# stefanopini/simple-HRNet

Hardware: AMD Instinct MI355X
Metric: person-crops/sec HRNet-W48 384x288 (model forward + heat-map decode) (higher is better)
Workload: dtype bf16; 1 GPU; HRNet-W48 384x288, batch=256 random crops per GPU, bf16 MFMA (BASELINE configs[2]); global_batch=256, micro_batch=256, lanes_per_gpu=1, parallelism=dp1 (crop sharding, RCCL all-gather of keypoints), weights=random-init seeded (synth_state_dict seed 0), BN stats randomised, engine_switches=

## Files before the change

include/hrnet_mi355.h:

```cpp
#ifndef HRNET_MI355_H
#define HRNET_MI355_H

#include <stddef.h>
#include <stdint.h>

#ifdef __cplusplus
extern "C" {
#endif

typedef struct hrn_ctx *hrn_handle;

enum { HRN_F32 = 0, HRN_BF16 = 1, HRN_F16 = 2 };
enum { HRN_BOX_I32 = 0, HRN_BOX_F32 = 1 };
enum { HRN_T_F32 = 0, HRN_T_I64 = 1 };

typedef struct {
    const char *name;
    const void *data;
    int32_t ndim;
    int64_t dims[4];
    int32_t dtype;
} hrn_tensor_desc;

typedef struct {
// ... 117 lines not shown
enum { HRN_LB_RGB = 0, HRN_LB_BGR = 1 };
enum { HRN_DET_COMPACT = 1 };
enum { HRN_DET_MAX_CLASSES = 16 };
typedef struct { int32_t new_w, new_h, left, top; double ratio_w, ratio_h, dw, dh; } hrn_letterbox;
int hrn_letterbox_geometry(int rule, const int32_t *frame_hw , int n, int out_h, int out_w,
                           hrn_letterbox *out );
const char *hrn_letterbox_last_error(void);
int hrn_letterbox_frames(hrn_handle h, const hrn_frame *frames_host, int n, int rule, int out_h, int out_w,
                         const uint8_t *pad , int order, int form, void *out_dev, hrn_letterbox *geometry_host ,
                         void *stream);
int hrn_letterbox_frames_yuv(hrn_handle h, const hrn_yuv_frame *frames_host, int n, int rule, int out_h, int out_w,
                             const uint8_t *pad , int order, int form, void *out_dev,
                             hrn_letterbox *geometry_host , void *stream);
int hrn_detections_to_frame(int rule, const float *dets, int det_stride, const int32_t *start , int P,
                            const hrn_letterbox *geometry, const int32_t *frame_hw , int out_h, int out_w,
                            int conf_col, float conf_thres, int class_col, const int32_t *classes, int nclasses, int flags,
                            float *dets_out, int32_t *counts_out , int32_t *status_out );
int hrn_detections_to_frame_dev(hrn_handle h, int rule, const float *dets_dev, int det_stride, const int32_t *start_host, int P,
                                const hrn_letterbox *geometry_host, const int32_t *frame_hw_host, int out_h, int out_w,
                                int conf_col, float conf_thres, int class_col, const int32_t *classes_host, int nclasses, int flags,
                                float *dets_out_dev, int32_t *counts_dev, int32_t *status_dev, void *stream);

enum { HRN_INTER_NEAREST = 0, HRN_INTER_LINEAR = 1, HRN_INTER_CUBIC = 2 };
int hrn_resize_frames(hrn_handle h, const uint8_t *frames_dev, int n, int frame_h, int frame_w, int interpolation,
                      float *images_dev, void *stream);

int hrn_warp_crops(hrn_handle h, const uint8_t *frames_dev, int nframes, int frame_h, int frame_w,
                   const int32_t *frame_index_host, const double *matrices_host, int n, float *images_dev, void *stream);

int hrn_forward_flip_tta(hrn_handle h, const void *images_dev, int n, const int32_t *flip_pairs_host, int npairs,
                         int post_processing, float *heatmaps_dev, float *preds_dev, float *maxvals_dev, void *stream);

int hrn_target_centers(const double *joints, const float *vis, const float *joints_weight , int n, int J,
                       int height, int width, double sigma, int32_t *mu_out, float *draw_out, float *target_weight_out);
int hrn_generate_targets(hrn_handle h, const double *joints_host, const float *vis_host, const float *joints_weight_host,
                         int n, double sigma, float *targets_dev, float *target_weight_host, void *stream);
typedef struct {
    double *loss_mse, *loss_ohkm;
    float *avg_acc;
    int32_t *cnt;
    float *acc, *dists;
    double *map_loss;
    float *preds, *target_preds, *maxvals;
} hrn_score_out;
int hrn_score_heatmaps(hrn_handle h, const float *heatmaps_dev, int n, const float *targets_dev, const double *joints_host,
                       const float *vis_host, const float *joints_weight_host, double sigma, const float *target_weight_host,
                       float pck_thr, int ohkm_topk, const hrn_score_out *out_dev, void *stream);

enum { HRN_REFINE_NONE = 0, HRN_REFINE_QUARTER = 1, HRN_REFINE_DARK = 2 };
int hrn_forward_refined(hrn_handle h, const void *images_dev, int n, const void *boxes_dev, int box_dtype, int refine,
                        float *pts_dev, float *heatmaps_dev, void *stream);
int hrn_refine_coords(hrn_handle h, const float *heatmaps_dev, int n, int refine, float *coords_dev, void *stream);

int hrn_nms(int32_t *keep_out, int32_t *num_out, const float *boxes_host, int boxes_num, int boxes_dim,
            float nms_overlap_thresh, int device_id);
int hrn_nms_release(int device_id);
const char *hrn_nms_last_error(void);

int hrn_oks_nms(int32_t *keep_out, int32_t *num_out, const double *kpts, const double *areas, const int32_t *order, int n, int J,
                double thresh, const double *sigmas, double in_vis_thre);
int hrn_soft_oks_nms(int32_t *keep_out, int32_t *num_out, const double *kpts, const double *areas, const double *scores_sorted,
                     const int32_t *order, int n, int J, double thresh, const double *sigmas, double in_vis_thre);
int hrn_pose_similarity(const double *boxes_a, const float *poses_a, int na, const double *boxes_b, const float *poses_b, int nb, int J,
                        float *sim_bbox, float *sim_pose);
int hrn_assignment(const double *cost, int rows, int cols, int32_t *row_to_col);

typedef struct {
    char name[96];
    int32_t c, h, w;
    int32_t conv_index;
} hrn_tap_info;
int hrn_tap_count(hrn_handle h);
int hrn_get_tap_info(hrn_handle h, int index, hrn_tap_info *out);
int hrn_forward_tap(hrn_handle h, const void *images_dev, int n, const char *tap_name, int crop0, int ncrops, int crop_step,
                    float *dst_dev, float *heatmaps_dev, void *stream);

int hrn_conv_count(hrn_handle h);
int hrn_get_conv_info(hrn_handle h, int index, hrn_conv_info *out);
double hrn_flops_per_crop(hrn_handle h);
int64_t hrn_workspace_bytes(hrn_handle h);
int64_t hrn_map_rebuilds(hrn_handle h);
int hrn_launches_per_pass(hrn_handle h);
int hrn_stem_fused(hrn_handle h);
int hrn_conv_compact(hrn_handle h, int index);
const char *hrn_switches(hrn_handle h);
int64_t hrn_debug_pad_violations(hrn_handle h);
int hrn_plan_block_map(hrn_handle h, int group, int n, int reverse, int32_t *blocks, int capacity, int32_t *members,
                       int member_capacity);
int hrn_plan_direct_map(hrn_handle h, int group, int n, int32_t *blocks, int capacity, int32_t *members, int member_capacity,
                        int32_t *pixels_per_tile);
int hrn_plan_s2_map(hrn_handle h, int group, int n, int32_t *blocks, int capacity, int32_t *parts, int part_capacity,
                    int32_t *active);
int hrn_profile_pass(hrn_handle h, const void *images_dev, int n, float *conv_ms, int conv_ms_len,
                     float *other_ms , void *stream);
const char *hrn_version(void);

#ifdef __cplusplus
}
#endif
#endif
```

simple-hrnet_amd/_lib.py:

```python
from __future__ import annotations

import ctypes
import os
import shutil
import subprocess
from typing import List

_HERE = os.path.dirname(os.path.abspath(__file__))
CSRC = os.path.join(_HERE, "csrc")
INCLUDE = os.path.join(os.path.dirname(_HERE), "include")
LIB_PATH = os.path.join(_HERE, "libhrnet_mi355.so")
if os.environ.get("HRN_LIB_TAG"):
    LIB_PATH = LIB_PATH.replace(".so", "_%s.so" % os.environ["HRN_LIB_TAG"])
SOURCES = ["kernels.hip", "conv3x3_lds.hip", "conv_s2.hip", "stem_fused.hip", "conv3x3_f32.hip", "bottleneck_chain.hip", "prepath.hip", "warp.hip", "nms.hip", "postproc.cpp", "hrnet_mi355.cpp",
           "decode.hip",
           "score.hip",
           "draw.hip",
           "track.hip",
           "pose_nms.hip",
           "letterbox.hip",
           "assoc.hip",
           "conv3x3_lds_f16.hip", "conv_s2_f16.hip", "bottleneck_chain_f16.hip"]
HEADERS = [os.path.join(CSRC, "kernels.h"), os.path.join(CSRC, "dt16.h"), os.path.join(CSRC, "argmax.h"), os.path.join(CSRC, "conv3x3_n96.inc"), os.path.join(CSRC, "conv3x3_lds.inc"),
           os.path.join(CSRC, "conv_s2.inc"), os.path.join(CSRC, "bottleneck_chain.inc"), os.path.join(INCLUDE, "hrnet_mi355.h")]
# ... 45 lines not shown

def _stale(src: str) -> bool:
    o = _obj(src)
    if not os.path.exists(o) or not _stamp_ok():
        return True
    t = os.path.getmtime(o)
    return any(os.path.getmtime(d) > t for d in _deps(src))


def needs_build() -> bool:
    if not os.path.exists(LIB_PATH):
        return True
    if os.environ.get("HRN_LIB_TAG"):
        return False
    t = os.path.getmtime(LIB_PATH)
    deps = set()
    for s in SOURCES:
        deps.update(_deps(s))
    if any(os.path.getmtime(d) > t for d in deps):
        return True
    if os.path.isdir(_obj_dir()) and not _stamp_ok():
        return shutil.which("hipcc") is not None or os.path.exists("/opt/rocm/bin/hipcc")
    return False


def build(force: bool = False, verbose: bool = False) -> str:
    if not force and not needs_build():
        return LIB_PATH
    import fcntl
    from concurrent.futures import ThreadPoolExecutor

    os.makedirs(_obj_dir(), exist_ok=True)
    with open(os.path.join(_obj_dir(), "build.lock"), "w") as lock:
        fcntl.flock(lock, fcntl.LOCK_EX)
        try:
            if force or needs_build():
                os.makedirs(_obj_dir(), exist_ok=True)
                cflags = [f for f in HIPCC_FLAGS if f != "-shared"]

                def compile_one(src):
                    tmp = "%s.tmp.%d" % (_obj(src), os.getpid())
                    cmd = [_hipcc()] + cflags + ["-c", "-o", tmp, os.path.join(CSRC, src)]
                    if verbose:
                        print(" ".join(cmd), flush=True)
                    subprocess.check_call(cmd)
                    os.replace(tmp, _obj(src))

                todo = [s for s in SOURCES if force or _stale(s)]
                stamp = _stamp()
                with ThreadPoolExecutor(max_workers=min(len(todo), os.cpu_count() or 4, MAX_BUILD_WORKERS) or 1) as ex:
                    list(ex.map(compile_one, todo))
                tmp = "%s.tmp.%d" % (LIB_PATH, os.getpid())
                cmd = [_hipcc(), "--offload-arch=gfx950", "-shared", "-fPIC", "-o", tmp] + [_obj(s) for s in SOURCES]
                if verbose:
                    print(" ".join(cmd), flush=True)
                subprocess.check_call(cmd)
                with open(os.path.join(_obj_dir(), "build.stamp"), "w") as f:
                    f.write(stamp + "\n")
                os.replace(tmp, LIB_PATH)
        finally:
            fcntl.flock(lock, fcntl.LOCK_UN)
    return LIB_PATH


class TensorDesc(ctypes.Structure):
    _fields_ = [("name", ctypes.c_char_p), ("data", ctypes.c_void_p), ("ndim", ctypes.c_int32),
                ("dims", ctypes.c_int64 * 4), ("dtype", ctypes.c_int32)]


class ConvInfo(ctypes.Structure):
    _fields_ = [("name", ctypes.c_char * 96),
                ("cin", ctypes.c_int32), ("cout", ctypes.c_int32), ("ksize", ctypes.c_int32),
                ("stride", ctypes.c_int32), ("relu", ctypes.c_int32), ("has_residual", ctypes.c_int32),
                ("in_h", ctypes.c_int32), ("in_w", ctypes.c_int32), ("out_h", ctypes.c_int32),
                ("out_w", ctypes.c_int32), ("kpad", ctypes.c_int32), ("nr", ctypes.c_int32),
                ("algo", ctypes.c_int32), ("ks", ctypes.c_int32),
                ("w_offset", ctypes.c_int64), ("w_bytes", ctypes.c_int64), ("b_offset", ctypes.c_int64),
                ("flops", ctypes.c_double)]


class TapInfo(ctypes.Structure):
    _fields_ = [("name", ctypes.c_char * 96), ("c", ctypes.c_int32), ("h", ctypes.c_int32), ("w", ctypes.c_int32),
                ("conv_index", ctypes.c_int32)]


class ScoreOut(ctypes.Structure):
    _fields_ = [(name, ctypes.c_void_p) for name in ("loss_mse", "loss_ohkm", "avg_acc", "cnt", "acc", "dists", "map_loss", "preds",
                                                     "target_preds", "maxvals")]


class Frame(ctypes.Structure):
    _fields_ = [("data", ctypes.c_void_p), ("height", ctypes.c_int32), ("width", ctypes.c_int32)]


class YuvFrameC(ctypes.Structure):
    _fields_ = [("y", ctypes.c_void_p), ("u", ctypes.c_void_p), ("v", ctypes.c_void_p), ("height", ctypes.c_int32),
                ("width", ctypes.c_int32), ("pitch_y", ctypes.c_int32), ("pitch_c", ctypes.c_int32), ("format", ctypes.c_int32),
                ("matrix", ctypes.c_int32), ("range", ctypes.c_int32)]


class Letterbox(ctypes.Structure):
    _fields_ = [("new_w", ctypes.c_int32), ("new_h", ctypes.c_int32), ("left", ctypes.c_int32), ("top", ctypes.c_int32),
                ("ratio_w", ctypes.c_double), ("ratio_h", ctypes.c_double), ("dw", ctypes.c_double), ("dh", ctypes.c_double)]


class CanvasC(ctypes.Structure):
    _fields_ = list(YuvFrameC._fields_)


_P = ctypes.c_void_p
SYMBOLS = {
    "hrn_create": (ctypes.c_int, [ctypes.POINTER(_P), ctypes.c_int, ctypes.c_int, ctypes.c_int, ctypes.c_int,
                                  ctypes.c_int, ctypes.c_int, ctypes.c_int]),
    "hrn_create_model": (ctypes.c_int, [ctypes.POINTER(_P), ctypes.c_int, ctypes.c_int, ctypes.c_int, ctypes.c_int,
                                        ctypes.c_int, ctypes.c_int, ctypes.c_int, ctypes.c_int]),
    "hrn_destroy": (None, [_P]),
    "hrn_last_error": (ctypes.c_char_p, [_P]),
    "hrn_load_weights": (ctypes.c_int, [_P, ctypes.POINTER(TensorDesc), ctypes.c_int]),
    "hrn_weight_blob_bytes": (ctypes.c_int64, [_P]),
    "hrn_weight_blob_ptr": (_P, [_P]),
    "hrn_adopt_weights": (ctypes.c_int, [_P]),
    "hrn_weight_blob_read": (ctypes.c_int, [_P, ctypes.c_int64, _P, ctypes.c_int64]),
    "hrn_forward": (ctypes.c_int, [_P, _P, ctypes.c_int, _P, ctypes.c_int, _P, _P, _P]),
    "hrn_resize_frames": (ctypes.c_int, [_P, _P, ctypes.c_int, ctypes.c_int, ctypes.c_int, ctypes.c_int, _P, _P]),
    "hrn_warp_crops": (ctypes.c_int, [_P, _P, ctypes.c_int, ctypes.c_int, ctypes.c_int, _P, _P, ctypes.c_int, _P, _P]),
    "hrn_target_centers": (ctypes.c_int, [_P, _P, _P, ctypes.c_int, ctypes.c_int, ctypes.c_int, ctypes.c_int, ctypes.c_double, _P, _P, _P]),
    "hrn_generate_targets": (ctypes.c_int, [_P, _P, _P, _P, ctypes.c_int, ctypes.c_double, _P, _P, _P]),
    "hrn_score_heatmaps": (ctypes.c_int, [_P, _P, ctypes.c_int, _P, _P, _P, _P, ctypes.c_double, _P, ctypes.c_float, ctypes.c_int,
                                          ctypes.POINTER(ScoreOut), _P]),
    "hrn_preprocess_frame": (ctypes.c_int, [_P, _P, ctypes.c_int, ctypes.c_int, _P, ctypes.c_int, ctypes.c_int, ctypes.c_int, _P, _P, _P, _P]),
    "hrn_preprocess_frames": (ctypes.c_int, [_P, ctypes.POINTER(Frame), ctypes.c_int, _P, ctypes.c_int, _P, ctypes.c_int, ctypes.c_int, _P, _P, _P, _P]),
    "hrn_yuv_coefficients": (ctypes.c_int, [ctypes.c_int, ctypes.c_int, _P]),
    "hrn_yuv_to_bgr": (ctypes.c_int, [_P, ctypes.POINTER(YuvFrameC), _P, _P]),
    "hrn_preprocess_frames_yuv": (ctypes.c_int, [_P, ctypes.POINTER(YuvFrameC), ctypes.c_int, _P, ctypes.c_int, _P, ctypes.c_int, ctypes.c_int,
                                                 _P, _P, _P, _P]),
    "hrn_draw_poses": (ctypes.c_int, [_P, ctypes.POINTER(CanvasC), ctypes.c_int, _P, ctypes.c_int, ctypes.c_int, _P, _P, ctypes.c_int,
                                      _P, ctypes.c_int, _P, ctypes.c_int, _P, ctypes.c_int, ctypes.c_int, ctypes.c_float, _P]),
    "hrn_draw_poses_ids_dev": (ctypes.c_int, [_P, ctypes.POINTER(CanvasC), ctypes.c_int, _P, ctypes.c_int, ctypes.c_int, _P, _P, ctypes.c_int,
                                              _P, ctypes.c_int, _P, ctypes.c_int, _P, ctypes.c_int, ctypes.c_int, ctypes.c_float, _P]),
    "hrn_associate_people": (ctypes.c_int, [ctypes.c_int, _P, _P, ctypes.c_int, _P, _P, _P, _P, _P, _P, ctypes.c_double, ctypes.c_double,
                                            ctypes.c_double, _P, _P, _P]),
    "hrn_associate_people_last_error": (ctypes.c_char_p, []),
    "hrn_associate_people_dev": (ctypes.c_int, [_P, ctypes.c_int, _P, _P, ctypes.c_int, _P, _P, _P, _P, _P, _P, ctypes.c_double,
                                                ctypes.c_double, ctypes.c_double, _P, _P, _P, _P]),
    "hrn_assoc_exp": (ctypes.c_int, [_P, ctypes.c_int, _P]),
    "hrn_associate_similarity": (ctypes.c_int, [_P, _P, ctypes.c_int, _P, _P, ctypes.c_int, ctypes.c_int, ctypes.c_double, _P, _P]),
    "hrn_pose_nms": (ctypes.c_int, [ctypes.c_int, _P, ctypes.c_int, ctypes.c_int, _P, _P, _P, ctypes.c_double, ctypes.c_double,
                                    ctypes.c_double, _P, _P, _P, _P, _P, _P]),
    "hrn_pose_nms_last_error": (ctypes.c_char_p, []),
    "hrn_pose_nms_dev": (ctypes.c_int, [_P, ctypes.c_int, _P, ctypes.c_int, ctypes.c_int, _P, _P, _P, ctypes.c_double, ctypes.c_double,
                                        ctypes.c_double, _P, _P, _P, _P, _P, _P, _P]),
    "hrn_pose_nms_oks_row": (ctypes.c_int, [ctypes.c_int, ctypes.c_int, ctypes.c_int, _P, _P, ctypes.c_int, ctypes.c_double, _P, _P]),
    "hrn_letterbox_geometry": (ctypes.c_int, [ctypes.c_int, _P, ctypes.c_int, ctypes.c_int, ctypes.c_int, _P]),
    "hrn_letterbox_last_error": (ctypes.c_char_p, []),
    "hrn_letterbox_frames": (ctypes.c_int, [_P, ctypes.POINTER(Frame), ctypes.c_int, ctypes.c_int, ctypes.c_int, ctypes.c_int, _P, ctypes.c_int,
                                            ctypes.c_int, _P, _P, _P]),
    "hrn_letterbox_frames_yuv": (ctypes.c_int, [_P, ctypes.POINTER(YuvFrameC), ctypes.c_int, ctypes.c_int, ctypes.c_int, ctypes.c_int, _P,
                                                ctypes.c_int, ctypes.c_int, _P, _P, _P]),
    "hrn_detections_to_frame": (ctypes.c_int, [ctypes.c_int, _P, ctypes.c_int, _P, ctypes.c_int, _P, _P, ctypes.c_int, ctypes.c_int, ctypes.c_int,
                                               ctypes.c_float, ctypes.c_int, _P, ctypes.c_int, ctypes.c_int, _P, _P, _P]),
    "hrn_detections_to_frame_dev": (ctypes.c_int, [_P, ctypes.c_int, _P, ctypes.c_int, _P, ctypes.c_int, _P, _P, ctypes.c_int, ctypes.c_int,
                                                   ctypes.c_int, ctypes.c_float, ctypes.c_int, _P, ctypes.c_int, ctypes.c_int, _P, _P, _P, _P]),
    "hrn_yuv_from_bgr": (ctypes.c_int, [ctypes.c_int, ctypes.c_int, _P, ctypes.c_int, _P]),
    "hrn_crop_geometry": (ctypes.c_int, [_P, ctypes.c_int, ctypes.c_int, _P, ctypes.c_int, ctypes.c_int, ctypes.c_int, ctypes.c_int, _P, _P]),
    "hrn_crop_geometry_last_error": (ctypes.c_char_p, []),
    "hrn_pose_boxes": (ctypes.c_int, [_P, ctypes.c_int, ctypes.c_int, _P, ctypes.c_int, ctypes.c_float, ctypes.c_int, ctypes.c_double,
                                      ctypes.c_double, _P]),
    "hrn_pose_boxes_last_error": (ctypes.c_char_p, []),
    "hrn_boxes_from_poses": (ctypes.c_int, [_P, _P, ctypes.c_int, ctypes.c_int, _P, ctypes.c_int, ctypes.c_float, ctypes.c_int,
                                            ctypes.c_double, ctypes.c_double, _P, _P]),
    "hrn_preprocess_frames_dev": (ctypes.c_int, [_P, ctypes.POINTER(Frame), ctypes.c_int, _P, ctypes.c_int, _P, ctypes.c_int, ctypes.c_int,
                                                 _P, _P, _P, _P]),
    "hrn_preprocess_frames_yuv_dev": (ctypes.c_int, [_P, ctypes.POINTER(YuvFrameC), ctypes.c_int, _P, ctypes.c_int, _P, ctypes.c_int,
                                                     ctypes.c_int, _P, _P, _P, _P]),
    "hrn_forward_flip_tta": (ctypes.c_int, [_P, _P, ctypes.c_int, _P, ctypes.c_int, ctypes.c_int, _P, _P, _P, _P]),
    "hrn_forward_refined": (ctypes.c_int, [_P, _P, ctypes.c_int, _P, ctypes.c_int, ctypes.c_int, _P, _P, _P]),
    "hrn_refine_coords": (ctypes.c_int, [_P, _P, ctypes.c_int, ctypes.c_int, _P, _P]),
    "hrn_nms": (ctypes.c_int, [_P, _P, _P, ctypes.c_int, ctypes.c_int, ctypes.c_float, ctypes.c_int]),
    "hrn_nms_release": (ctypes.c_int, [ctypes.c_int]),
    "hrn_nms_last_error": (ctypes.c_char_p, []),
    "hrn_oks_nms": (ctypes.c_int, [_P, _P, _P, _P, _P, ctypes.c_int, ctypes.c_int, ctypes.c_double, _P, ctypes.c_double]),
    "hrn_soft_oks_nms": (ctypes.c_int, [_P, _P, _P, _P, _P, _P, ctypes.c_int, ctypes.c_int, ctypes.c_double, _P, ctypes.c_double]),
    "hrn_pose_similarity": (ctypes.c_int, [_P, _P, ctypes.c_int, _P, _P, ctypes.c_int, ctypes.c_int, _P, _P]),
    "hrn_assignment": (ctypes.c_int, [_P, ctypes.c_int, ctypes.c_int, _P]),
    "hrn_tap_count": (ctypes.c_int, [_P]),
    "hrn_get_tap_info": (ctypes.c_int, [_P, ctypes.c_int, ctypes.POINTER(TapInfo)]),
    "hrn_forward_tap": (ctypes.c_int, [_P, _P, ctypes.c_int, ctypes.c_char_p, ctypes.c_int, ctypes.c_int, ctypes.c_int, _P, _P, _P]),
    "hrn_conv_count": (ctypes.c_int, [_P]),
    "hrn_get_conv_info": (ctypes.c_int, [_P, ctypes.c_int, ctypes.POINTER(ConvInfo)]),
    "hrn_flops_per_crop": (ctypes.c_double, [_P]),
    "hrn_workspace_bytes": (ctypes.c_int64, [_P]),
    "hrn_map_rebuilds": (ctypes.c_int64, [_P]),
    "hrn_launches_per_pass": (ctypes.c_int, [_P]),
    "hrn_switches": (ctypes.c_char_p, [_P]),
    "hrn_stem_fused": (ctypes.c_int, [_P]),
    "hrn_conv_compact": (ctypes.c_int, [_P, ctypes.c_int]),
    "hrn_debug_pad_violations": (ctypes.c_int64, [_P]),
    "hrn_plan_block_map": (ctypes.c_int, [_P, ctypes.c_int, ctypes.c_int, ctypes.c_int, _P, ctypes.c_int, _P, ctypes.c_int]),
    "hrn_plan_direct_map": (ctypes.c_int, [_P, ctypes.c_int, ctypes.c_int, _P, ctypes.c_int, _P, ctypes.c_int, _P]),
    "hrn_plan_s2_map": (ctypes.c_int, [_P, ctypes.c_int, ctypes.c_int, _P, ctypes.c_int, _P, ctypes.c_int, _P]),
    "hrn_profile_pass": (ctypes.c_int, [_P, _P, ctypes.c_int, ctypes.POINTER(ctypes.c_float), ctypes.c_int,
                                        ctypes.POINTER(ctypes.c_float), _P]),
    "hrn_version": (ctypes.c_char_p, []),
}

_lib = None


def load(auto_build: bool = True) -> ctypes.CDLL:
    global _lib
    if _lib is not None:
        return _lib
    if auto_build and needs_build():
        build()
    lib = ctypes.CDLL(LIB_PATH)
    for name, (res, args) in SYMBOLS.items():
        fn = getattr(lib, name)
        fn.restype = res
        fn.argtypes = args
    _lib = lib
    return lib


def header_symbols() -> List[str]:
    import re

    text = open(os.path.join(INCLUDE, "hrnet_mi355.h")).read()
    text = re.sub(r"/\*.*?\*/", "", text, flags=re.S)
    return sorted(set(re.findall(r"\b(hrn_[a-z_0-9]+)\s*\(", text)))
```

simple-hrnet_amd/csrc/ctx_memory.inc:

```
    bool hip_ok(hipError_t e, const char *what) {
        if (e == hipSuccess) return true;
        err = std::string(what) + ": " + hipGetErrorString(e);
        return false;
    }
    bool refuse_plan_only() {
        if (plan_only) err = "plan-only handle (device_id < 0): there is no CPU compute path";
        return plan_only;
    }

    bool allocate() {
        workspace_bytes = 0;
        for (auto &b : buffers) workspace_bytes += (int64_t)b.bytes;
        const int64_t small_crops = std::min<int64_t>(max_batch, (191 + head_slabs) / head_slabs);
        const int64_t part = std::max((int64_t)max_batch * joints * head_slabs, small_crops * joints * head_slabs_small);
        workspace_bytes += part * 8;
        if (plan_only) {
            fill_problems();
            index_s2groups();
            blob = (char *)calloc(1, (size_t)blob_bytes);
            return blob != nullptr;
        }
        if (!hip_ok(hipSetDevice(device), "hipSetDevice")) return false;
        for (auto &b : buffers) {
            if (!hip_ok(hipMalloc((void **)&b.dev, b.bytes), "hipMalloc(activation)")) return false;
// ... 45 lines not shown
        const bool keep_short_full = small && small_keep_above > 0 && small_blocks > small_keep_above;
        auto short_conv = [&](const ConvOp &cv) { return cv.ks != 16 && !cv.n96 && (cv.ks == 48 ? 2 : 1) * cv.slices <= 2; };
        auto small_conv = [&](const ConvOp &cv) {
            if (cv.ks == 16 && f32_small_slices > 0 && cv.slices >= f32_small_slices) return true;
            return small && !(keep_short_full && short_conv(cv));
        };
        auto tile_px = [&](const ConvOp &cv, const Tensor &to) {
            return fused_now(cv, nb) ? 512 : small_conv(cv) ? 128 : conv3x3_lds_bm(cv.ks, cv.nr, to.wp);
        };
        auto tiles_per_block = [&](const ConvOp &cv, int div) {
            return std::max(1, conv3_tiles_per_block(cv) / (fused_now(cv, nb) ? bbf_tpb_div : 1) / div);
        };
        auto count_blocks = [&](int div) {
            long total = 0;
            for (int ci : g.conv_idx) {
                const ConvOp &cv = convs[ci];
                if (skipped(cv, nb)) continue;
                const Tensor &to = tensors[cv.out_t];
                const int bm = tile_px(cv, to);
                const int mtiles = (int)((m_pixels(cv, to, nb) + bm - 1) / bm);
                const int tpb = tiles_per_block(cv, div);
                total += (long)((mtiles + tpb - 1) / tpb) * cv.ntiles;
            }
            return total;
        };
        int div = 1;
        while (div < 64 && count_blocks(div) < 512) div *= 2;
        int lf = all_short ? 1 : (int)std::min<long>(long_factor, count_blocks(div) / 768);
        if (lf < 1) lf = 1;
        for (size_t k = 0; k < g.conv_idx.size(); ++k) {
            const ConvOp &cv = convs[g.conv_idx[k]];
            if (skipped(cv, nb)) continue;
            const Tensor &to = tensors[cv.out_t];
            const int bm = tile_px(cv, to);
            const bool fused = fused_now(cv, nb);
            const int prob = fused ? g.fused_prob[k] : (int)k;
            const int mtiles = (int)((m_pixels(cv, to, nb) + bm - 1) / bm);
            const int tpb_short = tiles_per_block(cv, div);
            const int tpb_long = tpb_short * lf;
            const int long_tiles = ((int)(mtiles * long_share) / (8 * tpb_long)) * (8 * tpb_long);
            for (int phase = 0; phase < 2; ++phase) {
                const int tpb = phase == 0 ? tpb_long : tpb_short;
                const int first = phase == 0 ? 0 : long_tiles;
                const int count = phase == 0 ? long_tiles : mtiles - long_tiles;
                if (count <= 0) continue;
                const int mgroups = (count + tpb - 1) / tpb;
                const int total = mgroups * cv.ntiles;
                int seq = 0;
                for (int round = 0; round * 8 < mgroups; ++round)
                    for (int nt = 0; nt < cv.ntiles; ++nt)
                        for (int x = 0; x < 8; ++x) {
                            const int mg = round * 8 + x;
                            if (mg >= mgroups) continue;
                            const int i = seq++;
                            int tiles = count - mg * tpb;
                            if (tiles > tpb) tiles = tpb;
                            double key = (i + 0.5) / total;
                            if (block_order == 1)
                                key = -(fused ? 28000.0 + (tiles - 1) * bbf_slide_cost
                                        : (double)tiles * (cv.ks == 16 ? cv.slices * (double)bm * 36.0 + 2000.0
                                                        : cv.n96      ? cv.slices * 3.0 * (bm == 512 ? 3900.0 : 3000.0) + (bm == 512 ? 7000.0 : 5000.0)
                                                                 : cv.slices * 2.0 * (bm == 512 ? 4300.0 : 3500.0) + (bm == 512 ? 5000.0 : 3000.0))) +
                                      1e-3 * key;
                            int mt0 = first + mg * tpb;
                            if (reverse) mt0 = mtiles - mt0 - tiles;
                            ents.push_back({key, int2{prob | (nt << 8) | (tiles << 16), mt0 | (fused ? 1 << 29 : small_conv(cv) ? 1 << 30 : 0)}, bm});
                        }
            }
        }
        std::stable_sort(ents.begin(), ents.end(), [](const Ent &a, const Ent &b) { return a.key < b.key; });
        if (tile_px_out) {
            tile_px_out->resize(ents.size());
            for (size_t i = 0; i < ents.size(); ++i) (*tile_px_out)[i] = ents[i].bm;
        }
        if (out) {
            out->resize(ents.size());
            for (size_t i = 0; i < ents.size(); ++i) (*out)[i] = ents[i].v;
        }
        return (int)ents.size();
    }

    const Tensor &grid_of(const ConvOp &cv) const { return tensors[cv.up ? cv.in_t : cv.out_t]; }

    ConvArgs conv_args(const ConvOp &cv, int nb, bool rev) const {
        const Tensor &ti = tensors[cv.in_t], &to = grid_of(cv);
        ConvArgs a;
        a.in = row0(cv.in_t), a.out = row0(cv.out_t);
        a.w = blob + cv.w_off, a.bias = (const float *)(blob + cv.b_off);
        a.res = cv.res_t >= 0 ? row0(cv.res_t) : nullptr;
        a.cin = cv.cin, a.cout = cv.cout;
        a.in_wp = ti.wp, a.in_hpwp = ti.hpwp;
        a.out_h = to.h, a.out_w = to.w, a.out_wp = to.wp, a.out_hpwp = to.hpwp;
        a.m = nb * to.hpwp;
        a.ksize = cv.k, a.stride = cv.stride, a.relu = cv.relu, a.kchunks = cv.kchunks;
        a.rev = rev;
        a.pre_mode = pre_mode;
        a.wlds = direct_wlds && is16() ? 1 : 0;
        a.xlds = conv_xl(cv) ? 1 : 0;
        a.up = cv.up ? 1 : 0, a.up_a = cv.up ? (cv.up - 1) >> 1 : 0, a.up_b = cv.up ? (cv.up - 1) & 1 : 0;
        a.up_wp = tensors[cv.out_t].wp, a.up_hpwp = tensors[cv.out_t].hpwp;
        for (int t = 0; t < 4; ++t) {
            const int dy = (t >> 1) - 1 + a.up_a, dx = (t & 1) - 1 + a.up_b;
            a.taps[t] = cv.up ? dy * ti.wp + dx : 0;
        }
        return a;
    }

    int direct_group_blocks(const DirectGroup &g, int nb, std::vector<int2> *out, int mr = 4) const {
        struct Cls {
            int in_t, k, stride;
            std::vector<int> members;
            double cost = 0;
        };
        std::vector<Cls> cls;
        for (size_t k = 0; k < g.conv_idx.size(); ++k) {
            const ConvOp &cv = convs[g.conv_idx[k]];
            size_t ci = 0;
            for (; ci < cls.size(); ++ci)
                if (cls[ci].in_t == cv.in_t && cls[ci].k == cv.k && cls[ci].stride == cv.stride) break;
            if (ci == cls.size()) cls.push_back(Cls{cv.in_t, cv.k, cv.stride, {}, 0});
            cls[ci].members.push_back((int)k);
            cls[ci].cost += (double)grid_of(cv).hpwp * (cv.cout / (16 * g.nr)) * cv.kchunks;
        }
        std::stable_sort(cls.begin(), cls.end(), [](const Cls &a, const Cls &b) { return a.cost > b.cost; });
        int n = 0;
        if (out) out->clear();
        for (const Cls &cl : cls) {
            const int mtiles = (nb * grid_of(convs[g.conv_idx[cl.members[0]]]).hpwp + 64 * mr - 1) / (64 * mr);
            for (int round = 0; round * 8 < mtiles; ++round)
                for (int k : cl.members) {
                    const int ngroups = convs[g.conv_idx[k]].cout / (16 * g.nr);
                    for (int ng = 0; ng < ngroups; ++ng)
                        for (int x = 0; x < 8; ++x, ++n)
                            if (out) out->push_back(int2{k | (ng << 8), round * 8 + x});
                }
        }
        return n;
    }

    int64_t m_pixels(const ConvOp &cv, const Tensor &to, int nb) const {
        return cv.compact ? (int64_t)nb * to.h * to.w : (int64_t)nb * to.hpwp;
    }
    static int compact_slab_rows(int h, int w, int bm, int crops) {
        const int wp = w + 1, hpwp = (h + 1) * wp, hw = h * w;
        auto flat = [&](int64_t c) { const int64_t n = c / hw, r = c % hw; return n * hpwp + (r / w) * wp + r % w; };
        const int64_t m = (int64_t)crops * hw;
        int64_t span = 0;
        for (int64_t c0 = 0; c0 < m; c0 += bm) span = std::max(span, flat(std::min(c0 + bm, m) - 1) - flat(c0) + 1);
        return (int)span + 2 * wp + 2;
    }

    bool setup_dgroups() {
        for (auto &g : dgroups) {
            g.map_capacity = std::max<int64_t>(direct_group_blocks(g, max_batch, nullptr), 4 * 512 + 64 * (int64_t)g.conv_idx.size() * 8);
            for (MapSlot &sl : g.slot) {
                if (!alloc_slot(sl, g.map_capacity, g.conv_idx.size())) return false;
                workspace_bytes += g.map_capacity * (int64_t)sizeof(int2) + (int64_t)(g.conv_idx.size() * sizeof(ConvArgs));
            }
        }
        return true;
    }

    size_t index_s2groups() {
        size_t n = 0;
        for (auto &g : s2groups) g.prob_first = (int)n, n += g.probs.size();
        if (stem_fuse) stemf.prob_first = (int)n, n += stemf.probs.size();
        return n;
    }
    long s2_tiles(const S2Group &g, int nb) const {
        long t = 0;
        for (auto &pr : g.probs) t += (long)nb * pr.tiles_per_image;
        return t;
    }
    bool s2_active(const S2Group &g, int nb) const { return s2_tiles(g, nb) >= s2_min_tiles; }
    int s2_blocks(const S2Group &g, int nb, std::vector<int2> *out) const {
        struct Ent {
            double key;
            int2 v;
        };
        std::vector<double> cost(g.probs.size());
        double total = 0;
        for (size_t k = 0; k < g.probs.size(); ++k) {
            const S2Group::Prob &pr = g.probs[k];
            const Tensor &to = tensors[convs[pr.parts[0].first].out_t];
            const int frags = (pr.rows * to.wp + 15) / 16;
            const int wm = std::max(1, 8 / (int)pr.parts.size());
            const int cin = convs[pr.parts[0].first].cin;
            cost[k] = (double)((frags + wm - 1) / wm) * ((9 * cin + 31) / 32) * s2_frags_per_part(cin) + 60;
            total += cost[k] * nb * pr.tiles_per_image;
        }
        const double per_block = total / s2_target_blocks;
        std::vector<Ent> ents;
        for (size_t k = 0; k < g.probs.size(); ++k) {
            const S2Group::Prob &pr = g.probs[k];
            const int tiles = nb * pr.tiles_per_image;
            int run = (int)(per_block / cost[k] + 0.5);
            run = run < 1 ? 1 : run > 64 ? 64 : run;
            if (&g == &stemf) run = (tiles + s2_target_blocks - 1) / s2_target_blocks;
            for (int t0 = 0; t0 < tiles; t0 += run) {
                const int cnt = tiles - t0 < run ? tiles - t0 : run;
                ents.push_back({-(cnt * cost[k]) + 1e-9 * t0, int2{(int)k | (cnt << 8), t0}});
            }
        }
        std::stable_sort(ents.begin(), ents.end(), [](const Ent &a, const Ent &b) { return a.key < b.key; });
        if (out) {
            out->resize(ents.size());
            for (size_t i = 0; i < ents.size(); ++i) (*out)[i] = ents[i].v;
        }
        return (int)ents.size();
    }

    static void s2_wave_table(int nparts, unsigned char *part, unsigned char *f0, unsigned char *fs) {
        struct W {
            int p, i, m;
        };
        std::vector<W> ws;
        for (int p = 0; p < nparts; ++p) {
            const int m = std::max(1, 8 / nparts + (p < 8 % nparts ? 1 : 0));
            for (int i = 0; i < m && (int)ws.size() < 8; ++i) ws.push_back({p, i, m});
        }
        std::stable_sort(ws.begin(), ws.end(), [](const W &a, const W &b) { return a.m < b.m; });
        double load[4] = {0, 0, 0, 0};
        bool used[8] = {};
        for (int w = 0; w < 8; ++w) part[w] = 0xff, f0[w] = 0, fs[w] = 1;
        for (const W &x : ws) {
            int best = -1;
            for (int w = 0; w < 8; ++w)
                if (!used[w] && (best < 0 || load[w & 3] < load[best & 3] - 1e-12)) best = w;
            used[best] = true;
            load[best & 3] += 1.0 / x.m;
            part[best] = (unsigned char)x.p, f0[best] = (unsigned char)x.i, fs[best] = (unsigned char)x.m;
        }
    }

    bool setup_s2groups() {
        const size_t nprob = index_s2groups();
        if (!nprob) return true;
        std::vector<S2Problem> hp(nprob);
        std::vector<S2Group *> all;
        for (auto &g : s2groups) all.push_back(&g);
        if (stem_fuse) all.push_back(&stemf);
// ... 91 lines not shown

    size_t fill_problems() {
        const size_t nprob = index_groups();
        probs_host.assign(nprob, Conv3Problem{});
        std::vector<Conv3Problem> &hp = probs_host;
        for (auto &g : groups) {
            g.max_wp = 0;
            for (size_t k = 0; k < g.conv_idx.size(); ++k) {
                const ConvOp &cv = convs[g.conv_idx[k]];
                const Tensor &to = tensors[cv.out_t];
                Conv3Problem &q = hp[g.prob_first + k];
                q.in = row0(cv.in_t), q.out = row0(cv.out_t);
                q.w = blob + cv.w_off, q.bias = (const float *)(blob + cv.b_off);
                q.res = cv.res_t >= 0 ? row0(cv.res_t) : nullptr;
                q.cin = cv.cin, q.cout = cv.cout, q.h = to.h, q.wd = to.w, q.wp = to.wp, q.hpwp = to.hpwp;
                q.relu = cv.relu, q.slices = cv.slices, q.ntiles = cv.ntiles;
                q.w2 = nullptr, q.bias2 = nullptr;
                q.n96 = cv.n96 ? 1 : 0;
                q.compact = cv.compact ? 1 : 0, q.hw = to.h * to.w;
                q.slab_rows = q.slab_rows_small = 0;
                if (cv.compact) {
                    fast_div(q.hw, &q.magic_hw, &q.shift_hw);
                    fast_div(to.w, &q.magic_w, &q.shift_w);
                    q.slab_rows = compact_slab_rows(to.h, to.w, 512, max_batch), q.slab_rows_small = compact_slab_rows(to.h, to.w, 128, max_batch);
                }
                q.tiles_per_block = conv3_tiles_per_block(cv);
                q.bm = conv3x3_lds_bm(cv.ks, cv.nr, to.wp);
                fast_div(to.hpwp, &q.magic_hpwp, &q.shift_hpwp);
                fast_div(to.wp, &q.magic_wp, &q.shift_wp);
                if (to.wp > g.max_wp) g.max_wp = to.wp;
                if (cv.fuse_with >= 0) {
                    const ConvOp &c2 = convs[cv.fuse_with];
                    Conv3Problem &f = hp[g.prob_first + g.fused_prob[k]];
                    f = q;
                    f.out = row0(c2.out_t), f.relu = c2.relu, f.res = nullptr;
                    f.w2 = blob + c2.w_off, f.bias2 = (const float *)(blob + c2.b_off);
                }
            }
        }
        return nprob;
    }

    bool setup_groups() {
        const size_t nprob = fill_problems();
        if (!nprob) return true;
        std::vector<Conv3Problem> &hp = probs_host;
        for (auto &g : groups) {
            g.map_capacity = 64 + 4 * (int64_t)std::max(small_below, 256) + 1024;
            for (int ci : g.conv_idx) {
                const ConvOp &cv = convs[ci];
                const Tensor &to = tensors[cv.out_t];
                const int bm = f32_small_slices > 0 ? 128 : conv3x3_lds_bm(cv.ks, cv.nr, to.wp);
                g.map_capacity += (int64_t)((max_batch * to.hpwp + bm - 1) / bm) * cv.ntiles;
            }
            for (MapSlot &sl : g.slot) {
                if (!alloc_slot(sl, g.map_capacity, 0)) return false;
                workspace_bytes += g.map_capacity * (int64_t)sizeof(int2);
            }
        }
        if (!hip_ok(hipMalloc((void **)&probs_dev, nprob * sizeof(Conv3Problem)), "hipMalloc(problems)")) return false;
        return hip_ok(hipMemcpy(probs_dev, hp.data(), nprob * sizeof(Conv3Problem), hipMemcpyHostToDevice),
                      "hipMemcpy(problems)");
    }

    void free_all() {
        if (plan_only) {
            free(blob);
        } else {
            (void)hipSetDevice(device);
            for (auto &b : buffers)
                if (b.dev) (void)hipFree(b.dev);
            if (blob) (void)hipFree(blob);
            if (scratch_hm) (void)hipFree(scratch_hm);
            free_scratch();
            if (part_val) (void)hipFree(part_val);
            if (part_idx) (void)hipFree(part_idx);
            if (probs_dev) (void)hipFree(probs_dev);
            if (s2probs_dev) (void)hipFree(s2probs_dev);
            for (auto &g : s2groups)
                for (MapSlot &sl : g.slot) free_slot(sl);
            for (MapSlot &sl : stemf.slot) free_slot(sl);
            for (auto &g : groups)
                for (MapSlot &sl : g.slot) free_slot(sl);
            for (auto &g : dgroups)
                for (MapSlot &sl : g.slot) free_slot(sl);
        }
        blob = nullptr;
    }

    char *row0(int t) const {
        const Tensor &tt = tensors[t];
        const Buffer &b = buffers[tt.buf];
        return b.dev ? b.dev + b.lead_rows * tt.c * esize : nullptr;
    }
```

simple-hrnet_amd/csrc/ctx_plan.inc:

```
    int new_tensor(int ch, int h, int w) {
        Tensor t;
        t.c = ch, t.h = h, t.w = w, t.wp = w + 1, t.hp = h + 1, t.hpwp = t.wp * t.hp;
        for (size_t i = 0; i < buffers.size(); ++i)
            if (!buffers[i].in_use && buffers[i].c == ch && buffers[i].h == h && buffers[i].w == w) {
                t.buf = (int)i;
                break;
            }
        if (t.buf < 0) {
            Buffer b;
            b.c = ch, b.h = h, b.w = w;
            b.lead_rows = (size_t)t.wp + 1;
            b.rows = b.lead_rows + (size_t)max_batch * t.hpwp + t.wp + 1 + kConvBlockRows;
            b.bytes = (size_t)align_up((int64_t)(b.rows * ch * esize), 256);
            buffers.push_back(b);
            t.buf = (int)buffers.size() - 1;
        }
        buffers[t.buf].in_use = true;
        tensors.push_back(t);
        return (int)tensors.size() - 1;
    }
    void release(int t) { buffers[tensors[t].buf].in_use = false; }

    int default_nr(int cout, int stride) const {
        int nr = (cout % 64 == 0) ? 4 : (cout % 48 == 0) ? 3 : 2;
        if (is16() && stride == 2 && cout % 96 == 0 && direct_nr6) nr = 6;
        return nr;
    }
    int common_nr(const std::vector<int> &couts, int stride) const {
        bool all64 = true, all48 = true, all96 = true;
        for (int co : couts) all64 &= co % 64 == 0, all48 &= co % 48 == 0, all96 &= co % 96 == 0;
        if (is16() && stride == 2 && all96 && direct_nr6) return 6;
        return all64 ? 4 : all48 ? 3 : 2;
    }

    static int s2_rows(int wop, int ho, int cin) {
        const int r = (s2_slot_capacity(cin) - 2 * wop) / s2_pair_pitch(wop);
        return r > ho ? ho : (r < 0 ? 0 : r);
    }

    int add_conv(const std::string &conv, const std::string &bn, int in_t, int cout, int k, int stride, int relu,
                 int res_t = -1, bool emit = true, int nr_override = 0, int up = 0, int up_out_t = -1, bool force_generic = false) {
        const Tensor ti = tensors[in_t];
        ConvOp op;
        op.conv = conv, op.bn = bn, op.in_t = in_t, op.res_t = res_t;
        op.cin = ti.c, op.cout = cout, op.k = k, op.stride = stride, op.relu = relu;
        const int oh = ti.h / stride, ow = ti.w / stride;
        op.up = up;
        op.out_t = up ? up_out_t : new_tensor(cout, oh, ow);
        const int kc = is16() ? 32 : 16;
        const int K = k * k * op.cin;
        op.kchunks = (K + kc - 1) / kc;
        op.kpad = op.kchunks * kc;
        op.nr = nr_override ? nr_override : default_nr(cout, stride);
        op.flops = 2.0 * cout * (double)K * oh * ow;
        int lds_ks = 0, lds_nrb = 0;
        if (is16() && k == 3 && stride == 1 && !disable_lds && !up && !force_generic) {
            const int64_t out_bytes = ((int64_t)max_batch * (oh + 1) * (ow + 1) + 2 * (ow + 2) + 512) * std::max(op.cin, cout) * 2;
            if (!disable_n96 && op.cin % 32 == 0 && cout % 96 == 0 && conv3x3_lds_bm(32, 6, ow + 1) > 0 && out_bytes < (int64_t(1) << 32))
                lds_ks = 32, lds_nrb = 6, op.n96 = true;
            else if (op.cin % 48 == 0 && cout % 48 == 0)
                lds_ks = 48, lds_nrb = 3;
            else if (op.cin % 32 == 0 && !disable_lds32)
                lds_ks = 32, lds_nrb = cout % 64 == 0 ? 4 : cout % 48 == 0 ? 3 : cout % 32 == 0 ? 2 : 0;
            if (lds_nrb && conv3x3_lds_bm(lds_ks, lds_nrb, ow + 1) == 0) lds_nrb = 0;
            if (op.n96 && lds_nrb == 6 && !disable_compact && conv3x3_lds_bm(32, 6, ow + 1) == 512 &&
                1.0 - (double)(oh * ow) / ((oh + 1) * (ow + 1)) >= compact_min_pad &&
                (compact_slab_rows(oh, ow, 512, max_batch) + 15) / 16 * 16 <= conv3x3_n96_max_rows() && (int64_t)max_batch * oh * ow < (int64_t(1) << 27))
                op.compact = true;
        }
        if (lds_nrb) {
            op.algo = 1, op.ks = lds_ks, op.nr = lds_nrb;
            op.slices = op.cin / lds_ks, op.ntiles = cout / (16 * lds_nrb), op.nch = (9 * lds_ks + 31) / 32;
            op.kpad = op.nch * 32 * op.slices;
        }
        if (dtype == HRN_F32 && k == 3 && stride == 1 && !up && !disable_lds && !disable_f32lds && op.cin % 16 == 0 &&
            (cout % 48 == 0 || cout % 32 == 0) && conv3x3_lds_bm(16, cout % 48 == 0 ? 3 : 2, ow + 1) > 0) {
            op.algo = 1, op.ks = 16, op.nr = cout % 48 == 0 ? 3 : 2;
            op.slices = op.cin / 16, op.ntiles = cout / (16 * op.nr), op.nch = 9;
            op.kpad = 9 * 16 * op.slices;
        }
        if (is16() && k == 3 && stride == 2 && (op.cin == 48 || op.cin == 32 || op.cin == 64) &&
            cout % (16 * s2_frags_per_part(op.cin)) == 0 && !up && !disable_s2 && op.algo == 0 &&
            (s2_rows(ow + 1, oh, op.cin) >= 2 || s2_rows(ow + 1, oh, op.cin) == oh))
            op.s2 = true;
        convs.push_back(op);
        if (emit) emit_convs({(int)convs.size() - 1});
        return op.out_t;
    }

    static int c3_family(const ConvOp &cv) { return ((cv.ks == 48 && cv.nr == 3) || cv.n96) ? 0 : cv.ks * 16 + cv.nr; }

    void emit_direct(const std::vector<int> &idx, std::vector<Op> &dst) {
        std::vector<std::vector<int>> dsets;
        for (int i : idx) {
            if (disable_dgroup) {
                dst.push_back({OP_CONV, i});
                continue;
            }
            bool placed = false;
            for (auto &set : dsets)
                if (convs[set[0]].nr == convs[i].nr && set.size() < 255) {
                    set.push_back(i);
                    placed = true;
                    break;
                }
            if (!placed) dsets.push_back({i});
        }
        for (auto &set : dsets) {
            if (set.size() == 1) {
                dst.push_back({OP_CONV, set[0]});
                continue;
            }
            DirectGroup g;
            g.conv_idx = set, g.nr = convs[set[0]].nr;
            dgroups.push_back(g);
            dst.push_back({OP_CONV_GROUP, (int)dgroups.size() - 1});
        }
    }

    void emit_convs(const std::vector<int> &idx) {
        std::vector<int> lds, direct, s2;
        for (int i : idx) {
            if (convs[i].algo == 1)
                lds.push_back(i);
            else if (convs[i].s2)
                s2.push_back(i);
            else
                direct.push_back(i);
        }
        emit_direct(direct, ops);
        if (!s2.empty()) {
            S2Group g;
            g.conv_idx = s2;
            for (int i : s2) {
                const ConvOp &cv = convs[i];
                for (int t = 0; t < cv.cout / (16 * s2_frags_per_part(cv.cin)); ++t) {
                    S2Group::Prob *pr = nullptr;
                    for (auto &q : g.probs)
                        if (q.in_t == cv.in_t && (int)q.parts.size() < kS2MaxParts) pr = &q;
                    if (!pr) {
                        g.probs.push_back(S2Group::Prob());
                        pr = &g.probs.back();
                        pr->in_t = cv.in_t;
                        const Tensor &to = tensors[cv.out_t];
                        pr->rows = s2_rows(to.wp, to.h, cv.cin);
                        pr->tiles_per_image = (to.h + pr->rows - 1) / pr->rows;
                    }
                    pr->parts.push_back({i, t});
                }
            }
            emit_direct(s2, g.fallback);
            s2groups.push_back(g);
            ops.push_back({OP_S2_GROUP, (int)s2groups.size() - 1});
        }
        if (lds.empty()) return;
        std::vector<std::vector<int>> sets;
        for (int i : lds) {
            bool placed = false;
            if (!disable_group)
                for (auto &set : sets)
                    if (c3_family(convs[set[0]]) == c3_family(convs[i])) {
                        set.push_back(i);
                        placed = true;
                        break;
                    }
            if (!placed) sets.push_back({i});
        }
        for (auto &set : sets) {
            Conv3Group g;
            g.conv_idx = set;
            groups.push_back(g);
            ops.push_back({OP_CONV3_GROUP, (int)groups.size() - 1});
        }
    }

    int add_fuse(const std::vector<int> &terms, const std::vector<int> &shifts, const std::string &name) {
        FuseOp f;
        f.name = name;
        f.nterms = (int)terms.size();
        for (int i = 0; i < f.nterms; ++i) f.term_t[i] = terms[i], f.shift[i] = shifts[i];
        const Tensor &t0 = tensors[terms[0]];
        int ref = -1;
        for (int i = 0; i < f.nterms; ++i)
            if (shifts[i] == 0) ref = terms[i];
        const Tensor &tr = tensors[ref >= 0 ? ref : terms[0]];
        (void)t0;
        f.out_t = new_tensor(tr.c, tr.h, tr.w);
        fuses.push_back(f);
        return f.out_t;
    }

    void add_stage(const std::string &name, std::vector<int> &xs, int nout) {
        const int nb = (int)xs.size();
        char buf[160];
        for (int k = 0; k < 4; ++k) {
            std::vector<int> t1(nb), g1, g2;
            for (int b = 0; b < nb; ++b) {
                snprintf(buf, sizeof buf, "%s.branches.%d.%d", name.c_str(), b, k);
                const std::string p = buf;
                t1[b] = add_conv(p + ".conv1", p + ".bn1", xs[b], c << b, 3, 1, 1, -1, false);
                g1.push_back((int)convs.size() - 1);
            }
            emit_convs(g1);
            for (int b = 0; b < nb; ++b) {
                snprintf(buf, sizeof buf, "%s.branches.%d.%d", name.c_str(), b, k);
                const std::string p = buf;
                const int t2 = add_conv(p + ".conv2", p + ".bn2", t1[b], c << b, 3, 1, 1, xs[b], false);
                const int i2 = (int)convs.size() - 1, i1 = g1[b];
                const ConvOp &a1 = convs[i1], &a2 = convs[i2];
                if (!disable_bbf && is16() && a1.algo == 1 && a2.algo == 1 && a1.ks == 48 && a1.nr == 3 && a1.slices == 1 &&
                    a1.ntiles == 1 && a2.slices == 1 && a2.ntiles == 1 && conv3x3_lds_bbf_ok(tensors[t2].wp)) {
                    convs[i1].fuse_with = i2;
                    convs[i2].fused_away = true;
                }
                g2.push_back(i2);
                release(t1[b]);
                release(xs[b]);
                xs[b] = t2;
            }
            emit_convs(g2);
        }
        std::vector<std::vector<int>> term(nout, std::vector<int>(nb, -1));
        std::vector<std::vector<int>> cur(nout, std::vector<int>(nb, -1));
        for (int level = 0; level < nb; ++level) {
            std::vector<int> made, dead;
            for (int j = 0; j < nb; ++j) {
                std::vector<int> c1, c2;
                if (level == 0)
                    for (int i = 0; i < nout && i < j; ++i) c1.push_back(c << i);
                for (int i = j + 1 + level; i < nout; ++i)
                    if (level == 0) c2.push_back(i - j == 1 ? (c << i) : (c << j));
                const int nr1 = (dgroup_nr_mode == 1 && c1.size() > 1) ? common_nr(c1, 1) : 0;
                const int nr2 = (dgroup_nr_mode == 1 && c2.size() > 1) ? common_nr(c2, 2) : 0;
                for (int i = 0; i < nout; ++i) {
                    snprintf(buf, sizeof buf, "%s.fuse_layers.%d.%d", name.c_str(), i, j);
                    const std::string q = buf;
                    if (i < j && level == 0) {
                        term[i][j] = add_conv(q + ".0", q + ".1", xs[j], c << i, 1, 1, 0, -1, false, nr1);
                        made.push_back((int)convs.size() - 1);
                    } else if (i > j && level < i - j) {
                        const bool last = (level == i - j - 1);
                        snprintf(buf, sizeof buf, "%s.%d", q.c_str(), level);
                        const std::string qq = buf;
                        const int src = level == 0 ? xs[j] : cur[i][j];
                        const int nt = add_conv(qq + ".0", qq + ".1", src, last ? (c << i) : (c << j), 3, 2, last ? 0 : 1, -1,
                                                false, level == 0 ? nr2 : 0);
                        made.push_back((int)convs.size() - 1);
                        if (level > 0) dead.push_back(src);
                        cur[i][j] = nt;
                        if (last) term[i][j] = nt;
                    }
                }
            }
            if (made.empty()) break;
            emit_convs(made);
            for (int t : dead) release(t);
        }
        std::vector<int> outs;
        for (int i = 0; i < nout; ++i) {
            std::vector<int> terms, shifts;
            for (int j = 0; j < nb; ++j) {
                terms.push_back(i == j ? xs[j] : term[i][j]);
                shifts.push_back(i < j ? j - i : 0);
            }
            snprintf(buf, sizeof buf, "%s.fuse.%d", name.c_str(), i);
            outs.push_back(add_fuse(terms, shifts, buf));
        }
        {
            const int first = (int)fuses.size() - nout;
            for (int i = 0; i < nout; ++i) {
                fuses[first + i].group = disable_fgroup ? 1 : (i == 0 ? nout : 0);
                if (fuses[first + i].group) ops.push_back({OP_FUSE, first + i});
            }
        }
        for (int i = 0; i < nout; ++i)
            for (int j = 0; j < nb; ++j)
                if (i != j) release(term[i][j]);
        for (int b = 0; b < nb; ++b) release(xs[b]);
        xs = outs;
    }

    int add_layer1(int x, int nblocks) {
        char buf[96];
        int o1_next = -1;
        for (int b = 0; b < nblocks; ++b) {
            snprintf(buf, sizeof buf, "layer1.%d", b);
            const std::string p = buf;
            int o1 = o1_next, r = x;
            const bool chain = is16() && !disable_chain && b < nblocks - 1;
            int ds_idx = -1;
            if (b == 0 && chain && !disable_chain_ds) {
                o1 = add_conv(p + ".conv1", p + ".bn1", x, 64, 1, 1, 1);
                r = add_conv(p + ".downsample.0", p + ".downsample.1", x, 256, 1, 1, 0, -1, false, 2);
                ds_idx = (int)convs.size() - 1;
                release(r);
            } else if (b == 0) {
                o1 = add_conv(p + ".conv1", p + ".bn1", x, 64, 1, 1, 1, -1, false);
                r = add_conv(p + ".downsample.0", p + ".downsample.1", x, 256, 1, 1, 0, -1, false);
                emit_convs({(int)convs.size() - 2, (int)convs.size() - 1});
            } else if (o1 < 0) {
                o1 = add_conv(p + ".conv1", p + ".bn1", x, 64, 1, 1, 1);
            }
            const bool c2_generic = is16() && b >= 1;
            const bool chain3 = c2_generic && !disable_chain && !disable_chain3;
            const int o2 = c2_generic ? add_conv(p + ".conv2", p + ".bn2", o1, 64, 3, 1, 1, -1, !chain3, 2, 0, -1, true)
                                      : add_conv(p + ".conv2", p + ".bn2", o1, 64, 3, 1, 1);
            const int i2 = (int)convs.size() - 1;
            int o3;
            o1_next = -1;
            if (chain3 && !chain) {
                o3 = add_conv(p + ".conv3", p + ".bn3", o2, 256, 1, 1, 1, r, false, 2);
                chains.push_back({(int)convs.size() - 1, -1, -1, i2});
                ops.push_back({OP_CHAIN, (int)chains.size() - 1});
            } else if (chain) {
                snprintf(buf, sizeof buf, "layer1.%d", b + 1);
                const std::string pn = buf;
                o3 = add_conv(p + ".conv3", p + ".bn3", o2, 256, 1, 1, 1, r, false, 2);
                const int i3 = (int)convs.size() - 1;
                o1_next = add_conv(pn + ".conv1", pn + ".bn1", o3, 64, 1, 1, 1, -1, false, 4);
                chains.push_back({i3, (int)convs.size() - 1, ds_idx, chain3 ? i2 : -1});
                ops.push_back({OP_CHAIN, (int)chains.size() - 1});
            } else {
                o3 = add_conv(p + ".conv3", p + ".bn3", o2, 256, 1, 1, 1, r);
            }
            release(o1), release(o2);
            if (b == 0 && ds_idx < 0) release(r);
            release(x);
            x = o3;
        }
        return x;
    }

    void build_plan_poseresnet() {
        static const int spec50[4] = {3, 4, 6, 3}, spec101[4] = {3, 4, 23, 3}, spec152[4] = {3, 8, 36, 3};
        const int *layers = c == 50 ? spec50 : c == 101 ? spec101 : spec152;
        stem_out_t = new_tensor(64, H / 2, W / 2);
        ops.push_back({OP_STEM7, 0});
        int x = new_tensor(64, H / 4, W / 4);
        pool_in_t = stem_out_t, pool_out_t = x;
        ops.push_back({OP_MAXPOOL, 0});
        release(stem_out_t);
        char buf[96];
        x = add_layer1(x, layers[0]);
        for (int li = 1; li < 4; ++li) {
            const int planes = 64 << li;
            for (int b = 0; b < layers[li]; ++b) {
                snprintf(buf, sizeof buf, "layer%d.%d", li + 1, b);
                const std::string p = buf;
                const int stride = (b == 0 && li > 0) ? 2 : 1;
                int r = x;
                const int o1 = add_conv(p + ".conv1", p + ".bn1", x, planes, 1, 1, 1, -1, false);
                std::vector<int> first{(int)convs.size() - 1};
                if (b == 0) {
                    r = add_conv(p + ".downsample.0", p + ".downsample.1", x, planes * 4, 1, stride, 0, -1, false);
                    first.push_back((int)convs.size() - 1);
                }
                emit_convs(first);
                const int o2 = add_conv(p + ".conv2", p + ".bn2", o1, planes, 3, stride, 1);
                const int o3 = add_conv(p + ".conv3", p + ".bn3", o2, planes * 4, 1, 1, 1, r);
                release(o1), release(o2);
                if (b == 0) release(r);
                release(x);
                x = o3;
            }
        }
        for (int i = 0; i < 3; ++i) {
            const Tensor tx = tensors[x];
            const int up_t = new_tensor(256, tx.h * 2, tx.w * 2);
            snprintf(buf, sizeof buf, "deconv_layers.%d", 3 * i);
            const std::string cn = buf;
            snprintf(buf, sizeof buf, "deconv_layers.%d", 3 * i + 1);
            const std::string bn = buf;
            std::vector<int> phases;
            for (int ph = 0; ph < 4; ++ph) {
                add_conv(cn, bn, x, 256, 2, 1, 1, -1, false, 0, 1 + ph, up_t);
                phases.push_back((int)convs.size() - 1);
            }
            emit_convs(phases);
            release(x);
            x = up_t;
        }
        head_in_t = x;
        head_c = tensors[x].c;
        ops.push_back({OP_HEAD, 0});
        ops.push_back({OP_DECODE, 0});
        layout_blob();
    }

    void build_plan() {
        if (model == 1) return build_plan_poseresnet();
        head_c = c;
        stem_out_t = new_tensor(64, H / 2, W / 2);
        ops.push_back({OP_STEM, 0});
        int x = add_conv("conv2", "bn2", stem_out_t, 64, 3, 2, 1);
        stem_conv2_op = (int)ops.size() - 1;
        if (is16() && !disable_stem_fuse && !disable_stem_mfma && stem_fused_fits(tensors[x].wp, W)) {
            stem_fuse = true;
            convs.back().w2_image = true;
            stemf = S2Group();
            stemf.conv_idx = {(int)convs.size() - 1};
            for (int t = 0; t < 2; ++t) {
                if (stemf.probs.empty()) {
                    stemf.probs.push_back(S2Group::Prob());
                    stemf.probs[0].in_t = stem_out_t;
                    stemf.probs[0].rows = 1, stemf.probs[0].tiles_per_image = tensors[x].h;
                }
                stemf.probs[0].parts.push_back({(int)convs.size() - 1, t});
            }
        }
        release(stem_out_t);
        char buf[96];
        x = add_layer1(x, 4);
        std::vector<int> xs;
        xs.push_back(add_conv("transition1.0.0", "transition1.0.1", x, c, 3, 1, 1, -1, false));
        xs.push_back(add_conv("transition1.1.0.0", "transition1.1.0.1", x, 2 * c, 3, 2, 1, -1, false));
        emit_convs({(int)convs.size() - 2, (int)convs.size() - 1});
        release(x);
        add_stage("stage2.0", xs, 2);
        xs.push_back(add_conv("transition2.2.0.0", "transition2.2.0.1", xs[1], 4 * c, 3, 2, 1));
        for (int m = 0; m < 4; ++m) {
            snprintf(buf, sizeof buf, "stage3.%d", m);
            add_stage(buf, xs, 3);
        }
        xs.push_back(add_conv("transition3.3.0.0", "transition3.3.0.1", xs[2], 8 * c, 3, 2, 1));
        add_stage("stage4.0", xs, 4);
        add_stage("stage4.1", xs, 4);
        add_stage("stage4.2", xs, 1);
        head_in_t = xs[0];
        ops.push_back({OP_HEAD, 0});
        ops.push_back({OP_DECODE, 0});

        layout_blob();
    }

    void index_taps() {
        taps.clear();
        auto add = [&](const std::string &name, int tensor, int op, int conv) {
            for (TapPoint &t : taps)
                if (t.name == name) {
                    t.op = op;
                    return;
                }
            taps.push_back(TapPoint{name, tensor, op, conv});
        };
        for (size_t oi = 0; oi < ops.size(); ++oi) {
            const Op &op = ops[oi];
            switch (op.kind) {
                case OP_STEM:
                case OP_STEM7: add("stem", stem_out_t, (int)oi, -1); break;
                case OP_MAXPOOL: add("maxpool", pool_out_t, (int)oi, -1); break;
                case OP_CONV: add(convs[op.idx].conv, convs[op.idx].out_t, (int)oi, op.idx); break;
                case OP_CONV3_GROUP:
                    for (int ci : groups[op.idx].conv_idx) add(convs[ci].conv, convs[ci].out_t, (int)oi, ci);
                    break;
                case OP_CONV_GROUP:
                    for (int ci : dgroups[op.idx].conv_idx) add(convs[ci].conv, convs[ci].out_t, (int)oi, ci);
                    break;
                case OP_S2_GROUP:
                    for (int ci : s2groups[op.idx].conv_idx) add(convs[ci].conv, convs[ci].out_t, (int)oi, ci);
                    break;
                case OP_CHAIN:
                    add(convs[chains[op.idx].conv3].conv, convs[chains[op.idx].conv3].out_t, (int)oi, chains[op.idx].conv3);
                    if (chains[op.idx].conv1 >= 0)
                        add(convs[chains[op.idx].conv1].conv, convs[chains[op.idx].conv1].out_t, (int)oi, chains[op.idx].conv1);
                    break;
                case OP_FUSE:
                    for (int k = 0; k < fuses[op.idx].group; ++k) add(fuses[op.idx + k].name, fuses[op.idx + k].out_t, (int)oi, -1);
                    break;
                default: break;
            }
        }
    }

    void layout_blob() {
        int64_t off = 0;
        stem_w_off = off, off = align_up(off + (model == 1 ? 147 : 27) * 64 * 4, 256);
        stem_b_off = off, off = align_up(off + 64 * 4, 256);
        stem_wp_off = off, off = align_up(off + (model == 1 ? 5 : 1) * 4 * 1024, 256);
        for (auto &cv : convs) {
            cv.w_off = off;
            cv.w_bytes = cv.algo == 1 ? (int64_t)cv.ntiles * cv.slices * cv.nch * cv.nr * 1024
                                      : (int64_t)(cv.cout / 16) * cv.kchunks * 1024;
            off = align_up(off + cv.w_bytes, 256);
            cv.b_off = off;
            off = align_up(off + cv.cout * 4, 256);
            if (cv.s2 || cv.w2_image) {
                const int nf = s2_frags_per_part(cv.cin);
                cv.w2_off = off;
                cv.w2_bytes = (int64_t)(cv.cout / (16 * nf)) * ((9 * cv.cin + 31) / 32) * nf * 1024;
                off = align_up(off + cv.w2_bytes, 256);
            }
        }
        head_w_off = off, off = align_up(off + (int64_t)joints * head_c * 4, 256);
        head_b_off = off, off = align_up(off + joints * 4, 256);
        head_wp_off = off, off = align_up(off + (int64_t)((joints + 31) / 32) * 2 * ((head_c + 31) / 32) * 1024, 256);
        blob_bytes = off;

        const int hw = (H / 4) * (W / 4);
        head_slab_px = 1024;
        head_slabs = (hw + head_slab_px - 1) / head_slab_px;
        head_slabs_small = (hw + kHeadSlabPxSmall - 1) / kHeadSlabPxSmall;
    }
```

simple-hrnet_amd/csrc/ctx_run.inc:

```
    struct Timing {
        std::vector<hipEvent_t> ev;
    };

    bool run_pass(const float *images, int nb, const void *boxes, int box_dtype, float *pts, float *heatmaps,
                  hipStream_t s, Timing *tm, int flip = 0, const TapReq *tap = nullptr, int refine = RF_NONE) {
        if (tm && !hip_ok(hipEventRecord(tm->ev[0], s), "hipEventRecord")) return false;
        const bool fused_stem = stem_fuse && !(tap && tap->op == 0);
        for (size_t oi = 0; oi < ops.size(); ++oi) {
            const bool rev = alternate && (oi & 1);
            hipError_t e = hipSuccess;
            if (fused_stem && oi == 0)
                e = exec_stem_fused(images, nb, s, flip);
            else if (!(fused_stem && (int)oi == stem_conv2_op))
                e = exec_op(ops[oi], rev, images, nb, boxes, box_dtype, pts, heatmaps, s, flip, refine);
            if (!hip_ok(e, "kernel launch")) return false;
            if (tap && tap->op == (int)oi) {
                const Tensor &t = tensors[tap->tensor];
                TapArgs a;
                a.in = row0(tap->tensor), a.dst = tap->dst;
                a.c = t.c, a.h = t.h, a.w = t.w, a.wp = t.wp, a.hpwp = t.hpwp;
                a.crop0 = tap->crop0, a.ncrops = tap->ncrops, a.crop_step = tap->crop_step;
                if (!hip_ok(launch_tap(dtype, a, s), "tap launch")) return false;
            }
            if (tm && !hip_ok(hipEventRecord(tm->ev[oi + 1], s), "hipEventRecord")) return false;
        }
        return true;
    }

    hipError_t exec_stem_fused(const float *images, int nb, hipStream_t s, int flip) {
        S2Group &g = stemf;
        bool hit;
        MapSlot *sl = find_slot(g.slot, nb, &hit);
        hipError_t e = slot_ready(sl, hit, s);
        if (e != hipSuccess) return e;
        if (!hit) {
            sl->nblocks = s2_blocks(g, nb, &g.map_host);
            if (sl->nblocks > g.map_capacity) return hipErrorInvalidValue;
            memcpy(sl->pin, g.map_host.data(), (size_t)sl->nblocks * sizeof(int2));
            e = hipMemcpyAsync(sl->dev, sl->pin, (size_t)sl->nblocks * sizeof(int2), hipMemcpyHostToDevice, s);
            if (e == hipSuccess) e = hipEventRecord(sl->landed, s);
            if (e != hipSuccess) return e;
            sl->nb = nb;
            ++map_builds;
        }
        const Tensor &t = tensors[stem_out_t];
        StemArgs a;
        a.images = images, a.out = nullptr;
        a.w = nullptr, a.bias = (const float *)(blob + stem_b_off), a.wp = (const void *)(blob + stem_wp_off);
        a.n = nb, a.H = H, a.W = W;
        a.out_h = t.h, a.out_w = t.w, a.out_wp = t.wp, a.out_hpwp = t.hpwp;
        a.flip = flip;
        return launch_stem_fused(dtype, s2probs_dev + g.prob_first, sl->dev, sl->nblocks, a, s);
    }

    hipError_t exec_op(const Op &op, bool rev, const float *images, int nb, const void *boxes, int box_dtype, float *pts,
                       float *heatmaps, hipStream_t s, int flip, int refine) {
        hipError_t e = hipSuccess;
        switch (op.kind) {
        case OP_STEM: {
            const Tensor &t = tensors[stem_out_t];
            StemArgs a;
            a.images = images, a.out = row0(stem_out_t);
            a.w = (const float *)(blob + stem_w_off), a.bias = (const float *)(blob + stem_b_off);
            a.wp = (is16() && !disable_stem_mfma) ? (const void *)(blob + stem_wp_off) : nullptr;
            a.n = nb, a.H = H, a.W = W;
            a.out_h = t.h, a.out_w = t.w, a.out_wp = t.wp, a.out_hpwp = t.hpwp;
            a.flip = flip;
            e = launch_stem(dtype, a, s);
            break;
        }
        case OP_STEM7: {
            const Tensor &t = tensors[stem_out_t];
            Stem7Args a;
            a.images = images, a.out = row0(stem_out_t);
            a.w = (const float *)(blob + stem_w_off), a.bias = (const float *)(blob + stem_b_off);
            a.wp = (is16() && !disable_stem_mfma) ? (const void *)(blob + stem_wp_off) : nullptr;
            a.n = nb, a.H = H, a.W = W;
            a.out_h = t.h, a.out_w = t.w, a.out_wp = t.wp, a.out_hpwp = t.hpwp;
            a.flip = flip;
            e = launch_stem7(dtype, a, s);
            break;
        }
        case OP_MAXPOOL: {
            const Tensor &ti = tensors[pool_in_t], &to = tensors[pool_out_t];
            PoolArgs a;
            a.in = row0(pool_in_t), a.out = row0(pool_out_t);
            a.c = to.c, a.n = nb, a.in_wp = ti.wp, a.in_hpwp = ti.hpwp;
            a.out_h = to.h, a.out_w = to.w, a.out_wp = to.wp, a.out_hpwp = to.hpwp;
            e = launch_maxpool(dtype, a, s);
            break;
        }
        case OP_CONV: {
            const ConvOp &cv = convs[op.idx];
            const ConvArgs a = conv_args(cv, nb, rev);
            e = launch_conv(dtype, a, cv.nr, s);
            break;
        }
        case OP_CONV3_GROUP: {
            Conv3Group &g = groups[op.idx];
            bool hit;
            MapSlot *sl = find_slot(g.slot, nb, &hit);
            if ((e = slot_ready(sl, hit, s)) != hipSuccess) break;
            if (!hit) {
                sl->nblocks = group_blocks(g, nb, &g.map_host, rev);
                if (sl->nblocks > g.map_capacity) {
                    e = hipErrorInvalidValue;
                    break;
                }
                memcpy(sl->pin, g.map_host.data(), (size_t)sl->nblocks * sizeof(int2));
                e = hipMemcpyAsync(sl->dev, sl->pin, (size_t)sl->nblocks * sizeof(int2), hipMemcpyHostToDevice, s);
                if (e == hipSuccess) e = hipEventRecord(sl->landed, s);
                if (e != hipSuccess) break;
                sl->nb = nb;
                ++map_builds;
            }
            e = (dtype == HRN_F16 ? launch_conv3x3_lds_f16 : launch_conv3x3_lds)(probs_dev + g.prob_first, sl->dev, sl->nblocks, nb,
                                                                             convs[g.conv_idx[0]].ks, convs[g.conv_idx[0]].nr, s);
            break;
        }
        case OP_CONV_GROUP: {
            DirectGroup &g = dgroups[op.idx];
            bool hit;
            MapSlot *sl = find_slot(g.slot, nb, &hit);
            if ((e = slot_ready(sl, hit, s)) != hipSuccess) break;
            if (!hit) {
                for (size_t k = 0; k < g.conv_idx.size(); ++k) sl->args_pin[k] = conv_args(convs[g.conv_idx[k]], nb, rev);
                sl->mr = 4;
                while (sl->mr > 1 && direct_group_blocks(g, nb, nullptr, sl->mr) < 512) sl->mr >>= 1;
                sl->nblocks = direct_group_blocks(g, nb, &g.map_host, sl->mr);
                if (sl->nblocks > g.map_capacity) {
                    e = hipErrorInvalidValue;
                    break;
                }
                memcpy(sl->pin, g.map_host.data(), (size_t)sl->nblocks * sizeof(int2));
                e = hipMemcpyAsync(sl->args_dev, sl->args_pin, g.conv_idx.size() * sizeof(ConvArgs), hipMemcpyHostToDevice, s);
                if (e == hipSuccess)
                    e = hipMemcpyAsync(sl->dev, sl->pin, (size_t)sl->nblocks * sizeof(int2), hipMemcpyHostToDevice, s);
                if (e == hipSuccess) e = hipEventRecord(sl->landed, s);
                if (e != hipSuccess) break;
                sl->nb = nb;
                ++map_builds;
            }
            {
                int wl = direct_wlds && is16() ? 1 : 0;
                if (wl)
                    for (int ci : g.conv_idx)
                        if (conv_xl(convs[ci])) wl = 2;
                e = launch_conv_group(dtype, sl->args_dev, sl->dev, sl->nblocks, g.nr, sl->mr, wl, s);
            }
            break;
        }
        case OP_S2_GROUP: {
            S2Group &g = s2groups[op.idx];
            if (!s2_active(g, nb)) {
                for (const Op &f : g.fallback) {
                    e = exec_op(f, rev, images, nb, boxes, box_dtype, pts, heatmaps, s, flip, refine);
                    if (e != hipSuccess) break;
                }
                break;
            }
            bool hit;
            MapSlot *sl = find_slot(g.slot, nb, &hit);
            if ((e = slot_ready(sl, hit, s)) != hipSuccess) break;
            if (!hit) {
                sl->nblocks = s2_blocks(g, nb, &g.map_host);
                if (sl->nblocks > g.map_capacity) {
                    e = hipErrorInvalidValue;
                    break;
                }
                memcpy(sl->pin, g.map_host.data(), (size_t)sl->nblocks * sizeof(int2));
                e = hipMemcpyAsync(sl->dev, sl->pin, (size_t)sl->nblocks * sizeof(int2), hipMemcpyHostToDevice, s);
                if (e == hipSuccess) e = hipEventRecord(sl->landed, s);
                if (e != hipSuccess) break;
                sl->nb = nb;
                ++map_builds;
            }
            e = (dtype == HRN_F16 ? launch_conv_s2_f16 : launch_conv_s2)(s2probs_dev + g.prob_first, sl->dev, sl->nblocks, s);
            break;
        }
        case OP_CHAIN: {
            const Chain &ch = chains[op.idx];
            const ConvOp &c3 = convs[ch.conv3];
            const Tensor &to = tensors[c3.out_t];
            ChainArgs a;
            a.in = row0(c3.in_t), a.res = row0(c3.res_t), a.out_y = row0(c3.out_t);
            a.w3 = blob + c3.w_off, a.b3 = (const float *)(blob + c3.b_off);
            a.out_t = nullptr, a.w1 = nullptr, a.b1 = nullptr;
            if (ch.conv1 >= 0) {
                const ConvOp &c1 = convs[ch.conv1];
                a.out_t = row0(c1.out_t), a.w1 = blob + c1.w_off, a.b1 = (const float *)(blob + c1.b_off);
            }
            a.in3 = nullptr, a.w2 = nullptr, a.b2 = nullptr;
            if (ch.conv2 >= 0) {
                const ConvOp &c2 = convs[ch.conv2];
                a.in3 = row0(c2.in_t), a.w2 = blob + c2.w_off, a.b2 = (const float *)(blob + c2.b_off);
                a.in = nullptr;
            }
            a.x = nullptr, a.wds = nullptr, a.bds = nullptr;
            if (ch.ds >= 0) {
                const ConvOp &cd = convs[ch.ds];
                a.x = row0(cd.in_t), a.wds = blob + cd.w_off, a.bds = (const float *)(blob + cd.b_off);
                a.res = nullptr;
            }
            a.m = nb * to.hpwp, a.h = to.h, a.w = to.w, a.wp = to.wp, a.hpwp = to.hpwp, a.rev = rev, a.max_blocks = chain_blocks;
            e = dtype == HRN_F16 ? launch_bottleneck_chain_f16(a, s) : launch_bottleneck_chain(a, s);
            break;
        }
        case OP_FUSE: {
            FuseGroupArgs ga;
            ga.nf = fuses[op.idx].group;
            for (int k = 0; k < ga.nf; ++k) {
                const FuseOp &f = fuses[op.idx + k];
                const Tensor &to = tensors[f.out_t];
                FuseArgs &a = ga.f[k];
                a.nterms = f.nterms;
                for (int i = 0; i < f.nterms; ++i) {
                    const Tensor &tt = tensors[f.term_t[i]];
                    a.t[i].ptr = row0(f.term_t[i]), a.t[i].shift = f.shift[i];
                    a.t[i].wp = tt.wp, a.t[i].hpwp = tt.hpwp;
                }
                for (int i = f.nterms; i < 4; ++i) a.t[i] = FuseTerm{nullptr, 0, 0, 0};
                a.out = row0(f.out_t), a.c = to.c, a.h = to.h, a.w = to.w, a.wp = to.wp, a.hpwp = to.hpwp;
                a.m = nb * to.hpwp, a.rev = rev;
            }
            e = ga.nf == 1 ? launch_fuse(dtype, ga.f[0], s) : launch_fuse_group(dtype, ga, s);
            break;
        }
        case OP_HEAD: {
            const Tensor &t = tensors[head_in_t];
            HeadArgs a;
            a.in = row0(head_in_t);
            a.wgt = (const float *)(blob + head_w_off), a.bias = (const float *)(blob + head_b_off);
            a.wimg = (is16() && !disable_head_mfma) ? (const void *)(blob + head_wp_off) : nullptr;
            a.heatmaps = heatmaps, a.part_val = part_val, a.part_idx = part_idx;
            a.n = nb, a.c = t.c, a.joints = joints, a.h = t.h, a.w = t.w, a.wp = t.wp, a.hpwp = t.hpwp;
            a.slabs = head_slabs_for(nb), a.slab_px = head_px_for(nb);
            e = launch_head(dtype, a, s);
            break;
        }
        case OP_DECODE: {
            if (!pts) break;
            const Tensor &t = tensors[head_in_t];
            DecodeArgs a{};
            a.part_val = part_val, a.part_idx = part_idx, a.heatmaps = heatmaps, a.boxes = boxes;
            a.box_is_float = box_dtype == HRN_BOX_F32, a.pts = pts;
            a.n = nb, a.joints = joints, a.h = t.h, a.w = t.w, a.slabs = head_slabs_for(nb), a.mode = refine;
            e = launch_decode(a, s);
            break;
        }
    }
        return e;
    }

    bool check_forward_args(const void *images, int n, const void *boxes, float *pts, float *heatmaps, bool outputs_optional = false) {
        if (refuse_plan_only()) return false;
        if (!weights_loaded) {
            err = "weights not loaded (call hrn_load_weights or hrn_adopt_weights)";
            return false;
        }
        if (n < 0 || (n > 0 && !images)) {
            err = "bad images / n";
            return false;
        }
        if (!pts && !heatmaps && !outputs_optional) {
            err = "both pts and heatmaps are NULL";
            return false;
        }
        if (pts && !boxes && n > 0) {
            err = "pts requested without boxes";
            return false;
        }
        return true;
    }
```

simple-hrnet_amd/csrc/ctx_types.h:

```cpp
#pragma once

using namespace hrn;

std::string g_create_error;

struct Tensor {
    int c = 0, h = 0, w = 0;
    int wp = 0, hp = 0, hpwp = 0;
    int buf = -1;
};

struct Buffer {
    int c, h, w;
    size_t lead_rows, rows, bytes;
    char *dev = nullptr;
    bool in_use = false;
};

enum OpKind { OP_STEM, OP_STEM7, OP_MAXPOOL, OP_CONV, OP_CONV3_GROUP, OP_CONV_GROUP, OP_S2_GROUP, OP_CHAIN, OP_FUSE, OP_HEAD, OP_DECODE };

struct ConvOp {
    std::string conv, bn;
    int in_t, out_t, res_t;
    int cin, cout, k, stride, relu;
    int kpad, kchunks, nr;
    int algo = 0;
    int up = 0;
    int ks = 0, slices = 0, ntiles = 0, nch = 0;
    bool n96 = false;
    int fuse_with = -1;
    bool fused_away = false;
    int64_t w_off = 0, w_bytes = 0, b_off = 0;
    bool compact = false;
    bool s2 = false;
    bool w2_image = false;
    int64_t w2_off = 0, w2_bytes = 0;
    double flops = 0;
};

constexpr int kMapSlots = 4;
struct MapSlot {
    int nb = -1;
    int nblocks = 0;
    int mr = 4;
    int2 *dev = nullptr, *pin = nullptr;
    ConvArgs *args_dev = nullptr, *args_pin = nullptr;
    hipEvent_t landed = nullptr;
    hipStream_t up_stream = nullptr;
    uint64_t stamp = 0;
};

struct Conv3Group {
    std::vector<int> conv_idx;
    std::vector<int> fused_prob;
    int prob_first = 0;
    int max_wp = 0;
    int64_t map_capacity = 0;
    MapSlot slot[kMapSlots];
    std::vector<int2> map_host;
};

struct DirectGroup {
    std::vector<int> conv_idx;
    int nr = 0;
    int64_t map_capacity = 0;
    MapSlot slot[kMapSlots];
    std::vector<int2> map_host;
};

struct Op {
    OpKind kind;
    int idx;
};

struct S2Group {
    struct Prob {
        int in_t;
        std::vector<std::pair<int, int>> parts;
        int rows = 1, tiles_per_image = 1;
    };
    std::vector<int> conv_idx;
    std::vector<Prob> probs;
    std::vector<Op> fallback;
    int prob_first = 0;
    int64_t map_capacity = 0;
    MapSlot slot[kMapSlots];
    std::vector<int2> map_host;
};

struct FuseOp {
    int term_t[4];
    int shift[4];
    int nterms;
    int out_t;
    std::string name;
    int group = 1;
};

struct TapPoint {
    std::string name;
    int tensor;
    int op;
    int conv;
};
struct TapReq {
    int op, tensor, crop0, ncrops, crop_step;
    float *dst;
};

inline void fast_div(int d, unsigned *magic, int *shift) {
    int l = 0;
    while ((1 << l) < d) ++l;
    *shift = 30 + l;
    *magic = (unsigned)((1ull << *shift) / (unsigned)d + 1);
}

inline int64_t align_up(int64_t x, int64_t a) { return (x + a - 1) / a * a; }

inline uint16_t f32_to_bf16_host(float f) {
    uint32_t u;
    memcpy(&u, &f, 4);
    u += 0x7fffu + ((u >> 16) & 1u);
    return (uint16_t)(u >> 16);
}

inline uint16_t f32_to_f16_host(float f) {
    uint32_t x;
    memcpy(&x, &f, 4);
    const uint16_t sign = (uint16_t)((x >> 16) & 0x8000u);
    const uint32_t ax = x & 0x7fffffffu;
    if (ax > 0x7f800000u) return sign | 0x7e00u;
    if (ax >= 0x477ff000u) return sign | 0x7c00u;
    if (ax >= 0x38800000u) {
        uint32_t m = ax - 0x38000000u;
        m += 0xfffu + ((m >> 13) & 1u);
        return sign | (uint16_t)(m >> 13);
    }
    float a;
    memcpy(&a, &ax, 4);
    return sign | (uint16_t)std::nearbyint(a * 16777216.0f);
}
```

simple-hrnet_amd/csrc/hrnet_mi355.cpp:

```cpp
#include "../../include/hrnet_mi355.h"

#include <hip/hip_runtime.h>

#include <algorithm>
#include <cmath>
#include <cstdio>
#include <cstdlib>
#include <cstring>
#include <map>
#include <memory>
#include <string>
#include <vector>

#include "assoc_math.h"
#include "letterbox_math.h"
#include "pose_nms_math.h"
#include "kernels.h"
#include "track_geometry.h"

namespace {
#include "ctx_types.h"
}

namespace {
thread_local std::string g_env_seen;
const char *env_sw(const char *name) {
    const char *v = hrn_env(name);
    if (v) {
        const std::string item = std::string(name) + "=" + v + ";";
        if (g_env_seen.find(item) == std::string::npos) g_env_seen += item;
    }
    return v;
}
}

struct hrn_ctx {
    std::string switches;
    int c, joints, H, W, dtype, max_batch, device;
    int model = 0;
    int head_c = 0;
    int pool_in_t = -1, pool_out_t = -1;
    bool plan_only;
    int esize;
    std::string err;
    bool is16() const { return dtype == HRN_BF16 || dtype == HRN_F16; }

    std::vector<Tensor> tensors;
    std::vector<Buffer> buffers;
    std::vector<ConvOp> convs;
    std::vector<FuseOp> fuses;
    std::vector<Conv3Group> groups;
    std::vector<DirectGroup> dgroups;
    std::vector<S2Group> s2groups;
    S2Problem *s2probs_dev = nullptr;
    struct Chain {
        int conv3, conv1, ds;
        int conv2 = -1;
    };
    std::vector<Chain> chains;
    std::vector<TapPoint> taps;
    Conv3Problem *probs_dev = nullptr;
    std::vector<Op> ops;
    int stem_out_t = -1, head_in_t = -1;
    int64_t stem_w_off = 0, stem_b_off = 0, stem_wp_off = 0, head_w_off = 0, head_b_off = 0, head_wp_off = 0;

    int64_t blob_bytes = 0;
    char *blob = nullptr;
    bool weights_loaded = false;

    bool disable_lds = env_sw("HRN_DISABLE_LDS") != nullptr;
    bool assoc_no_assign = env_sw("HRN_ASSOC_NO_ASSIGN") != nullptr;
    bool disable_group = env_sw("HRN_DISABLE_GROUP") != nullptr;
    bool disable_dgroup = env_sw("HRN_DISABLE_DGROUP") != nullptr;
    bool disable_chain = env_sw("HRN_DISABLE_CHAIN") != nullptr;
    bool small_tiles = env_sw("HRN_SMALL_TILES") ? atoi(env_sw("HRN_SMALL_TILES")) != 0 : true;
    int small_below = env_sw("HRN_SMALL_BELOW") ? atoi(env_sw("HRN_SMALL_BELOW")) : 384;
    int small_keep_above = env_sw("HRN_SMALL_KEEP") ? atoi(env_sw("HRN_SMALL_KEEP")) : 300;
    bool disable_chain_ds = env_sw("HRN_DISABLE_CHAIN_DS") != nullptr;
    int pre_mode = env_sw("HRN_PRE_MODE") ? atoi(env_sw("HRN_PRE_MODE")) : 1;
    int chain_blocks = env_sw("HRN_CHAIN_BLOCKS") ? atoi(env_sw("HRN_CHAIN_BLOCKS")) : 512;
    bool disable_chain3 = env_sw("HRN_DISABLE_CHAIN3") != nullptr;
    bool direct_wlds = !(env_sw("HRN_DIRECT_WLDS") && atoi(env_sw("HRN_DIRECT_WLDS")) == 0);
    bool direct_xlds = !(env_sw("HRN_DIRECT_XLDS") && atoi(env_sw("HRN_DIRECT_XLDS")) == 0);
    bool conv_xl(const ConvOp &cv) const {
        return direct_xlds && direct_wlds && is16() && cv.k == 3 && cv.stride == 2 && cv.cin % 32 == 0 && !cv.up && cv.res_t < 0 && cv.nr == 6 &&
               cv.kchunks >= 4;
    }
    bool disable_bbf = env_sw("HRN_BBF") && atoi(env_sw("HRN_BBF")) == 0;
    int bbf_tpb_div = env_sw("HRN_BBF_TPB_DIV") ? std::max(1, atoi(env_sw("HRN_BBF_TPB_DIV"))) : 3;
    double bbf_slide_cost = env_sw("HRN_BBF_SLIDE_COST") ? atof(env_sw("HRN_BBF_SLIDE_COST")) : 24600.0;
    int bbf_min_tiles = env_sw("HRN_BBF_MIN_TILES") ? atoi(env_sw("HRN_BBF_MIN_TILES")) : 1100;
    int dgroup_nr_mode = env_sw("HRN_DGROUP_NR") ? atoi(env_sw("HRN_DGROUP_NR")) : 1;
    bool disable_lds32 = env_sw("HRN_DISABLE_LDS32") != nullptr;
    bool disable_n96 = env_sw("HRN_DISABLE_N96") != nullptr;
    bool disable_fgroup = env_sw("HRN_DISABLE_FGROUP") != nullptr;
    bool disable_f32lds = env_sw("HRN_DISABLE_F32LDS") != nullptr;
    int f32_small_slices = env_sw("HRN_F32_SMALL_SLICES") ? atoi(env_sw("HRN_F32_SMALL_SLICES")) : 0;
    std::vector<Conv3Problem> probs_host;
    bool disable_compact = env_sw("HRN_DISABLE_COMPACT") != nullptr;
    double compact_min_pad = env_sw("HRN_COMPACT_MIN_PAD") ? atof(env_sw("HRN_COMPACT_MIN_PAD")) : 0.08;
    bool disable_s2 = env_sw("HRN_DISABLE_S2") != nullptr;
    int s2_min_tiles = env_sw("HRN_S2_MIN_TILES") ? atoi(env_sw("HRN_S2_MIN_TILES")) : 256;
    int s2_target_blocks = env_sw("HRN_S2_BLOCKS") ? std::max(1, atoi(env_sw("HRN_S2_BLOCKS"))) : 256;
    bool disable_stem_mfma = env_sw("HRN_DISABLE_STEM_MFMA") != nullptr;
    bool disable_stem_fuse = env_sw("HRN_DISABLE_STEM_FUSE") != nullptr;
    bool stem_fuse = false;
    int stem_conv2_op = -1;
    S2Group stemf;
    bool disable_head_mfma = env_sw("HRN_DISABLE_HEAD_MFMA") != nullptr;
    bool direct_nr6 = env_sw("HRN_DIRECT_NR6") ? atoi(env_sw("HRN_DIRECT_NR6")) != 0 : true;
    int half_stages_per_block = env_sw("HRN_HALF_STAGES") ? atoi(env_sw("HRN_HALF_STAGES")) : 8;
    bool alternate = env_sw("HRN_ALTERNATE") ? atoi(env_sw("HRN_ALTERNATE")) != 0 : true;
    int block_order = env_sw("HRN_BLOCK_ORDER") ? atoi(env_sw("HRN_BLOCK_ORDER")) : 1;
    int long_factor = env_sw("HRN_LONG_FACTOR") ? atoi(env_sw("HRN_LONG_FACTOR")) : 4;
    double long_share = env_sw("HRN_LONG_SHARE") ? atof(env_sw("HRN_LONG_SHARE")) : 0.85;
    int head_slabs = 1, head_slab_px = 1024;
    static constexpr int kHeadSlabPxSmall = 256;
    int head_slabs_small = 1;
    int head_px_for(int nb) const { return (long)nb * head_slabs >= 192 ? head_slab_px : kHeadSlabPxSmall; }
    int head_slabs_for(int nb) const { return (long)nb * head_slabs >= 192 ? head_slabs : head_slabs_small; }
    float *part_val = nullptr;
    int *part_idx = nullptr;
    uint64_t map_clock = 0;
    int64_t map_builds = 0;
    float *scratch_hm = nullptr;
    float *scratch_heatmaps() {
        if (!scratch_hm && !hip_ok(hipMalloc((void **)&scratch_hm, (size_t)max_batch * joints * (H / 4) * (W / 4) * sizeof(float)),
                                   "hipMalloc(scratch heat-maps)"))
            scratch_hm = nullptr;
        return scratch_hm;
    }
    int64_t workspace_bytes = 0;

#include "ctx_plan.inc"
#include "ctx_memory.inc"
#include "ctx_weights.inc"
#include "ctx_run.inc"
#include "ctx_scratch.inc"
};

namespace {
using CallScope = hrn_ctx::CallScope;

template <class Pass>
int each_micro_batch(hrn_ctx *h, int n, bool scratch, hipStream_t s, const Pass &pass) {
    if (!h->hip_ok(hipSetDevice(h->device), "hipSetDevice")) return 6;
    if (n == 0) return 0;
    if (scratch && !h->scratch_heatmaps()) return 6;
    CallScope scope(h, &h->pass, s);
    if (!scope.entered) return 6;
    for (int off = 0; off < n; off += h->max_batch)
        if (!pass(off, std::min(n - off, h->max_batch))) return 8;
    return scope.leave() ? 0 : 6;
}

bool valid_refine(hrn_ctx *h, int refine) {
    if (refine == HRN_REFINE_NONE || refine == HRN_REFINE_QUARTER || refine == HRN_REFINE_DARK) return true;
    h->err = "refine must be HRN_REFINE_NONE, HRN_REFINE_QUARTER or HRN_REFINE_DARK";
    return false;
}

const char *bgr_frame_fault(const hrn_frame &f) { return !f.data || f.height <= 0 || f.width <= 0 ? "is null or has no size" : nullptr; }

template <class Frame>
bool frame_table_fault(hrn_handle h, const char *entry, int variant, int n, int nframes, int det_stride, bool pointers, const int32_t *fidx,
                       const Frame *frames, const char *(*frame_fault)(const Frame &)) {
    const std::string name = entry;
    std::string why;
    if (variant != HRN_CROP_PAD && variant != HRN_CROP_CLAMP) why = "variant must be HRN_CROP_PAD or HRN_CROP_CLAMP";
    else if (n < 0 || nframes < 0 || det_stride < 4 || (n > 0 && (nframes < 1 || !pointers))) why = "bad frames / detections / n";
    else if (n > 0 && !fidx && nframes != 1) why = name + ": without frame_index there must be one frame";
    for (int i = 0; why.empty() && i < n; ++i) {
        const long f = fidx ? (long)fidx[i] : 0;
        if (f < 0 || f >= nframes)
            why = name + ": frame_index " + std::to_string(f) + " of person " + std::to_string(i) + " is outside [0, " + std::to_string(nframes) + ")";
        else if (const char *fault = frame_fault(frames[f]))
            why = name + ": frame " + std::to_string(f) + ", which person " + std::to_string(i) + " is cut from, " + fault;
    }
// ... 1102 lines not shown
        h->err = maps ? "hrn_score_heatmaps: target maps come with target_weight and without visibility / joints_weight"
                      : "hrn_score_heatmaps: joints come with visibility and without target_weight";
        return 7;
    }
    if (!std::isfinite(pck_thr)) {
        h->err = "hrn_score_heatmaps: pck_thr is not finite";
        return 7;
    }
    if (ohkm_topk > h->joints) {
        h->err = "hrn_score_heatmaps: ohkm_topk " + std::to_string(ohkm_topk) + " exceeds the " + std::to_string(h->joints) + " joints";
        return 7;
    }
    if (!out_dev || !out_dev->loss_mse || !out_dev->loss_ohkm || !out_dev->avg_acc || !out_dev->cnt || !out_dev->acc ||
        (n > 0 && (!out_dev->dists || !out_dev->map_loss || !out_dev->preds || !out_dev->target_preds || !out_dev->maxvals))) {
        h->err = "hrn_score_heatmaps: every field of hrn_score_out must point to device memory (the per-person ones unless n is 0)";
        return 7;
    }
    if (!h->hip_ok(hipSetDevice(h->device), "hipSetDevice")) return 6;
    const int64_t count = (int64_t)n * h->joints;
    unsigned ring = 0;
    ScoreJoint *recs = (ScoreJoint *)h->pre_stage((size_t)std::max<int64_t>(count, 1) * sizeof(ScoreJoint), &ring);
    if (!recs) return 6;
    ScoreArgs a{};
    if (analytic) {
        const std::string bad = target_centers(joints_host, vis_host, joints_weight_host, n, h->joints, h->H, h->W, sigma, nullptr, nullptr,
                                               nullptr, recs);
        if (!bad.empty()) {
            h->err = "hrn_score_heatmaps: " + bad;
            return 7;
        }
        a.t = (int)(3.0 * sigma);
        a.table = h->score_table(a.t, sigma);
        if (!a.table) return 6;
    } else {
        for (int64_t k = 0; k < count; ++k) recs[k] = ScoreJoint{0, 0, target_weight_host[k], 0};
    }
    hipStream_t s = (hipStream_t)stream;
    const size_t bytes = (size_t)count * sizeof(ScoreJoint);
    if (!h->score_joints.reserve(h, bytes, (size_t)std::max<int64_t>(count, 256 * 17) * sizeof(ScoreJoint), "hipMalloc(score records)")) return 6;
    CallScope scope(h, &h->score_joints, s);
    if (!scope.entered || (count > 0 && !h->pre_upload(ring, s, {{h->score_joints.ptr, recs, bytes, "hipMemcpyAsync(score records)"}}))) return 6;
    a.heatmaps = heatmaps_dev, a.targets = targets_dev, a.joints = h->score_joints.as<ScoreJoint>();
    a.n = n, a.J = h->joints, a.h = h->H / 4, a.w = h->W / 4;
    a.map_loss = out_dev->map_loss, a.preds = out_dev->preds, a.target_preds = out_dev->target_preds, a.maxvals = out_dev->maxvals;
    a.loss_mse = out_dev->loss_mse, a.loss_ohkm = out_dev->loss_ohkm, a.avg_acc = out_dev->avg_acc, a.acc = out_dev->acc;
    a.dists = out_dev->dists, a.cnt = out_dev->cnt, a.pck_thr = pck_thr, a.ohkm_topk = ohkm_topk;
    if (!h->hip_ok(launch_score(a, s), "score launch")) return 8;
    return scope.leave() ? 0 : 6;
}

int hrn_tap_count(hrn_handle h) { return h ? (int)h->taps.size() : 0; }

int hrn_get_tap_info(hrn_handle h, int index, hrn_tap_info *out) {
    if (!h || !out || index < 0 || index >= (int)h->taps.size()) return 1;
    const TapPoint &tp = h->taps[index];
    const Tensor &t = h->tensors[tp.tensor];
    memset(out, 0, sizeof *out);
    snprintf(out->name, sizeof out->name, "%s", tp.name.c_str());
    out->c = t.c, out->h = t.h, out->w = t.w, out->conv_index = tp.conv;
    return 0;
}

int hrn_forward_tap(hrn_handle h, const void *images_dev, int n, const char *tap_name, int crop0, int ncrops, int crop_step,
                    float *dst_dev, float *heatmaps_dev, void *stream) {
    if (!h) return 1;
    if (!h->check_forward_args(images_dev, n, nullptr, nullptr, nullptr, true)) return 7;
    if (!tap_name || !dst_dev || n < 1 || n > h->max_batch || crop0 < 0 || ncrops < 1 || crop_step < 1 ||
        (int64_t)crop0 + (int64_t)(ncrops - 1) * crop_step >= n) {
        h->err = "hrn_forward_tap: needs a tap name, a destination, 1 <= n <= max_batch and crops crop0, crop0 + step, ... inside the call";
        return 7;
    }
    const TapPoint *tp = nullptr;
    for (const TapPoint &t : h->taps)
        if (t.name == tap_name) tp = &t;
    if (!tp) {
        h->err = std::string("hrn_forward_tap: no tensor named '") + tap_name + "' is written by this plan";
        return 7;
    }
    if (tp->conv >= 0 && h->fused_now(h->convs[tp->conv], n)) {
        h->err = std::string("hrn_forward_tap: '") + tap_name + "' stays in LDS at this batch size (fused BasicBlock pass); tap the block's conv2";
        return 7;
    }
    if (!h->hip_ok(hipSetDevice(h->device), "hipSetDevice")) return 6;
    const TapReq req{tp->op, tp->tensor, crop0, ncrops, crop_step, dst_dev};
    CallScope scope(h, &h->pass, (hipStream_t)stream);
    if (!scope.entered) return 6;
    if (!h->run_pass((const float *)images_dev, n, nullptr, 0, nullptr, heatmaps_dev, (hipStream_t)stream, nullptr, 0, &req)) return 8;
    return scope.leave() ? 0 : 6;
}

int hrn_conv_count(hrn_handle h) { return h ? (int)h->convs.size() : 0; }

int hrn_get_conv_info(hrn_handle h, int index, hrn_conv_info *out) {
    if (!h || !out || index < 0 || index >= (int)h->convs.size()) return 1;
    const ConvOp &cv = h->convs[index];
    memset(out, 0, sizeof *out);
    snprintf(out->name, sizeof out->name, "%s", cv.conv.c_str());
    out->cin = cv.cin, out->cout = cv.cout, out->ksize = cv.k, out->stride = cv.stride, out->relu = cv.relu;
    out->has_residual = cv.res_t >= 0;
    out->in_h = h->tensors[cv.in_t].h, out->in_w = h->tensors[cv.in_t].w;
    out->out_h = h->tensors[cv.out_t].h, out->out_w = h->tensors[cv.out_t].w;
    out->kpad = cv.kpad, out->nr = cv.nr, out->algo = cv.fuse_with >= 0 || cv.fused_away ? 2 : cv.n96 ? 3 : cv.s2 ? 4 : cv.algo, out->ks = cv.ks;
    out->w_offset = cv.w_off, out->w_bytes = cv.w_bytes, out->b_offset = cv.b_off;
    out->flops = cv.flops;
    return 0;
}

double hrn_flops_per_crop(hrn_handle h) {
    if (!h) return 0;
    double f = 2.0 * 64 * (h->model == 1 ? 147 : 27) * (h->H / 2) * (double)(h->W / 2);
    for (auto &cv : h->convs) f += cv.flops;
    f += 2.0 * h->joints * h->head_c * (h->H / 4) * (double)(h->W / 4);
    return f;
}

int64_t hrn_workspace_bytes(hrn_handle h) { return h ? h->workspace_bytes : 0; }
int64_t hrn_map_rebuilds(hrn_handle h) { return h ? h->map_builds : -1; }
int hrn_launches_per_pass(hrn_handle h) { return h ? (int)h->ops.size() - (h->stem_fuse ? 1 : 0) : 0; }
int hrn_stem_fused(hrn_handle h) { return h && h->stem_fuse ? 1 : 0; }
int hrn_conv_compact(hrn_handle h, int index) { return h && index >= 0 && index < (int)h->convs.size() && h->convs[index].compact ? 1 : 0; }
const char *hrn_switches(hrn_handle h) { return h ? h->switches.c_str() : ""; }

int64_t hrn_debug_pad_violations(hrn_handle h) {
    if (!h || h->plan_only) return -1;
    if (!h->hip_ok(hipSetDevice(h->device), "hipSetDevice")) return -1;
    unsigned long long *cnt = nullptr, host = 0;
    if (!h->hip_ok(hipMalloc((void **)&cnt, sizeof *cnt), "hipMalloc") || !h->hip_ok(hipMemset(cnt, 0, sizeof *cnt), "hipMemset")) return -1;
    bool ok = h->hip_ok(hipDeviceSynchronize(), "hipDeviceSynchronize");
    for (const Buffer &b : h->buffers) {
        if (!ok) break;
        PadCheckArgs a;
        a.buf = b.dev, a.count = cnt, a.rows = (long)b.rows, a.lead_rows = (long)b.lead_rows;
        a.c = b.c, a.h = b.h, a.w = b.w, a.wp = b.w + 1, a.hpwp = (b.h + 1) * (b.w + 1), a.nmax = h->max_batch;
        ok = h->hip_ok(launch_pad_check(h->dtype, a, nullptr), "pad check launch");
    }
    ok = ok && h->hip_ok(hipMemcpy(&host, cnt, sizeof host, hipMemcpyDeviceToHost), "hipMemcpy");
    (void)hipFree(cnt);
    return ok ? (int64_t)host : -1;
}

int hrn_plan_block_map(hrn_handle h, int group, int n, int reverse, int32_t *blocks, int capacity, int32_t *members, int member_capacity) {
    if (!h || n <= 0 || n > h->max_batch) return -1;
    if (group < 0 || group >= (int)h->groups.size()) return -1;
    const Conv3Group &g = h->groups[group];
    std::vector<int2> map;
    std::vector<int> px;
    const int nblocks = h->group_blocks(g, n, &map, reverse != 0, false, &px);
    for (int i = 0; i < nblocks && i < capacity; ++i) {
        const int x = map[i].x, y = map[i].y;
        int32_t *o = blocks + (size_t)i * 6;
        o[0] = x & 0xff, o[1] = (x >> 8) & 0xff, o[2] = x >> 16, o[3] = y & 0x1fffffff, o[4] = px[i],
        o[5] = ((y >> 29) & 1) | (((y >> 30) & 1) << 1);
    }
    int nm = 0;
    for (size_t k = 0; k < g.conv_idx.size(); ++k, ++nm)
        if (nm < member_capacity) members[nm] = g.conv_idx[k];
    for (size_t k = 0; k < g.conv_idx.size(); ++k)
        if (g.fused_prob[k] >= 0) {
            if (g.fused_prob[k] < member_capacity) members[g.fused_prob[k]] = g.conv_idx[k] | (1 << 30);
            ++nm;
        }
    return nblocks;
}

int hrn_plan_direct_map(hrn_handle h, int group, int n, int32_t *blocks, int capacity, int32_t *members, int member_capacity,
                        int32_t *pixels_per_tile) {
    if (!h || n <= 0 || n > h->max_batch) return -1;
    if (group < 0 || group >= (int)h->dgroups.size()) return -1;
    const DirectGroup &g = h->dgroups[group];
    int mr = 4;
    while (mr > 1 && h->direct_group_blocks(g, n, nullptr, mr) < 512) mr >>= 1;
    std::vector<int2> map;
    const int nblocks = h->direct_group_blocks(g, n, &map, mr);
    for (int i = 0; i < nblocks && i < capacity; ++i)
        blocks[(size_t)i * 3] = map[i].x & 0xff, blocks[(size_t)i * 3 + 1] = map[i].x >> 8, blocks[(size_t)i * 3 + 2] = map[i].y;
    for (size_t k = 0; k < g.conv_idx.size() && (int)k < member_capacity; ++k) members[k] = g.conv_idx[k];
    if (pixels_per_tile) *pixels_per_tile = 64 * mr;
    return nblocks;
}

int hrn_plan_s2_map(hrn_handle h, int group, int n, int32_t *blocks, int capacity, int32_t *parts, int part_capacity, int32_t *active) {
    if (!h || n <= 0 || n > h->max_batch) return -1;
    if (group == -1 && !h->stem_fuse) return -1;
    if (group < -1 || group >= (int)h->s2groups.size()) return -1;
    const S2Group &g = group == -1 ? h->stemf : h->s2groups[group];
    std::vector<int2> map;
    const int nblocks = h->s2_blocks(g, n, &map);
    for (int i = 0; i < nblocks && i < capacity; ++i)
        blocks[(size_t)i * 3] = map[i].x & 0xff, blocks[(size_t)i * 3 + 1] = map[i].x >> 8, blocks[(size_t)i * 3 + 2] = map[i].y;
    int np = 0;
    for (size_t k = 0; k < g.probs.size(); ++k)
        for (auto &pt : g.probs[k].parts) {
            if (np < part_capacity) {
                int32_t *o = parts + (size_t)np * 5;
                o[0] = (int32_t)k, o[1] = pt.first, o[2] = pt.second, o[3] = g.probs[k].rows, o[4] = g.probs[k].tiles_per_image;
            }
            ++np;
        }
    if (active) *active = h->s2_active(g, n) ? 1 : 0;
    return nblocks | (np << 20);
}

// ... 73 lines not shown
```

simple-hrnet_amd/csrc/kernels.h:

```cpp
#pragma once
#include <hip/hip_runtime.h>
#include <stdint.h>

#include <atomic>
#include <cstdlib>
#include <cstring>

namespace hrn {

inline hipError_t set_dynamic_lds(const void *func, int bytes, std::atomic<unsigned long long> &done) {
    int dev = 0;
    hipError_t e = hipGetDevice(&dev);
    if (e != hipSuccess) return e;
    const unsigned long long bit = 1ull << (dev & 63);
    if (done.load(std::memory_order_acquire) & bit) return hipSuccess;
    e = hipFuncSetAttribute(func, hipFuncAttributeMaxDynamicSharedMemorySize, bytes);
    if (e == hipSuccess) done.fetch_or(bit, std::memory_order_release);
    return e;
}

inline const char *hrn_env(const char *name) {
    static const bool debug = [] {
        const char *v = getenv("HRN_DEBUG_ENV");
        return v && *v && strcmp(v, "0") != 0;
    }();
    return debug ? getenv(name) : nullptr;
}

enum { DT_F32 = 0, DT_BF16 = 1, DT_F16 = 2 };

struct ConvArgs {
    const void *in;
    void *out;
    const void *w;
    const float *bias;
    const void *res;
    int cin, cout;
    int in_wp, in_hpwp;
    int out_h, out_w, out_wp, out_hpwp;
    int m;
    int ksize, stride, relu;
    int kchunks;
    int rev;
    int pre_mode;
    int wlds;
    int xlds;
    int up, up_a, up_b, up_wp, up_hpwp;
    int taps[4];
};

struct Conv3Problem {
    const void *in;
    void *out;
    const void *w;
    const float *bias;
    const void *res;
    int cin, cout;
    int h, wd, wp, hpwp;
    int relu;
    int slices;
    int ntiles;
    int tiles_per_block;
    int bm;
    unsigned magic_hpwp, magic_wp;
    int shift_hpwp, shift_wp;
    const void *w2;
    const float *bias2;
    int n96;
    int compact, hw;
    unsigned magic_hw, magic_w;
    int shift_hw, shift_w;
    int slab_rows, slab_rows_small;
};
int conv3x3_n96_ch64();
int conv3x3_lds_bbf_ok(int wp);
int conv3x3_n96_max_rows();
int conv3x3_lds_bm(int ks, int nrb, int wp);
int conv3x3_f32_bm(int wp);
hipError_t launch_conv3x3_f32(const Conv3Problem *probs_dev, const void *blockmap_dev, int nblocks, int nb, int nrb, hipStream_t s);

constexpr int kS2SlabBytes = 79872;
constexpr int s2_frags_per_part(int cin) { return cin == 48 ? 3 : 2; }
constexpr int s2_subslot_bytes(int cin) { return cin % 48 == 0 ? 96 : 32; }
constexpr int s2_region_bytes(int cin) { return kS2SlabBytes / (cin * 2 / s2_subslot_bytes(cin)) / 1024 * 1024; }
constexpr int s2_slot_capacity(int cin) { return s2_region_bytes(cin) / s2_subslot_bytes(cin); }
constexpr int s2_pair_pad(int wop) { return (8 - (3 * wop) % 8) % 8; }
constexpr int s2_pair_pitch(int wop) { return 4 * wop + s2_pair_pad(wop); }
constexpr int kS2MaxParts = 8;
struct S2Part {
    const void *w;
    const float *bias;
    void *out;
    int cout, ch0;
    int relu, pad_;
};
struct S2Problem {
    const void *in;
    int cin;
    int in_wp, in_hpwp;
    int ho, wo, wop, out_hpwp;
    int rows;
    int tiles_per_image;
    int nparts;
    unsigned char wave_part[8], wave_f0[8], wave_fs[8];
    unsigned magic_wop;
    int shift_wop;
    S2Part part[kS2MaxParts];
};
hipError_t launch_conv_s2(const S2Problem *probs_dev, const void *map_dev, int nblocks, hipStream_t s);
hipError_t launch_conv_s2_f16(const S2Problem *probs_dev, const void *map_dev, int nblocks, hipStream_t s);

constexpr int kStemFuseRegionBytes = 15360;
constexpr int kStemFusePatchBytes = 12544;
int stem_fused_fits(int wop, int w_in);

struct ChainArgs {
    const void *in;
    const void *res;
    void *out_y;
    void *out_t;
    const void *w3;
    const float *b3;
    const void *w1;
    const float *b1;
    const void *in3;
    const void *w2;
    const float *b2;
    const void *x;
    const void *wds;
    const float *bds;
    int m, h, w, wp, hpwp;
    int rev;
    int max_blocks;
};
hipError_t launch_bottleneck_chain(const ChainArgs &a, hipStream_t s);
hipError_t launch_bottleneck_chain_f16(const ChainArgs &a, hipStream_t s);

struct StemArgs {
    const float *images;
    void *out;
    const float *w;
    const float *bias;
    const void *wp;
    int n, H, W;
    int out_h, out_w, out_wp, out_hpwp;
    int flip;
};

hipError_t launch_stem_fused(int dtype, const S2Problem *probs_dev, const void *map_dev, int nblocks, const StemArgs &stem, hipStream_t s);

struct CropParams {
    int x1, y1, w_crop, h_crop;
    int pad_top, pad_left;
    int h_pad, w_pad;
    long long tmp_off;
    const unsigned char *frame;
    int frame_w, frame_h;
};
hipError_t launch_prepath(const CropParams *crops_dev, int n, int max_h_pad, unsigned char *tmp_dev, float *images_dev, int H, int W,
                          hipStream_t s);
struct YuvSource {
    const unsigned char *y, *u, *v;
    int pitch_y, pitch_c;
    int format;
    int coef[6];
    int pad_;
};
hipError_t launch_prepath_yuv(const CropParams *crops_dev, const YuvSource *src_dev, int n, int max_h_pad, unsigned char *tmp_dev,
                              float *images_dev, int H, int W, hipStream_t s);
hipError_t launch_yuv_to_bgr(const YuvSource &src, int height, int width, unsigned char *bgr_dev, hipStream_t s);
struct ResizeTaps {
    int ofs;
    short c[4];
};
inline double resize_scale(int dst, int src) { return 1.0 / ((double)dst / (double)src); }
hipError_t launch_resize_frames(const unsigned char *frames_dev, int n, int src_h, int src_w, int interp, ResizeTaps *taps_dev,
                                float *images_dev, int H, int W, hipStream_t s);
struct WarpParams {
    double m[6];
    int frame;
    int pad_;
};
hipError_t launch_warp_crops(const unsigned char *frames_dev, int frame_h, int frame_w, const WarpParams *params_dev, int n,
                             float *images_dev, int H, int W, hipStream_t s);

struct Stem7Args {
    const float *images;
    void *out;
    const float *w;
    const float *bias;
    const void *wp;
    int n, H, W;
    int out_h, out_w, out_wp, out_hpwp;
    int flip;
};
struct PoolArgs {
    const void *in;
    void *out;
    int c, n;
    int in_wp, in_hpwp;
    int out_h, out_w, out_wp, out_hpwp;
};
hipError_t launch_stem7(int dtype, const Stem7Args &a, hipStream_t s);
hipError_t launch_maxpool(int dtype, const PoolArgs &a, hipStream_t s);

struct FuseTerm {
    const void *ptr;
    int shift;
    int wp, hpwp;
};
struct FuseArgs {
    FuseTerm t[4];
    int nterms;
    void *out;
    int c, h, w, wp, hpwp;
    int m;
    int rev;
};

struct FuseGroupArgs {
    FuseArgs f[4];
    int nf;
    int block_end[4];
};
hipError_t launch_fuse_group(int dtype, FuseGroupArgs &g, hipStream_t s);

constexpr int kMaxJoints = 256;
struct HeadArgs {
    const void *in;
    const float *wgt;
    const void *wimg;
    const float *bias;
    float *heatmaps;
    float *part_val;
    int *part_idx;
    int n, c, joints, h, w, wp, hpwp, slabs, slab_px;
};

enum { RF_NONE = 0, RF_QUARTER = 1, RF_DARK = 2 };
struct DecodeArgs {
    const float *part_val;
    const int *part_idx;
    const void *boxes;
    int box_is_float;
    float *pts;
    int n, joints, h, w, slabs, mode;
    const float *heatmaps;
    float *coords;
};
hipError_t launch_decode(const DecodeArgs &a, hipStream_t s);
hipError_t launch_refine_coords(const DecodeArgs &a, hipStream_t s);

struct TtaArgs {
    float *hm;
    const float *hm_flipped;
    float *preds;
    float *maxvals;
    int pair[kMaxJoints];
    int n, joints, h, w, post_processing;
};
hipError_t launch_tta_decode(const TtaArgs &a, hipStream_t s);

struct ScoreJoint {
    int mu_x, mu_y;
    float weight;
    int draw;
};
struct ScoreArgs {
    const float *heatmaps;
    const float *targets;
    const ScoreJoint *joints;
    const float *table;
    int t;
    int n, J, h, w;
    double *map_loss;
    float *preds, *target_preds;
    float *maxvals;
    double *loss_mse, *loss_ohkm;
    float *avg_acc, *acc, *dists;
    int *cnt;
    float pck_thr;
    int ohkm_topk;
};
hipError_t launch_score(const ScoreArgs &a, hipStream_t s);
hipError_t launch_targets(const ScoreArgs &a, float *targets_out, hipStream_t s);

constexpr int kDrawTile = 32;
constexpr int kDrawMaxBones = 65535;
struct DrawFrame {
    unsigned char *p0, *p1, *p2;
    int height, width, pitch0, pitch1;
    int format;
    int radius;
// ... 48 lines not shown

struct AssocProblem {
    int cur0, n, prev0, m;
    long long scratch;
};
struct AssocArgs {
    int P, J;
    int no_assign;
    AssocProblem one;
    const AssocProblem *table;
    int *boxes;
    float *pts;
    const int *prev_boxes;
    const float *prev_pts;
    const int *prev_ids;
    int *next_id;
    double pose_alpha, similarity_threshold, smoothing_alpha;
    int *ids, *match, *status;
    char *scratch;
};
hipError_t launch_assoc(const AssocArgs &a, hipStream_t s);
hipError_t launch_bone_ids(const int *ids, int n, const unsigned *palette, int Cb, unsigned *bone, hipStream_t s);

struct PoseNmsProblem {
    int first, n;
};
struct PoseNmsArgs {
    int P, J, flags;
    PoseNmsProblem one;
    const PoseNmsProblem *table;
    void *kpts;
    void *areas;
    const void *scores;
    const double *sigmas;
    double thresh, in_vis_thre, rescore_thre;
    int *keep, *num;
    double *scores_out;
    int *suppressor, *status;
};
hipError_t launch_pose_nms(const PoseNmsArgs &a, hipStream_t s);

enum { LB_MODE_LINEAR = 0, LB_MODE_COPY = 1, LB_MODE_AREA = 2 };
struct LetterboxFrame {
    const unsigned char *bgr;
    YuvSource yuv;
    int src_h, src_w, new_h, new_w, top, left, mode, pad_;
    double scale_x, scale_y;
};
struct LetterboxArgs {
    int n, out_h, out_w, form, order, yuv;
    unsigned char pad[4];
    LetterboxFrame one;
    const LetterboxFrame *table;
    void *out;
};
hipError_t launch_letterbox(const LetterboxArgs &a, hipStream_t s);
struct DetFrame;
struct DetFilter;
struct DetArgs {
    int P, compact;
    const DetFrame *table;
    const float *dets;
    float *out;
    int *counts, *status;
};
hipError_t launch_detections_to_frame(const DetArgs &a, const DetFrame &one, const DetFilter &q, hipStream_t s);

struct TapArgs {
    const void *in;
    float *dst;
    int c, h, w, wp, hpwp, crop0, ncrops, crop_step;
};
hipError_t launch_tap(int dtype, const TapArgs &a, hipStream_t s);

struct PadCheckArgs {
    const void *buf;
    unsigned long long *count;
    long rows, lead_rows;
    int c, h, w, wp, hpwp, nmax;
};
hipError_t launch_pad_check(int dtype, const PadCheckArgs &a, hipStream_t s);

hipError_t launch_conv(int dtype, const ConvArgs &a, int nr, hipStream_t s);
hipError_t launch_conv_group(int dtype, const ConvArgs *probs_dev, const void *map_dev, int nblocks, int nr, int mr, int wlds,
                             hipStream_t s);
hipError_t launch_conv3x3_lds(const Conv3Problem *probs_dev, const void *blockmap_dev, int nblocks, int nb, int ks,
                              int nrb, hipStream_t s);
hipError_t launch_conv3x3_lds_f16(const Conv3Problem *probs_dev, const void *blockmap_dev, int nblocks, int nb, int ks,
                                  int nrb, hipStream_t s);
hipError_t launch_stem(int dtype, const StemArgs &a, hipStream_t s);
hipError_t launch_fuse(int dtype, const FuseArgs &a, hipStream_t s);
hipError_t launch_head(int dtype, const HeadArgs &a, hipStream_t s);

constexpr int kConvBlockRows = 704;

}
```

simple-hrnet_amd/csrc/kernels.hip:

```cpp
#include "kernels.h"
#include "argmax.h"
#include "dt16.h"
#include <stdlib.h>

namespace hrn {

typedef __attribute__((ext_vector_type(8))) __bf16 bf16x8;
typedef __attribute__((ext_vector_type(8))) short s16x8;
typedef __attribute__((ext_vector_type(4))) short s16x4;
typedef __attribute__((ext_vector_type(4))) float f32x4;

__device__ __forceinline__ float bf16_to_f32(unsigned short h) { return __uint_as_float(((unsigned)h) << 16); }
__device__ __forceinline__ unsigned short f32_to_bf16(float f) {
    unsigned u = __float_as_uint(f);
    u += 0x7fffu + ((u >> 16) & 1u);
    return (unsigned short)(u >> 16);
}

constexpr bool is16(int dt) { return dt != DT_F32; }

template <int DT>
struct Tr;
template <>
struct Tr<DT_BF16> {
    using elem = unsigned short;
    using vec = s16x8;
    using out4 = s16x4;
    static constexpr int KC = 32, VEC = 8;
    static __device__ __forceinline__ float ld(elem e) { return bf16_to_f32(e); }
    static __device__ __forceinline__ elem st(float f) { return f32_to_bf16(f); }
};
template <>
struct Tr<DT_F16> {
    using elem = unsigned short;
    using vec = s16x8;
    using out4 = s16x4;
    static constexpr int KC = 32, VEC = 8;
    static __device__ __forceinline__ float ld(elem e) { return H16<DT_F16>::ld(e); }
    static __device__ __forceinline__ elem st(float f) { return H16<DT_F16>::st(f); }
};
template <>
struct Tr<DT_F32> {
    using elem = float;
    using vec = f32x4;
    using out4 = f32x4;
    static constexpr int KC = 16, VEC = 4;
    static __device__ __forceinline__ float ld(elem e) { return e; }
    static __device__ __forceinline__ elem st(float f) { return f; }
};

template <int DT>
__device__ __forceinline__ f32x4 mma(typename Tr<DT>::vec w, typename Tr<DT>::vec x, f32x4 acc);
template <>
__device__ __forceinline__ f32x4 mma<DT_BF16>(s16x8 w, s16x8 x, f32x4 acc) {
    return __builtin_amdgcn_mfma_f32_16x16x32_bf16(__builtin_bit_cast(bf16x8, w), __builtin_bit_cast(bf16x8, x), acc, 0,
                                                   0, 0);
}
template <>
__device__ __forceinline__ f32x4 mma<DT_F16>(s16x8 w, s16x8 x, f32x4 acc) {
    return H16<DT_F16>::mma(w, x, acc);
}
template <>
__device__ __forceinline__ f32x4 mma<DT_F32>(f32x4 w, f32x4 x, f32x4 acc) {
#pragma unroll
    for (int t = 0; t < 4; ++t) acc = __builtin_amdgcn_mfma_f32_16x16x4f32(w[t], x[t], acc, 0, 0, 0);
    return acc;
}

#define GLOBAL_AS __attribute__((address_space(1)))

#ifndef HRN_WL_G
#define HRN_WL_G 4
#endif
constexpr int WL_G = HRN_WL_G;
template <int DT, int NR, int MR, bool PRE>
__device__ __forceinline__ void conv_direct_epilogue(const ConvArgs &p, const int ng, const int m0, const int li, const int g,
                                                     f32x4 (&acc)[MR][NR], s16x8 (&rpre)[PRE ? MR : 1][PRE ? NR / 2 : 1]) {
    using T = Tr<DT>;
    using elem = typename T::elem;
    const int ch0 = ng * 16 * NR + g * 4 * NR;
    float bias[4 * NR];
#pragma unroll
    for (int c = 0; c < 4 * NR; ++c) bias[c] = ((const GLOBAL_AS float *)p.bias)[ch0 + c];
    GLOBAL_AS elem *__restrict__ out = (GLOBAL_AS elem *)p.out;
    const GLOBAL_AS elem *__restrict__ res = (const GLOBAL_AS elem *)p.res;
#pragma unroll
    for (int i = 0; i < MR; ++i) {
        const int q = m0 + i * 16 + li;
        if (q >= p.m) continue;
        const int rem = q % p.out_hpwp;
        const int ho = rem / p.out_wp, wo = rem - ho * p.out_wp;
        const bool ok = (ho < p.out_h) && (wo < p.out_w);
        size_t o = (size_t)q * p.cout + ch0;
        if (p.up) {
            if (!ok) continue;
            o = ((size_t)(q / p.out_hpwp) * p.up_hpwp + (size_t)(2 * ho + p.up_a) * p.up_wp + 2 * wo + p.up_b) * p.cout + ch0;
        }
        if constexpr (is16(DT) && (NR % 2 == 0)) {
#pragma unroll
            for (int j = 0; j < NR; j += 2) {
                s16x8 r8 = {};
                if constexpr (PRE)
                    r8 = rpre[i][j / 2];
                else if (res)
                    r8 = *(const GLOBAL_AS s16x8 *)(res + o + j * 4);
                s16x8 o8;
#pragma unroll
                for (int r = 0; r < 8; ++r) {
                    float v = acc[i][j + (r >> 2)][r & 3] + bias[j * 4 + r];
                    if (PRE || res) v += T::ld((elem)r8[r]);
                    if (p.relu) v = fmaxf(v, 0.f);
                    if (!ok) v = 0.f;
                    o8[r] = (short)T::st(v);
                }
                *(GLOBAL_AS s16x8 *)(out + o + j * 4) = o8;
            }
        } else {
#pragma unroll
            for (int j = 0; j < NR; ++j) {
                typename T::out4 r4 = {};
                if (res) r4 = *(const GLOBAL_AS typename T::out4 *)(res + o + j * 4);
                typename T::out4 o4;
#pragma unroll
                for (int r = 0; r < 4; ++r) {
                    float v = acc[i][j][r] + bias[j * 4 + r];
                    if (res) v += T::ld((elem)r4[r]);
                    if (p.relu) v = fmaxf(v, 0.f);
                    if (!ok) v = 0.f;
                    o4[r] = T::st(v);
                }
                *(GLOBAL_AS typename T::out4 *)(out + o + j * 4) = o4;
            }
        }
    }
}

template <int DT, int NR, int MR, bool PRE = false, bool WL = false>
__device__ __forceinline__ void conv_direct_body(const ConvArgs &p, const int ng, const int mtile_in, char *smem = nullptr) {
    using T = Tr<DT>;
    using vec = typename T::vec;
    using elem = typename T::elem;
    typedef const GLOBAL_AS vec *gvec_p;
    const int lane = threadIdx.x & 63, wave = __builtin_amdgcn_readfirstlane(threadIdx.x >> 6);
    const int li = lane & 15, g = lane >> 4;
    if (mtile_in * 64 * MR >= p.m) return;
    const int mtile = p.rev ? (p.m + 64 * MR - 1) / (64 * MR) - 1 - mtile_in : mtile_in;
    const int m0 = (mtile * 4 + wave) * (16 * MR);
    const GLOBAL_AS elem *__restrict__ in = (const GLOBAL_AS elem *)p.in;

    long inrow[MR];
#pragma unroll
    for (int i = 0; i < MR; ++i) {
        const int q = m0 + i * 16 + li;
        int r;
        if (q >= p.m) {
            r = 0;
        } else if (p.stride == 1) {
            r = q;
        } else {
            const int n = q / p.out_hpwp, rem = q - n * p.out_hpwp;
            const int ho = rem / p.out_wp, wo = rem - ho * p.out_wp;
            r = n * p.in_hpwp + 2 * ho * p.in_wp + 2 * wo;
        }
        inrow[i] = (long)r * p.cin;
    }

    f32x4 acc[MR][NR];
#pragma unroll
    for (int i = 0; i < MR; ++i)
#pragma unroll
        for (int j = 0; j < NR; ++j) acc[i][j] = f32x4{0.f, 0.f, 0.f, 0.f};

    s16x8 rpre[PRE ? MR : 1][PRE ? NR / 2 : 1];
    if constexpr (PRE) {
        const GLOBAL_AS elem *__restrict__ res = (const GLOBAL_AS elem *)p.res;
#pragma unroll
        for (int i = 0; i < MR; ++i)
#pragma unroll
            for (int j = 0; j < NR; j += 2)
                rpre[i][j / 2] = *(const GLOBAL_AS s16x8 *)(res + (size_t)(m0 + i * 16 + li) * p.cout +
                                                            ng * 16 * NR + g * 4 * NR + j * 4);
    }

    int ci = g * T::VEC, tap = 0;
    while (ci >= p.cin) {
        ci -= p.cin;
        ++tap;
    }
    const int ntaps = p.ksize * p.ksize;
    const GLOBAL_AS char *__restrict__ wlane =
        (const GLOBAL_AS char *)p.w + ((size_t)ng * NR * p.kchunks * 64 + lane) * 16;

    auto stage = [&](int gi) {
        const GLOBAL_AS char *wsrc = (const GLOBAL_AS char *)p.w + (size_t)ng * NR * p.kchunks * 1024;
#pragma unroll
        for (int t0 = 0; t0 < NR * WL_G; t0 += 4) {
            const int t = t0 + wave;
            const int j = t / WL_G, c = gi * WL_G + (t - j * WL_G);
            if (t < NR * WL_G && c < p.kchunks)
                __builtin_amdgcn_global_load_lds(wsrc + ((size_t)(j * p.kchunks + c) * 64 + lane) * 16,
                                                 (__attribute__((address_space(3))) void *)(smem + ((gi & 1) * NR * WL_G + t) * 1024), 16, 0, 0);
        }
    };
    if constexpr (WL) stage(0);
    constexpr int KU = (is16(DT) && !WL && !PRE) ? (MR == 1 ? 4 : MR == 2 ? 2 : 1) : 1;
    if constexpr (KU > 1) {
        for (int kc0 = 0; kc0 < p.kchunks; kc0 += KU) {
            vec b[KU][NR], a[KU][MR];
#pragma unroll
            for (int u = 0; u < KU; ++u) {
                const int kc = kc0 + u;
                if (kc < p.kchunks) {
#pragma unroll
                    for (int j = 0; j < NR; ++j) b[u][j] = *(gvec_p)(wlane + ((size_t)j * p.kchunks + kc) * 1024);
                    if (tap < ntaps) {
                        int tapoff = 0;
                        if (p.ksize == 3) {
                            const int dh = (tap * 11) >> 5, dw = tap - dh * 3;
                            tapoff = (dh - 1) * p.in_wp + (dw - 1);
                        } else if (p.ksize == 2) {
                            tapoff = tap == 0 ? p.taps[0] : tap == 1 ? p.taps[1] : tap == 2 ? p.taps[2] : p.taps[3];
                        }
                        const long aoff = (long)tapoff * p.cin + ci;
#pragma unroll
                        for (int i = 0; i < MR; ++i) a[u][i] = *(gvec_p)(in + inrow[i] + aoff);
                    } else {
#pragma unroll
                        for (int i = 0; i < MR; ++i) a[u][i] = vec{};
                    }
                    ci += T::KC;
                    while (ci >= p.cin) {
                        ci -= p.cin;
                        ++tap;
                    }
                }
            }
#pragma unroll
            for (int u = 0; u < KU; ++u)
                if (kc0 + u < p.kchunks) {
#pragma unroll
                    for (int i = 0; i < MR; ++i)
#pragma unroll
                        for (int j = 0; j < NR; ++j) acc[i][j] = mma<DT>(b[u][j], a[u][i], acc[i][j]);
                }
        }
    } else
    for (int kc = 0; kc < p.kchunks; ++kc) {
        vec b[NR];
        if constexpr (WL) {
            const int gi = kc / WL_G, c = kc - gi * WL_G;
            if (c == 0) {
                asm volatile("s_waitcnt vmcnt(0)" ::: "memory");
                __syncthreads();
                if ((gi + 1) * WL_G < p.kchunks) stage(gi + 1);
            }
            const char *wl = smem + ((gi & 1) * NR * WL_G + c) * 1024 + lane * 16;
#pragma unroll
            for (int j = 0; j < NR; ++j) b[j] = *(const vec *)(wl + j * WL_G * 1024);
        } else {
#pragma unroll
            for (int j = 0; j < NR; ++j) b[j] = *(gvec_p)(wlane + ((size_t)j * p.kchunks + kc) * 1024);
        }
        vec a[MR];
        if (tap < ntaps) {
            int tapoff = 0;
            if (p.ksize == 3) {
                const int dh = (tap * 11) >> 5, dw = tap - dh * 3;
                tapoff = (dh - 1) * p.in_wp + (dw - 1);
            } else if (p.ksize == 2) {
                tapoff = tap == 0 ? p.taps[0] : tap == 1 ? p.taps[1] : tap == 2 ? p.taps[2] : p.taps[3];
            }
            const long aoff = (long)tapoff * p.cin + ci;
#pragma unroll
            for (int i = 0; i < MR; ++i) a[i] = *(gvec_p)(in + inrow[i] + aoff);
        } else {
#pragma unroll
            for (int i = 0; i < MR; ++i) a[i] = vec{};
        }
#pragma unroll
        for (int i = 0; i < MR; ++i)
#pragma unroll
            for (int j = 0; j < NR; ++j) acc[i][j] = mma<DT>(b[j], a[i], acc[i][j]);
        ci += T::KC;
        while (ci >= p.cin) {
            ci -= p.cin;
            ++tap;
        }
    }

    conv_direct_epilogue<DT, NR, MR, PRE>(p, ng, m0, li, g, acc, rpre);
}

constexpr int XL_G = 2, XL_D = 3;
constexpr int xl_lds_bytes(int nr) { return 2 * XL_G * nr * 1024 + 4 * XL_D * 4 * 1024; }
__device__ __forceinline__ bool conv_xl_ok(const ConvArgs &p) {
    return p.stride == 2 && p.ksize == 3 && (p.cin & 31) == 0 && !p.up && !p.res && p.kchunks >= 2 * XL_G;
}
__device__ __forceinline__ void xl_glds(const GLOBAL_AS char *base, unsigned voff, unsigned lds_dst) {
    asm volatile("s_mov_b32 m0, %1\n\ts_nop 0\n\tglobal_load_lds_dwordx4 %0, %2" ::"v"(voff), "s"(lds_dst), "s"(base) : "memory", "m0");
}
template <int DT, int NR>
__device__ __forceinline__ void conv_direct_xl_body(const ConvArgs &p, const int ng, const int mtile_in, char *smem) {
    constexpr int MR = 4;
    const int lane = threadIdx.x & 63, wave = __builtin_amdgcn_readfirstlane(threadIdx.x >> 6);
    const int li = lane & 15, g = lane >> 4;
    if (mtile_in * 64 * MR >= p.m) return;
    const int mtile = p.rev ? (p.m + 64 * MR - 1) / (64 * MR) - 1 - mtile_in : mtile_in;
    const int m0 = (mtile * 4 + wave) * (16 * MR);
    const int cin = p.cin, in_wp = p.in_wp, kchunks = p.kchunks;
    const int spt = cin >> 5;
    const int guard = (in_wp + 1) * cin;
    const GLOBAL_AS char *const base = (const GLOBAL_AS char *)p.in - (size_t)guard * 2;
    unsigned xoff[MR];
#pragma unroll
    for (int i = 0; i < MR; ++i) {
        const int q = m0 + i * 16 + li;
        int r = 0;
        if (q < p.m) {
            const int n = q / p.out_hpwp, rem = q - n * p.out_hpwp;
            const int ho = rem / p.out_wp, wo = rem - ho * p.out_wp;
            r = n * p.in_hpwp + 2 * ho * in_wp + 2 * wo;
        }
        xoff[i] = ((unsigned)r * (unsigned)cin + (unsigned)(guard + g * 8)) * 2u;
    }
    const unsigned lds0 = (unsigned)(size_t)(__attribute__((address_space(3))) char *)smem;
    const unsigned xring = lds0 + 2 * XL_G * NR * 1024 + wave * (XL_D * MR * 1024);
    const GLOBAL_AS char *const wsrc = (const GLOBAL_AS char *)p.w + (size_t)ng * NR * kchunks * 1024;
    const unsigned lane16 = lane * 16;
    auto px_issue = [&](int kc) {
        const int slot = kc % XL_D;
        const int kq = kc < kchunks ? kc : kchunks - 1;
        const int tap = kq / spt, sl = kq - tap * spt;
        const int dh = (tap * 11) >> 5, dw = tap - dh * 3;
        const GLOBAL_AS char *sb = base + ((long)((dh - 1) * in_wp + (dw - 1)) * cin + sl * 32) * 2;
#pragma unroll
        for (int i = 0; i < MR; ++i) xl_glds(sb, xoff[i], xring + (slot * MR + i) * 1024);
    };
    auto w_issue = [&](int gi) {
#pragma unroll
        for (int u = 0; u < (NR * XL_G + 3) / 4; ++u) {
            int t = wave + 4 * u;
            if (t >= NR * XL_G) t = NR * XL_G - 1;
            const int j = t / XL_G;
            int c = gi * XL_G + (t - j * XL_G);
            if (c >= kchunks) c = kchunks - 1;
            xl_glds(wsrc + (size_t)(j * kchunks + c) * 1024, lane16, lds0 + ((gi & 1) * NR * XL_G + t) * 1024);
        }
    };
    static_assert((NR * XL_G) % 4 == 0, "weight pieces per wave");
    constexpr int WOPS = NR * XL_G / 4;
    f32x4 acc[MR][NR];
#pragma unroll
    for (int i = 0; i < MR; ++i)
#pragma unroll
        for (int j = 0; j < NR; ++j) acc[i][j] = f32x4{0.f, 0.f, 0.f, 0.f};
    w_issue(0);
    px_issue(0);
    px_issue(1);
    for (int kc = 0; kc < kchunks; ++kc) {
        const int gi = kc / XL_G, c = kc - gi * XL_G;
        if (c == 0) {
            asm volatile("s_waitcnt vmcnt(%0)" ::"i"((XL_D - 1) * MR) : "memory");
            __builtin_amdgcn_s_barrier();
            w_issue(gi + 1);
        }
        px_issue(kc + XL_D - 1);
        asm volatile("s_waitcnt vmcnt(%0)" ::"i"((XL_D - 1) * MR + WOPS) : "memory");
        s16x8 a[MR], b[NR];
        const unsigned xa = xring + (kc % XL_D) * (MR * 1024) + lane16;
        const unsigned wa = lds0 + ((gi & 1) * NR * XL_G + c) * 1024 + lane16;
#pragma unroll
        for (int i = 0; i < MR; ++i) asm volatile("ds_read_b128 %0, %1 offset:%2" : "=v"(a[i]) : "v"(xa), "i"(i * 1024));
#pragma unroll
        for (int j = 0; j < NR; ++j) asm volatile("ds_read_b128 %0, %1 offset:%2" : "=v"(b[j]) : "v"(wa), "i"(j * XL_G * 1024));
        asm volatile("s_waitcnt lgkmcnt(0)" ::: "memory");
#pragma unroll
        for (int i = 0; i < MR; ++i)
#pragma unroll
            for (int j = 0; j < NR; ++j) acc[i][j] = mma<DT>(b[j], a[i], acc[i][j]);
    }
    asm volatile("s_waitcnt vmcnt(0)" ::: "memory");
    s16x8 rpre[1][1];
    conv_direct_epilogue<DT, NR, MR, false>(p, ng, m0, li, g, acc, rpre);
}

template <int DT, int NR, int MR, bool PRE, bool WL = false>
__global__ __launch_bounds__(256) void conv_direct_kernel(const ConvArgs p) {
    extern __shared__ __attribute__((aligned(16))) char smem_direct[];
    const int ngroups = p.cout / (16 * NR);
    const int ng = (blockIdx.x >> 3) % ngroups;
    const int mtile = (blockIdx.x / (8 * ngroups)) * 8 + (blockIdx.x & 7);
    if constexpr (WL && is16(DT) && NR == 6 && MR == 4 && !PRE) {
        if (p.xlds && conv_xl_ok(p)) {
            conv_direct_xl_body<DT, NR>(p, ng, mtile, smem_direct);
            return;
        }
    }
    conv_direct_body<DT, NR, MR, PRE, WL>(p, ng, mtile, smem_direct);
}

template <int DT, int NR, int MR, bool WL = false>
__global__ __launch_bounds__(256) void conv_direct_group_kernel(const ConvArgs *__restrict__ probs,
                                                                const int2 *__restrict__ map) {
    extern __shared__ __attribute__((aligned(16))) char smem_direct[];
    const int2 e = map[blockIdx.x];
    const int prob = __builtin_amdgcn_readfirstlane(e.x & 255), ng = __builtin_amdgcn_readfirstlane(e.x >> 8);
    const int mtile = __builtin_amdgcn_readfirstlane(e.y);
    const ConvArgs p = probs[prob];
    if constexpr (WL && is16(DT) && NR == 6 && MR == 4) {
        if (p.xlds && conv_xl_ok(p)) {
            conv_direct_xl_body<DT, NR>(p, ng, mtile, smem_direct);
            return;
        }
    }
    conv_direct_body<DT, NR, MR, false, WL>(p, ng, mtile, smem_direct);
}

template <int DT, int NR>
static constexpr int direct_lds_bytes(int wlds) {
    const int wl = 2 * WL_G * NR * 1024;
    if (is16(DT) && NR == 6 && wlds == 2) return wl > xl_lds_bytes(NR) ? wl : xl_lds_bytes(NR);
    return wl;
}

template <int DT, int NR>
static hipError_t launch_conv_group_t(const ConvArgs *probs, const int2 *map, int nblocks, int mr, int wlds, hipStream_t s) {
    if (mr == 1)
        hipLaunchKernelGGL((conv_direct_group_kernel<DT, NR, 1>), dim3(nblocks), dim3(256), 0, s, probs, map);
    else if (mr == 2)
        hipLaunchKernelGGL((conv_direct_group_kernel<DT, NR, 2>), dim3(nblocks), dim3(256), 0, s, probs, map);
    else if (is16(DT) && wlds)
    {
        const int lds = direct_lds_bytes<DT, NR>(wlds);
        static std::atomic<unsigned long long> lds_set{0};
        if (lds > 65536) {
            const hipError_t e = set_dynamic_lds((const void *)conv_direct_group_kernel<DT, NR, 4, is16(DT)>, direct_lds_bytes<DT, NR>(2), lds_set);
            if (e != hipSuccess) return e;
        }
        hipLaunchKernelGGL((conv_direct_group_kernel<DT, NR, 4, is16(DT)>), dim3(nblocks), dim3(256), lds, s, probs, map);
    }
    else
        hipLaunchKernelGGL((conv_direct_group_kernel<DT, NR, 4>), dim3(nblocks), dim3(256), 0, s, probs, map);
    return hipGetLastError();
}

hipError_t launch_conv_group(int dtype, const ConvArgs *probs_dev, const void *map_dev, int nblocks, int nr, int mr, int wlds,
                             hipStream_t s) {
    if (nblocks <= 0) return hipSuccess;
    const int2 *map = (const int2 *)map_dev;
    if (dtype == DT_BF16) {
        if (nr == 6) return launch_conv_group_t<DT_BF16, 6>(probs_dev, map, nblocks, mr, wlds, s);
        if (nr == 4) return launch_conv_group_t<DT_BF16, 4>(probs_dev, map, nblocks, mr, wlds, s);
        if (nr == 3) return launch_conv_group_t<DT_BF16, 3>(probs_dev, map, nblocks, mr, wlds, s);
        if (nr == 2) return launch_conv_group_t<DT_BF16, 2>(probs_dev, map, nblocks, mr, wlds, s);
    } else if (dtype == DT_F16) {
        if (nr == 6) return launch_conv_group_t<DT_F16, 6>(probs_dev, map, nblocks, mr, wlds, s);
        if (nr == 4) return launch_conv_group_t<DT_F16, 4>(probs_dev, map, nblocks, mr, wlds, s);
        if (nr == 3) return launch_conv_group_t<DT_F16, 3>(probs_dev, map, nblocks, mr, wlds, s);
        if (nr == 2) return launch_conv_group_t<DT_F16, 2>(probs_dev, map, nblocks, mr, wlds, s);
    } else {
        if (nr == 4) return launch_conv_group_t<DT_F32, 4>(probs_dev, map, nblocks, mr, wlds, s);
        if (nr == 3) return launch_conv_group_t<DT_F32, 3>(probs_dev, map, nblocks, mr, wlds, s);
        if (nr == 2) return launch_conv_group_t<DT_F32, 2>(probs_dev, map, nblocks, mr, wlds, s);
    }
    return hipErrorInvalidValue;
}

template <int DT, int NR, int MR, bool PRE>
static hipError_t launch_conv_tt(const ConvArgs &a, hipStream_t s) {
    const int mtiles = (a.m + 64 * MR - 1) / (64 * MR);
    dim3 grid(((mtiles + 7) / 8) * 8 * (a.cout / (16 * NR)));
    hipLaunchKernelGGL((conv_direct_kernel<DT, NR, MR, PRE>), grid, dim3(256), 0, s, a);
    return hipGetLastError();
}

template <int DT, int NR>
static hipError_t launch_conv_t(const ConvArgs &a, hipStream_t s) {
    if constexpr (is16(DT) && NR % 2 == 0) {
        const int pre_mode = a.pre_mode;
        if (a.res && a.ksize == 1 && pre_mode == 1) return launch_conv_tt<DT, NR, 4, true>(a, s);
        if (a.res && a.ksize == 1 && pre_mode == 2) return launch_conv_tt<DT, NR, 2, true>(a, s);
        if (a.res && a.ksize == 1 && pre_mode == 3) return launch_conv_tt<DT, NR, 2, false>(a, s);
    }
    const int ngroups = a.cout / (16 * NR);
    const long blocks4 = (long)((a.m + 255) / 256) * ngroups;
    if (blocks4 < 256) return launch_conv_tt<DT, NR, 1, false>(a, s);
    if (blocks4 < 512) return launch_conv_tt<DT, NR, 2, false>(a, s);
    if constexpr (is16(DT))
        if (a.wlds && a.kchunks >= 2 * WL_G) {
            const int mtiles = (a.m + 255) / 256;
            dim3 grid(((mtiles + 7) / 8) * 8 * (a.cout / (16 * NR)));
            const int lds = direct_lds_bytes<DT, NR>(a.xlds ? 2 : 1);
            static std::atomic<unsigned long long> lds_set{0};
            if (lds > 65536) {
                const hipError_t e = set_dynamic_lds((const void *)conv_direct_kernel<DT, NR, 4, false, true>, direct_lds_bytes<DT, NR>(2), lds_set);
                if (e != hipSuccess) return e;
            }
            hipLaunchKernelGGL((conv_direct_kernel<DT, NR, 4, false, true>), grid, dim3(256), lds, s, a);
            return hipGetLastError();
        }
    return launch_conv_tt<DT, NR, 4, false>(a, s);
}

hipError_t launch_conv(int dtype, const ConvArgs &a, int nr, hipStream_t s) {
    if (a.m <= 0) return hipSuccess;
    if (dtype == DT_BF16) {
        if (nr == 6) return launch_conv_t<DT_BF16, 6>(a, s);
        if (nr == 4) return launch_conv_t<DT_BF16, 4>(a, s);
        if (nr == 3) return launch_conv_t<DT_BF16, 3>(a, s);
        if (nr == 2) return launch_conv_t<DT_BF16, 2>(a, s);
    } else if (dtype == DT_F16) {
        if (nr == 6) return launch_conv_t<DT_F16, 6>(a, s);
        if (nr == 4) return launch_conv_t<DT_F16, 4>(a, s);
        if (nr == 3) return launch_conv_t<DT_F16, 3>(a, s);
        if (nr == 2) return launch_conv_t<DT_F16, 2>(a, s);
    } else {
        if (nr == 4) return launch_conv_t<DT_F32, 4>(a, s);
        if (nr == 3) return launch_conv_t<DT_F32, 3>(a, s);
        if (nr == 2) return launch_conv_t<DT_F32, 2>(a, s);
    }
    return hipErrorInvalidValue;
}

template <int DT>
__global__ __launch_bounds__(256) void stem_kernel(const StemArgs p) {
    using T = Tr<DT>;
    const int q = blockIdx.x * 256 + threadIdx.x;
    const int m = p.n * p.out_hpwp;
    if (q >= m) return;
    const int n = q / p.out_hpwp, rem = q - n * p.out_hpwp;
    const int ho = rem / p.out_wp, wo = rem - ho * p.out_wp;
    const bool ok = ho < p.out_h && wo < p.out_w;
    float x[27];
    const float *img = p.images + (size_t)n * 3 * p.H * p.W;
#pragma unroll
    for (int ci = 0; ci < 3; ++ci)
#pragma unroll
        for (int kh = 0; kh < 3; ++kh) {
            const int iy = 2 * ho + kh - 1;
#pragma unroll
            for (int kw = 0; kw < 3; ++kw) {
                const int ix = 2 * wo + kw - 1;
                float v = 0.f;
                if (ok && iy >= 0 && iy < p.H && ix >= 0 && ix < p.W)
                    v = img[((size_t)ci * p.H + iy) * p.W + (p.flip ? p.W - 1 - ix : ix)];
                x[ci * 9 + kh * 3 + kw] = v;
            }
        }
    typename T::elem *o = (typename T::elem *)p.out + (size_t)q * 64;
#pragma unroll
    for (int cg = 0; cg < 4; ++cg) {
        float acc[16];
#pragma unroll
        for (int c = 0; c < 16; ++c) acc[c] = p.bias[cg * 16 + c];
#pragma unroll
        for (int k = 0; k < 27; ++k) {
            const float *wk = p.w + k * 64 + cg * 16;
#pragma unroll
            for (int c = 0; c < 16; ++c) acc[c] = fmaf(x[k], wk[c], acc[c]);
        }
#pragma unroll
        for (int v = 0; v < 16 / T::VEC; ++v) {
            typename T::vec ov;
#pragma unroll
            for (int r = 0; r < T::VEC; ++r) {
                const float f = ok ? fmaxf(acc[v * T::VEC + r], 0.f) : 0.f;
                ov[r] = T::st(f);
            }
            *(typename T::vec *)(o + cg * 16 + v * T::VEC) = ov;
        }
    }
}

template <int DT>
__global__ __launch_bounds__(256) void stem7_kernel(const Stem7Args p) {
    using T = Tr<DT>;
    const int q = blockIdx.x * 256 + threadIdx.x;
    const int m = p.n * p.out_hpwp;
    if (q >= m) return;
    const int n = q / p.out_hpwp, rem = q - n * p.out_hpwp;
    const int ho = rem / p.out_wp, wo = rem - ho * p.out_wp;
    const bool ok = ho < p.out_h && wo < p.out_w;
    const float *img = p.images + (size_t)n * 3 * p.H * p.W;
    typename T::elem *o = (typename T::elem *)p.out + (size_t)q * 64;
    for (int cg = 0; cg < 4; ++cg) {
        float acc[16];
#pragma unroll
        for (int c = 0; c < 16; ++c) acc[c] = p.bias[cg * 16 + c];
// ... 602 lines not shown
```

simple-hrnet_amd/native.py:

```python
from __future__ import annotations

import contextlib
import ctypes
import math
from typing import Dict, List, Optional, Sequence, Tuple, Union

import numpy as np
import torch

from . import _lib
from .frames import (PIX_FORMATS, YUV_MATRICES, YUV_RANGES, Frames, YuvFrame, _check_frame, _frame_kind, as_tensor,
                     device_tensor, frame_stack, host_array, host_bytes)
from .palettes import bgr_to_yuv_colors, embedded_palette, find_palette

DTYPES = {"fp32": 0, "f32": 0, "float32": 0, torch.float32: 0, "bf16": 1, "bfloat16": 1, torch.bfloat16: 1,
          "fp16": 2, "f16": 2, "float16": 2, "half": 2, torch.float16: 2}
DTYPE_NAMES = {0: "fp32", 1: "bf16", 2: "fp16"}
REFINE_MODES = {None: 0, "quarter": 1, "dark": 2}


def refine_code(refine) -> int:
    if not (refine is None or isinstance(refine, str)) or refine not in REFINE_MODES:
        raise ValueError("refine must be None, 'quarter' or 'dark', got %r" % (refine,))
    return REFINE_MODES[refine]
# ... 953 lines not shown
            with pipe.filling(slot):
                for f, off in offs.items():
                    flat = host_bytes(frames[f])
                    arena[off:off + flat.numel()].copy_(flat, non_blocking=True)
            return frames.table({f: arena.data_ptr() + off for f, off in offs.items()}), first, len(frames), bool(offs)

        groups = group_frames(counts(), self.max_batch, per_pass)
        nxt = next(groups, None)
        pending = upload(0, nxt) if nxt is not None else None
        k, pieces = 0, {}
        while nxt is not None:
            slot, group, (table, first, nfr, busy) = k & 1, nxt, pending
            nxt = next(groups, None)
            pending = upload(slot ^ 1, nxt) if nxt is not None else None
            if busy:
                pipe.ready(slot)
                local = [(f - first, lo, hi) for f, lo, hi in group]
                dets = {f - first: held[f][1] for f, _, _ in group}
                for f, lo, hi, bx, pts, hm in self._run_group(table, nfr, dets, local, variant, return_heatmaps, refine):
                    if hi > lo:
                        pieces.setdefault(f + first, []).append((bx, pts, hm))
                pipe.release(slot)
            last = group[-1][0]
            for f in sorted({g[0] for g in group}):
                if f == last and nxt is not None and nxt[0][0] == f:
                    continue
                p = pieces.pop(f, None)
                del held[f]
                yield self._frame_result(p, return_heatmaps) if p else self._empty_result(return_heatmaps)
            k += 1

    def tap_infos(self) -> List[_lib.TapInfo]:
        out = []
        for i in range(self._lib.hrn_tap_count(self._h)):
            ti = _lib.TapInfo()
            rc = self._lib.hrn_get_tap_info(self._h, i, ctypes.byref(ti))
            self._check(rc, "hrn_get_tap_info")
            out.append(ti)
        return out

    def forward_tap(self, images: torch.Tensor, name: str, crop0: int = 0, ncrops: Optional[int] = None,
                    return_heatmaps: bool = False, crop_step: int = 1):
        x = self._images_ptr(images)
        n = x.shape[0]
        if ncrops is None:
            ncrops = (n - crop0 + crop_step - 1) // crop_step
        info = {t.name.decode(): t for t in self.tap_infos()}.get(name)
        if info is None:
            raise KeyError("no tensor named %r is written by this plan" % name)
        dst = torch.empty((ncrops, info.c, info.h, info.w), dtype=torch.float32, device=x.device)
        h, w = self.resolution
        hm = torch.empty((n, self.nof_joints, h // 4, w // 4), dtype=torch.float32, device=x.device) if return_heatmaps else None
        self._launch("hrn_forward_tap", x.data_ptr(), n, name.encode(), int(crop0), int(ncrops), int(crop_step), dst.data_ptr(),
                     hm.data_ptr() if hm is not None else None)
        return (dst, hm) if return_heatmaps else dst

    def conv_infos(self) -> List[_lib.ConvInfo]:
        out = []
        for i in range(self._lib.hrn_conv_count(self._h)):
            ci = _lib.ConvInfo()
            rc = self._lib.hrn_get_conv_info(self._h, i, ctypes.byref(ci))
            self._check(rc, "hrn_get_conv_info")
            out.append(ci)
        return out

    def flops_per_crop(self) -> float:
        return float(self._lib.hrn_flops_per_crop(self._h))

    def workspace_bytes(self) -> int:
        return int(self._lib.hrn_workspace_bytes(self._h))

    def map_rebuilds(self) -> int:
        return int(self._lib.hrn_map_rebuilds(self._h))

    def launches_per_pass(self) -> int:
        return int(self._lib.hrn_launches_per_pass(self._h))

    def conv_compact(self, index: int) -> bool:
        return bool(self._lib.hrn_conv_compact(self._h, index))

    def stem_fused(self) -> bool:
        return bool(self._lib.hrn_stem_fused(self._h))

    def pad_violations(self) -> int:
        return int(self._lib.hrn_debug_pad_violations(self._h))

    def switches(self) -> str:
        return self._lib.hrn_switches(self._h).decode()

    def profile_pass(self, images: torch.Tensor):
        x = self._images_ptr(images)
        n = min(x.shape[0], self.max_batch)
        nconv = self._lib.hrn_conv_count(self._h)
        conv_ms = (ctypes.c_float * nconv)()
        other = (ctypes.c_float * 4)()
        self._launch("hrn_profile_pass", x.data_ptr(), n, conv_ms, nconv, other)
        return list(conv_ms), dict(zip(("stem", "fuse", "head", "decode"), list(other)))


class MultiDeviceHRNet:

    def __init__(self, devices: Sequence[int], c: int = 48, nof_joints: int = 17, resolution: Tuple[int, int] = (384, 288),
                 dtype="bf16", max_batch: int = 32, model_name: str = "HRNet"):
        from concurrent.futures import ThreadPoolExecutor

        if len(devices) < 1:
            raise ValueError("at least one device")
        self.devices = [int(d) for d in devices]
        self.nets = [NativeHRNet(c, nof_joints, resolution, dtype, max_batch=max_batch, device=d, model_name=model_name)
                     for d in self.devices]
        self.streams = [torch.cuda.Stream(torch.device("cuda", d)) for d in self.devices]
        self.pool = ThreadPoolExecutor(max_workers=len(self.devices), thread_name_prefix="hrn-dev")
        first = self.nets[0]
        self.c, self.nof_joints, self.resolution = first.c, first.nof_joints, first.resolution
        self.dtype, self.max_batch, self.model_name = first.dtype, first.max_batch, first.model_name
        self.device_index = first.device_index

    @property
    def torch_device(self) -> torch.device:
        return self.nets[0].torch_device

    def eval(self):
        return self

    def to(self, *args, **kwargs):
        return self

    def close(self):
        for n in getattr(self, "nets", []):
            n.close()
        pool = getattr(self, "pool", None)
        if pool is not None:
            pool.shutdown(wait=True)
            self.pool = None

    def __del__(self):
        try:
            self.close()
        except Exception:
            pass

    def load_state_dict(self, state_dict: Dict) -> "MultiDeviceHRNet":
        self.nets[0].load_state_dict(state_dict)
        src = self.nets[0].weight_blob_tensor()
        for net in self.nets[1:]:
            net.weight_blob_tensor().copy_(src)
            torch.cuda.synchronize(net.torch_device)
            net.adopt_weights()
        torch.cuda.synchronize(self.torch_device)
        return self

    def load_checkpoint(self, path: str) -> "MultiDeviceHRNet":
        return self.load_state_dict(torch.load(path, map_location="cpu"))

    def adopt_from(self, src: "NativeHRNet") -> "MultiDeviceHRNet":
        blob = src.weight_blob_tensor()
        for net in self.nets:
            net.weight_blob_tensor().copy_(blob)
            torch.cuda.synchronize(net.torch_device)
            net.adopt_weights()
        return self

    def _ranges(self, n: int) -> List[Tuple[int, int]]:
        from .dist import shard_range

        return [shard_range(n, len(self.nets), k) for k in range(len(self.nets))]
# ... 102 lines not shown
```

Before: 10770 crops/s.

## Absorb HRNet fuse-layer sums into final stride-2 downsample conv epilogues

For 16-bit dtypes, the last stride-2 conv feeding each lower-resolution fuse output now adds the other fuse terms and writes the fused output directly in its epilogue. That fuse output then needs no separate fuse kernel pass. Stride-2 convs are rescheduled to run after the other fuse-branch convs, and a separate plain op list is kept for tap and debug paths. This cuts launches and one read-write of each absorbed fuse tensor, at the cost of extra terms loaded in the conv epilogue and more planning complexity.

```diff
diff --git a/include/hrnet_mi355.h b/include/hrnet_mi355.h
--- a/include/hrnet_mi355.h
+++ b/include/hrnet_mi355.h
@@ -223,6 +223,12 @@
 int64_t hrn_map_rebuilds(hrn_handle h);
 int hrn_launches_per_pass(hrn_handle h);
 int hrn_stem_fused(hrn_handle h);
+typedef struct {
+    char stage[96];
+    int32_t first_output, outputs;
+} hrn_fuse_launch_info;
+int hrn_fuse_launch_count(hrn_handle h, int unabsorbed);
+int hrn_get_fuse_launch_info(hrn_handle h, int unabsorbed, int index, hrn_fuse_launch_info *out);
 int hrn_conv_compact(hrn_handle h, int index);
 const char *hrn_switches(hrn_handle h);
 int64_t hrn_debug_pad_violations(hrn_handle h);
diff --git a/simple-hrnet_amd/_lib.py b/simple-hrnet_amd/_lib.py
--- a/simple-hrnet_amd/_lib.py
+++ b/simple-hrnet_amd/_lib.py
@@ -151,6 +151,10 @@
 class TapInfo(ctypes.Structure):
     _fields_ = [("name", ctypes.c_char * 96), ("c", ctypes.c_int32), ("h", ctypes.c_int32), ("w", ctypes.c_int32),
                 ("conv_index", ctypes.c_int32)]
+
+
+class FuseLaunchInfo(ctypes.Structure):
+    _fields_ = [("stage", ctypes.c_char * 96), ("first_output", ctypes.c_int32), ("outputs", ctypes.c_int32)]
 
 
 class ScoreOut(ctypes.Structure):
@@ -263,6 +267,8 @@
     "hrn_launches_per_pass": (ctypes.c_int, [_P]),
     "hrn_switches": (ctypes.c_char_p, [_P]),
     "hrn_stem_fused": (ctypes.c_int, [_P]),
+    "hrn_fuse_launch_count": (ctypes.c_int, [_P, ctypes.c_int]),
+    "hrn_get_fuse_launch_info": (ctypes.c_int, [_P, ctypes.c_int, ctypes.c_int, ctypes.POINTER(FuseLaunchInfo)]),
     "hrn_conv_compact": (ctypes.c_int, [_P, ctypes.c_int]),
     "hrn_debug_pad_violations": (ctypes.c_int64, [_P]),
     "hrn_plan_block_map": (ctypes.c_int, [_P, ctypes.c_int, ctypes.c_int, ctypes.c_int, _P, ctypes.c_int, _P, ctypes.c_int]),
diff --git a/simple-hrnet_amd/csrc/ctx_memory.inc b/simple-hrnet_amd/csrc/ctx_memory.inc
--- a/simple-hrnet_amd/csrc/ctx_memory.inc
+++ b/simple-hrnet_amd/csrc/ctx_memory.inc
@@ -151,7 +151,12 @@
 
     const Tensor &grid_of(const ConvOp &cv) const { return tensors[cv.up ? cv.in_t : cv.out_t]; }
 
-    ConvArgs conv_args(const ConvOp &cv, int nb, bool rev) const {
+    FuseTerm fuse_term(const FuseOp &f, int i) const {
+        const Tensor &tt = tensors[f.term_t[i]];
+        return FuseTerm{row0(f.term_t[i]), f.shift[i], tt.wp, tt.hpwp};
+    }
+
+    ConvArgs conv_args(const ConvOp &cv, int nb, bool rev, bool absorb = false) const {
         const Tensor &ti = tensors[cv.in_t], &to = grid_of(cv);
         ConvArgs a;
         a.in = row0(cv.in_t), a.out = row0(cv.out_t);
@@ -172,6 +177,19 @@
             const int dy = (t >> 1) - 1 + a.up_a, dx = (t & 1) - 1 + a.up_b;
             a.taps[t] = cv.up ? dy * ti.wp + dx : 0;
         }
+        a.fuse_n = 0, a.fuse_own = 0;
+        for (FuseTerm &ft : a.fuse_t) ft = FuseTerm{nullptr, 0, 0, 0};
+        if (absorb && cv.absorb_fuse >= 0) {
+            const FuseOp &f = fuses[cv.absorb_fuse];
+            a.out = row0(f.out_t);
+            a.fuse_n = f.nterms;
+            for (int i = 0; i < f.nterms; ++i) {
+                if (f.term_t[i] == cv.out_t)
+                    a.fuse_own = i;
+                else
+                    a.fuse_t[i] = fuse_term(f, i);
+            }
+        }
         return a;
     }
 
@@ -222,10 +240,11 @@
     bool setup_dgroups() {
         for (auto &g : dgroups) {
             g.map_capacity = std::max<int64_t>(direct_group_blocks(g, max_batch, nullptr), 4 * 512 + 64 * (int64_t)g.conv_idx.size() * 8);
-            for (MapSlot &sl : g.slot) {
-                if (!alloc_slot(sl, g.map_capacity, g.conv_idx.size())) return false;
-                workspace_bytes += g.map_capacity * (int64_t)sizeof(int2) + (int64_t)(g.conv_idx.size() * sizeof(ConvArgs));
-            }
+            for (int form = 0; form < (g.has_absorber ? 2 : 1); ++form)
+                for (MapSlot &sl : form ? g.slot_absorb : g.slot) {
+                    if (!alloc_slot(sl, g.map_capacity, g.conv_idx.size())) return false;
+                    workspace_bytes += g.map_capacity * (int64_t)sizeof(int2) + (int64_t)(g.conv_idx.size() * sizeof(ConvArgs));
+                }
         }
         return true;
     }
@@ -483,8 +502,10 @@
             for (MapSlot &sl : stemf.slot) free_slot(sl);
             for (auto &g : groups)
                 for (MapSlot &sl : g.slot) free_slot(sl);
-            for (auto &g : dgroups)
+            for (auto &g : dgroups) {
                 for (MapSlot &sl : g.slot) free_slot(sl);
+                for (MapSlot &sl : g.slot_absorb) free_slot(sl);
+            }
         }
         blob = nullptr;
     }
diff --git a/simple-hrnet_amd/csrc/ctx_plan.inc b/simple-hrnet_amd/csrc/ctx_plan.inc
--- a/simple-hrnet_amd/csrc/ctx_plan.inc
+++ b/simple-hrnet_amd/csrc/ctx_plan.inc
@@ -90,11 +90,12 @@
 
     static int c3_family(const ConvOp &cv) { return ((cv.ks == 48 && cv.nr == 3) || cv.n96) ? 0 : cv.ks * 16 + cv.nr; }
 
-    void emit_direct(const std::vector<int> &idx, std::vector<Op> &dst) {
+    void emit_direct(const std::vector<int> &idx, std::vector<Op> &dst, bool absorb = false) {
         std::vector<std::vector<int>> dsets;
+        auto single = [&](int i) { dst.push_back({OP_CONV, i, absorb && convs[i].absorb_fuse >= 0 ? 1 : 0}); };
         for (int i : idx) {
             if (disable_dgroup) {
-                dst.push_back({OP_CONV, i});
+                single(i);
                 continue;
             }
             bool placed = false;
@@ -108,13 +109,14 @@
         }
         for (auto &set : dsets) {
             if (set.size() == 1) {
-                dst.push_back({OP_CONV, set[0]});
+                single(set[0]);
                 continue;
             }
             DirectGroup g;
             g.conv_idx = set, g.nr = convs[set[0]].nr;
+            for (int i : set) g.has_absorber |= absorb && convs[i].absorb_fuse >= 0;
             dgroups.push_back(g);
-            dst.push_back({OP_CONV_GROUP, (int)dgroups.size() - 1});
+            dst.push_back({OP_CONV_GROUP, (int)dgroups.size() - 1, g.has_absorber ? 1 : 0});
         }
     }
 
@@ -222,8 +224,10 @@
         }
         std::vector<std::vector<int>> term(nout, std::vector<int>(nb, -1));
         std::vector<std::vector<int>> cur(nout, std::vector<int>(nb, -1));
+        std::vector<std::vector<int>> made(nb);
+        std::vector<std::vector<int>> last_of(nout, std::vector<int>(nb, -1)), level_of(nout, std::vector<int>(nb, -1));
+        std::vector<int> dead;
         for (int level = 0; level < nb; ++level) {
-            std::vector<int> made, dead;
             for (int j = 0; j < nb; ++j) {
                 std::vector<int> c1, c2;
                 if (level == 0)
@@ -237,7 +241,7 @@
                     const std::string q = buf;
                     if (i < j && level == 0) {
                         term[i][j] = add_conv(q + ".0", q + ".1", xs[j], c << i, 1, 1, 0, -1, false, nr1);
-                        made.push_back((int)convs.size() - 1);
+                        made[level].push_back((int)convs.size() - 1);
                     } else if (i > j && level < i - j) {
                         const bool last = (level == i - j - 1);
                         snprintf(buf, sizeof buf, "%s.%d", q.c_str(), level);
@@ -245,16 +249,13 @@
                         const int src = level == 0 ? xs[j] : cur[i][j];
                         const int nt = add_conv(qq + ".0", qq + ".1", src, last ? (c << i) : (c << j), 3, 2, last ? 0 : 1, -1,
                                                 false, level == 0 ? nr2 : 0);
-                        made.push_back((int)convs.size() - 1);
+                        made[level].push_back((int)convs.size() - 1);
                         if (level > 0) dead.push_back(src);
                         cur[i][j] = nt;
-                        if (last) term[i][j] = nt;
+                        if (last) term[i][j] = nt, last_of[i][j] = (int)convs.size() - 1, level_of[i][j] = level;
                     }
                 }
             }
-            if (made.empty()) break;
-            emit_convs(made);
-            for (int t : dead) release(t);
         }
         std::vector<int> outs;
         for (int i = 0; i < nout; ++i) {
@@ -265,14 +266,65 @@
             }
             snprintf(buf, sizeof buf, "%s.fuse.%d", name.c_str(), i);
             outs.push_back(add_fuse(terms, shifts, buf));
+            fuses.back().out_index = i;
+        }
+        const int first = (int)fuses.size() - nout;
+        auto generic_s2 = [&](int ci) { return convs[ci].algo == 0 && !convs[ci].s2 && convs[ci].k == 3 && convs[ci].stride == 2; };
+        bool absorbing = false;
+        if (is16() && !disable_fuse_absorb) {
+            for (int i = 1; i < nout; ++i) {
+                int best = -1;
+                for (int j = 0; j < i && j < nb; ++j)
+                    if (last_of[i][j] >= 0 && generic_s2(last_of[i][j]) && (best < 0 || level_of[i][j] > level_of[i][best])) best = j;
+                if (best >= 0 && convs[last_of[i][best]].nr != 6 && convs[last_of[i][best]].nr != 4) best = -1;
+                if (best >= 0) convs[last_of[i][best]].absorb_fuse = first + i, absorbing = true;
+            }
+            for (int level = 1; level < nb && absorbing; ++level)
+                for (int ci : made[level])
+                    if (!generic_s2(ci))
+                        for (int cj : made[level - 1])
+                            if (convs[cj].out_t == convs[ci].in_t && generic_s2(cj)) absorbing = false;
+            if (!absorbing)
+                for (auto &lv : made)
+                    for (int ci : lv) convs[ci].absorb_fuse = -1;
+        }
+        const size_t seg_begin = ops.size();
+        std::vector<Op> plain;
+        for (int level = 0; level < nb; ++level) {
+            if (made[level].empty()) break;
+            std::vector<int> now;
+            for (int ci : made[level])
+                if (!(absorbing && generic_s2(ci))) now.push_back(ci);
+            emit_convs(now);
+        }
+        plain.assign(ops.begin() + seg_begin, ops.end());
+        for (int level = 0; level < nb && absorbing; ++level) {
+            std::vector<int> moved;
+            for (int ci : made[level])
+                if (generic_s2(ci)) moved.push_back(ci);
+            const size_t at = ops.size();
+            emit_direct(moved, ops, true);
+            for (size_t k = at; k < ops.size(); ++k) plain.push_back({ops[k].kind, ops[k].idx, 0});
         }
         {
-            const int first = (int)fuses.size() - nout;
+            std::vector<bool> absorbed(nout, false);
+            for (auto &lv : made)
+                for (int ci : lv)
+                    if (convs[ci].absorb_fuse >= 0) absorbed[convs[ci].absorb_fuse - first] = true;
             for (int i = 0; i < nout; ++i) {
                 fuses[first + i].group = disable_fgroup ? 1 : (i == 0 ? nout : 0);
-                if (fuses[first + i].group) ops.push_back({OP_FUSE, first + i});
-            }
-        }
+                if (fuses[first + i].group) plain.push_back({OP_FUSE, first + i});
+            }
+            for (int i = 0; i < nout; ++i) {
+                if (absorbed[i]) continue;
+                int run = 1;
+                while (!disable_fgroup && i + run < nout && !absorbed[i + run]) ++run;
+                ops.push_back({OP_FUSE, first + i, absorbing ? run : 0});
+                i += run - 1;
+            }
+        }
+        if (absorbing) plain_segs.push_back({seg_begin, ops.size(), plain});
+        for (int t : dead) release(t);
         for (int i = 0; i < nout; ++i)
             for (int j = 0; j < nb; ++j)
                 if (i != j) release(term[i][j]);
@@ -429,48 +481,74 @@
         head_in_t = xs[0];
         ops.push_back({OP_HEAD, 0});
         ops.push_back({OP_DECODE, 0});
+        build_plain_list();
 
         layout_blob();
+    }
+
+    void build_plain_list() {
+        ops_plain.clear();
+        if (plain_segs.empty()) return;
+        size_t at = 0;
+        for (const PlainSeg &sg : plain_segs) {
+            ops_plain.insert(ops_plain.end(), ops.begin() + at, ops.begin() + sg.begin);
+            ops_plain.insert(ops_plain.end(), sg.plain.begin(), sg.plain.end());
+            at = sg.end;
+        }
+        ops_plain.insert(ops_plain.end(), ops.begin() + at, ops.end());
     }
 
     void index_taps() {
         taps.clear();
-        auto add = [&](const std::string &name, int tensor, int op, int conv) {
-            for (TapPoint &t : taps)
-                if (t.name == name) {
-                    t.op = op;
-                    return;
-                }
-            taps.push_back(TapPoint{name, tensor, op, conv});
-        };
-        for (size_t oi = 0; oi < ops.size(); ++oi) {
-            const Op &op = ops[oi];
-            switch (op.kind) {
-                case OP_STEM:
-                case OP_STEM7: add("stem", stem_out_t, (int)oi, -1); break;
-                case OP_MAXPOOL: add("maxpool", pool_out_t, (int)oi, -1); break;
-                case OP_CONV: add(convs[op.idx].conv, convs[op.idx].out_t, (int)oi, op.idx); break;
-                case OP_CONV3_GROUP:
-                    for (int ci : groups[op.idx].conv_idx) add(convs[ci].conv, convs[ci].out_t, (int)oi, ci);
-                    break;
-                case OP_CONV_GROUP:
-                    for (int ci : dgroups[op.idx].conv_idx) add(convs[ci].conv, convs[ci].out_t, (int)oi, ci);
-                    break;
-                case OP_S2_GROUP:
-                    for (int ci : s2groups[op.idx].conv_idx) add(convs[ci].conv, convs[ci].out_t, (int)oi, ci);
-                    break;
-                case OP_CHAIN:
-                    add(convs[chains[op.idx].conv3].conv, convs[chains[op.idx].conv3].out_t, (int)oi, chains[op.idx].conv3);
-                    if (chains[op.idx].conv1 >= 0)
-                        add(convs[chains[op.idx].conv1].conv, convs[chains[op.idx].conv1].out_t, (int)oi, chains[op.idx].conv1);
-                    break;
-                case OP_FUSE:
-                    for (int k = 0; k < fuses[op.idx].group; ++k) add(fuses[op.idx + k].name, fuses[op.idx + k].out_t, (int)oi, -1);
-                    break;
-                default: break;
-            }
-        }
-    }
+        for (int pass = 0; pass < 2; ++pass) {
+            const bool plain = pass == 1;
+            const std::vector<Op> &list = plain ? ops_plain : ops;
+            const size_t known = taps.size();
+            auto add = [&](const std::string &name, int tensor, int op, int conv) {
+                for (size_t i = 0; i < taps.size(); ++i)
+                    if (taps[i].name == name) {
+                        if (i >= known || !plain) taps[i].op = op;
+                        return;
+                    }
+                taps.push_back(TapPoint{name, tensor, op, conv, plain});
+            };
+            auto add_conv_tap = [&](int ci, bool absorb, int oi) {
+                const ConvOp &cv = convs[ci];
+                if (absorb && cv.absorb_fuse >= 0)
+                    add(fuses[cv.absorb_fuse].name, fuses[cv.absorb_fuse].out_t, oi, -1);
+                else
+                    add(cv.conv, cv.out_t, oi, ci);
+            };
+            for (size_t oi = 0; oi < list.size(); ++oi) {
+                const Op &op = list[oi];
+                switch (op.kind) {
+                    case OP_STEM:
+                    case OP_STEM7: add("stem", stem_out_t, (int)oi, -1); break;
+                    case OP_MAXPOOL: add("maxpool", pool_out_t, (int)oi, -1); break;
+                    case OP_CONV: add_conv_tap(op.idx, op.n != 0, (int)oi); break;
+                    case OP_CONV3_GROUP:
+                        for (int ci : groups[op.idx].conv_idx) add(convs[ci].conv, convs[ci].out_t, (int)oi, ci);
+                        break;
+                    case OP_CONV_GROUP:
+                        for (int ci : dgroups[op.idx].conv_idx) add_conv_tap(ci, op.n != 0, (int)oi);
+                        break;
+                    case OP_S2_GROUP:
+                        for (int ci : s2groups[op.idx].conv_idx) add(convs[ci].conv, convs[ci].out_t, (int)oi, ci);
+                        break;
+                    case OP_CHAIN:
+                        add(convs[chains[op.idx].conv3].conv, convs[chains[op.idx].conv3].out_t, (int)oi, chains[op.idx].conv3);
+                        if (chains[op.idx].conv1 >= 0)
+                            add(convs[chains[op.idx].conv1].conv, convs[chains[op.idx].conv1].out_t, (int)oi, chains[op.idx].conv1);
+                        break;
+                    case OP_FUSE:
+                        for (int k = 0; k < fuse_count(op); ++k) add(fuses[op.idx + k].name, fuses[op.idx + k].out_t, (int)oi, -1);
+                        break;
+                    default: break;
+                }
+            }
+        }
+    }
+    int fuse_count(const Op &op) const { return op.n ? op.n : fuses[op.idx].group; }
 
     void layout_blob() {
         int64_t off = 0;
diff --git a/simple-hrnet_amd/csrc/ctx_run.inc b/simple-hrnet_amd/csrc/ctx_run.inc
--- a/simple-hrnet_amd/csrc/ctx_run.inc
+++ b/simple-hrnet_amd/csrc/ctx_run.inc
@@ -6,13 +6,14 @@
                   hipStream_t s, Timing *tm, int flip = 0, const TapReq *tap = nullptr, int refine = RF_NONE) {
         if (tm && !hip_ok(hipEventRecord(tm->ev[0], s), "hipEventRecord")) return false;
         const bool fused_stem = stem_fuse && !(tap && tap->op == 0);
-        for (size_t oi = 0; oi < ops.size(); ++oi) {
+        const std::vector<Op> &list = (tap && tap->plain) ? ops_plain : ops;
+        for (size_t oi = 0; oi < list.size(); ++oi) {
             const bool rev = alternate && (oi & 1);
             hipError_t e = hipSuccess;
             if (fused_stem && oi == 0)
                 e = exec_stem_fused(images, nb, s, flip);
             else if (!(fused_stem && (int)oi == stem_conv2_op))
-                e = exec_op(ops[oi], rev, images, nb, boxes, box_dtype, pts, heatmaps, s, flip, refine);
+                e = exec_op(list[oi], rev, images, nb, boxes, box_dtype, pts, heatmaps, s, flip, refine);
             if (!hip_ok(e, "kernel launch")) return false;
             if (tap && tap->op == (int)oi) {
                 const Tensor &t = tensors[tap->tensor];
@@ -92,7 +93,7 @@
         }
         case OP_CONV: {
             const ConvOp &cv = convs[op.idx];
-            const ConvArgs a = conv_args(cv, nb, rev);
+            const ConvArgs a = conv_args(cv, nb, rev, op.n != 0);
             e = launch_conv(dtype, a, cv.nr, s);
             break;
         }
@@ -121,10 +122,10 @@
         case OP_CONV_GROUP: {
             DirectGroup &g = dgroups[op.idx];
             bool hit;
-            MapSlot *sl = find_slot(g.slot, nb, &hit);
+            MapSlot *sl = find_slot(op.n ? g.slot_absorb : g.slot, nb, &hit);
             if ((e = slot_ready(sl, hit, s)) != hipSuccess) break;
             if (!hit) {
-                for (size_t k = 0; k < g.conv_idx.size(); ++k) sl->args_pin[k] = conv_args(convs[g.conv_idx[k]], nb, rev);
+                for (size_t k = 0; k < g.conv_idx.size(); ++k) sl->args_pin[k] = conv_args(convs[g.conv_idx[k]], nb, rev, op.n != 0);
                 sl->mr = 4;
                 while (sl->mr > 1 && direct_group_blocks(g, nb, nullptr, sl->mr) < 512) sl->mr >>= 1;
                 sl->nblocks = direct_group_blocks(g, nb, &g.map_host, sl->mr);
@@ -146,7 +147,7 @@
                 if (wl)
                     for (int ci : g.conv_idx)
                         if (conv_xl(convs[ci])) wl = 2;
-                e = launch_conv_group(dtype, sl->args_dev, sl->dev, sl->nblocks, g.nr, sl->mr, wl, s);
+                e = launch_conv_group(dtype, sl->args_dev, sl->dev, sl->nblocks, g.nr, sl->mr, wl, op.n, s);
             }
             break;
         }
@@ -208,17 +209,13 @@
         }
         case OP_FUSE: {
             FuseGroupArgs ga;
-            ga.nf = fuses[op.idx].group;
+            ga.nf = fuse_count(op);
             for (int k = 0; k < ga.nf; ++k) {
                 const FuseOp &f = fuses[op.idx + k];
                 const Tensor &to = tensors[f.out_t];
                 FuseArgs &a = ga.f[k];
                 a.nterms = f.nterms;
-                for (int i = 0; i < f.nterms; ++i) {
-                    const Tensor &tt = tensors[f.term_t[i]];
-                    a.t[i].ptr = row0(f.term_t[i]), a.t[i].shift = f.shift[i];
-                    a.t[i].wp = tt.wp, a.t[i].hpwp = tt.hpwp;
-                }
+                for (int i = 0; i < f.nterms; ++i) a.t[i] = fuse_term(f, i);
                 for (int i = f.nterms; i < 4; ++i) a.t[i] = FuseTerm{nullptr, 0, 0, 0};
                 a.out = row0(f.out_t), a.c = to.c, a.h = to.h, a.w = to.w, a.wp = to.wp, a.hpwp = to.hpwp;
                 a.m = nb * to.hpwp, a.rev = rev;
diff --git a/simple-hrnet_amd/csrc/ctx_types.h b/simple-hrnet_amd/csrc/ctx_types.h
--- a/simple-hrnet_amd/csrc/ctx_types.h
+++ b/simple-hrnet_amd/csrc/ctx_types.h
@@ -34,6 +34,7 @@
     bool compact = false;
     bool s2 = false;
     bool w2_image = false;
+    int absorb_fuse = -1;
     int64_t w2_off = 0, w2_bytes = 0;
     double flops = 0;
 };
@@ -65,12 +66,15 @@
     int nr = 0;
     int64_t map_capacity = 0;
     MapSlot slot[kMapSlots];
+    bool has_absorber = false;
+    MapSlot slot_absorb[kMapSlots];
     std::vector<int2> map_host;
 };
 
 struct Op {
     OpKind kind;
     int idx;
+    int n = 0;
 };
 
 struct S2Group {
@@ -94,6 +98,7 @@
     int nterms;
     int out_t;
     std::string name;
+    int out_index = 0;
     int group = 1;
 };
 
@@ -102,10 +107,12 @@
     int tensor;
     int op;
     int conv;
+    bool plain;
 };
 struct TapReq {
     int op, tensor, crop0, ncrops, crop_step;
     float *dst;
+    bool plain;
 };
 
 inline void fast_div(int d, unsigned *magic, int *shift) {
diff --git a/simple-hrnet_amd/csrc/hrnet_mi355.cpp b/simple-hrnet_amd/csrc/hrnet_mi355.cpp
--- a/simple-hrnet_amd/csrc/hrnet_mi355.cpp
+++ b/simple-hrnet_amd/csrc/hrnet_mi355.cpp
@@ -61,6 +61,12 @@
     std::vector<TapPoint> taps;
     Conv3Problem *probs_dev = nullptr;
     std::vector<Op> ops;
+    struct PlainSeg {
+        size_t begin, end;
+        std::vector<Op> plain;
+    };
+    std::vector<PlainSeg> plain_segs;
+    std::vector<Op> ops_plain;
     int stem_out_t = -1, head_in_t = -1;
     int64_t stem_w_off = 0, stem_b_off = 0, stem_wp_off = 0, head_w_off = 0, head_b_off = 0, head_wp_off = 0;
 
@@ -94,6 +100,7 @@
     bool disable_lds32 = env_sw("HRN_DISABLE_LDS32") != nullptr;
     bool disable_n96 = env_sw("HRN_DISABLE_N96") != nullptr;
     bool disable_fgroup = env_sw("HRN_DISABLE_FGROUP") != nullptr;
+    bool disable_fuse_absorb = env_sw("HRN_DISABLE_FUSE_ABSORB") != nullptr;
     bool disable_f32lds = env_sw("HRN_DISABLE_F32LDS") != nullptr;
     int f32_small_slices = env_sw("HRN_F32_SMALL_SLICES") ? atoi(env_sw("HRN_F32_SMALL_SLICES")) : 0;
     std::vector<Conv3Problem> probs_host;
@@ -1362,7 +1369,7 @@
         return 7;
     }
     if (!h->hip_ok(hipSetDevice(h->device), "hipSetDevice")) return 6;
-    const TapReq req{tp->op, tp->tensor, crop0, ncrops, crop_step, dst_dev};
+    const TapReq req{tp->op, tp->tensor, crop0, ncrops, crop_step, dst_dev, tp->plain};
     CallScope scope(h, &h->pass, (hipStream_t)stream);
     if (!scope.entered) return 6;
     if (!h->run_pass((const float *)images_dev, n, nullptr, 0, nullptr, heatmaps_dev, (hipStream_t)stream, nullptr, 0, &req)) return 8;
@@ -1398,6 +1405,26 @@
 int64_t hrn_map_rebuilds(hrn_handle h) { return h ? h->map_builds : -1; }
 int hrn_launches_per_pass(hrn_handle h) { return h ? (int)h->ops.size() - (h->stem_fuse ? 1 : 0) : 0; }
 int hrn_stem_fused(hrn_handle h) { return h && h->stem_fuse ? 1 : 0; }
+
+int hrn_fuse_launch_count(hrn_handle h, int unabsorbed) {
+    if (!h) return 0;
+    int n = 0;
+    for (const Op &op : (unabsorbed && !h->ops_plain.empty()) ? h->ops_plain : h->ops) n += op.kind == OP_FUSE;
+    return n;
+}
+
+int hrn_get_fuse_launch_info(hrn_handle h, int unabsorbed, int index, hrn_fuse_launch_info *out) {
+    if (!h || !out || index < 0) return 1;
+    for (const Op &op : (unabsorbed && !h->ops_plain.empty()) ? h->ops_plain : h->ops) {
+        if (op.kind != OP_FUSE || index-- > 0) continue;
+        const FuseOp &f = h->fuses[op.idx];
+        memset(out, 0, sizeof *out);
+        snprintf(out->stage, sizeof out->stage, "%s", f.name.substr(0, f.name.rfind(".fuse.")).c_str());
+        out->first_output = f.out_index, out->outputs = h->fuse_count(op);
+        return 0;
+    }
+    return 1;
+}
 int hrn_conv_compact(hrn_handle h, int index) { return h && index >= 0 && index < (int)h->convs.size() && h->convs[index].compact ? 1 : 0; }
 const char *hrn_switches(hrn_handle h) { return h ? h->switches.c_str() : ""; }
 
diff --git a/simple-hrnet_amd/csrc/kernels.h b/simple-hrnet_amd/csrc/kernels.h
--- a/simple-hrnet_amd/csrc/kernels.h
+++ b/simple-hrnet_amd/csrc/kernels.h
@@ -28,6 +28,12 @@
 }
 
 enum { DT_F32 = 0, DT_BF16 = 1, DT_F16 = 2 };
+
+struct FuseTerm {
+    const void *ptr;
+    int shift;
+    int wp, hpwp;
+};
 
 struct ConvArgs {
     const void *in;
@@ -47,6 +53,8 @@
     int xlds;
     int up, up_a, up_b, up_wp, up_hpwp;
     int taps[4];
+    int fuse_n, fuse_own;
+    FuseTerm fuse_t[4];
 };
 
 struct Conv3Problem {
@@ -204,11 +212,6 @@
 hipError_t launch_stem7(int dtype, const Stem7Args &a, hipStream_t s);
 hipError_t launch_maxpool(int dtype, const PoolArgs &a, hipStream_t s);
 
-struct FuseTerm {
-    const void *ptr;
-    int shift;
-    int wp, hpwp;
-};
 struct FuseArgs {
     FuseTerm t[4];
     int nterms;
@@ -423,7 +426,7 @@
 hipError_t launch_pad_check(int dtype, const PadCheckArgs &a, hipStream_t s);
 
 hipError_t launch_conv(int dtype, const ConvArgs &a, int nr, hipStream_t s);
-hipError_t launch_conv_group(int dtype, const ConvArgs *probs_dev, const void *map_dev, int nblocks, int nr, int mr, int wlds,
+hipError_t launch_conv_group(int dtype, const ConvArgs *probs_dev, const void *map_dev, int nblocks, int nr, int mr, int wlds, int absorb,
                              hipStream_t s);
 hipError_t launch_conv3x3_lds(const Conv3Problem *probs_dev, const void *blockmap_dev, int nblocks, int nb, int ks,
                               int nrb, hipStream_t s);
diff --git a/simple-hrnet_amd/csrc/kernels.hip b/simple-hrnet_amd/csrc/kernels.hip
--- a/simple-hrnet_amd/csrc/kernels.hip
+++ b/simple-hrnet_amd/csrc/kernels.hip
@@ -73,7 +73,34 @@
 #define HRN_WL_G 4
 #endif
 constexpr int WL_G = HRN_WL_G;
-template <int DT, int NR, int MR, bool PRE>
+template <int DT>
+__device__ __forceinline__ s16x8 fuse_absorb8(const ConvArgs &p, const s16x8 own, const int q, const int n, const int ho, const int wo,
+                                              const bool ok, const int ch) {
+    using T = Tr<DT>;
+    using elem = typename T::elem;
+    float sum[8];
+#pragma unroll
+    for (int t = 0; t < 4; ++t) {
+        if (t >= p.fuse_n) break;
+        s16x8 v = own;
+        if (t != p.fuse_own) {
+            const FuseTerm ft = p.fuse_t[t];
+            const long row = ft.shift == 0 ? (long)q : (long)n * ft.hpwp + (long)(ho >> ft.shift) * ft.wp + (wo >> ft.shift);
+            v = *(const GLOBAL_AS s16x8 *)((const GLOBAL_AS elem *)ft.ptr + row * p.cout + ch);
+        }
+#pragma unroll
+        for (int e = 0; e < 8; ++e) {
+            const float f = T::ld((elem)v[e]);
+            sum[e] = (t == 0) ? f : sum[e] + f;
+        }
+    }
+    s16x8 o8;
+#pragma unroll
+    for (int e = 0; e < 8; ++e) o8[e] = (short)T::st(ok ? fmaxf(sum[e], 0.f) : 0.f);
+    return o8;
+}
+
+template <int DT, int NR, int MR, bool PRE, bool ABS = false>
 __device__ __forceinline__ void conv_direct_epilogue(const ConvArgs &p, const int ng, const int m0, const int li, const int g,
                                                      f32x4 (&acc)[MR][NR], s16x8 (&rpre)[PRE ? MR : 1][PRE ? NR / 2 : 1]) {
     using T = Tr<DT>;
@@ -113,6 +140,8 @@
                     if (!ok) v = 0.f;
                     o8[r] = (short)T::st(v);
                 }
+                if constexpr (ABS)
+                    if (p.fuse_n) o8 = fuse_absorb8<DT>(p, o8, q, q / p.out_hpwp, ho, wo, ok, ch0 + j * 4);
                 *(GLOBAL_AS s16x8 *)(out + o + j * 4) = o8;
             }
         } else {
@@ -135,7 +164,7 @@
     }
 }
 
-template <int DT, int NR, int MR, bool PRE = false, bool WL = false>
+template <int DT, int NR, int MR, bool PRE = false, bool WL = false, bool ABS = false>
 __device__ __forceinline__ void conv_direct_body(const ConvArgs &p, const int ng, const int mtile_in, char *smem = nullptr) {
     using T = Tr<DT>;
     using vec = typename T::vec;
@@ -288,7 +317,7 @@
         }
     }
 
-    conv_direct_epilogue<DT, NR, MR, PRE>(p, ng, m0, li, g, acc, rpre);
+    conv_direct_epilogue<DT, NR, MR, PRE, ABS>(p, ng, m0, li, g, acc, rpre);
 }
 
 constexpr int XL_G = 2, XL_D = 3;
@@ -299,7 +328,7 @@
 __device__ __forceinline__ void xl_glds(const GLOBAL_AS char *base, unsigned voff, unsigned lds_dst) {
     asm volatile("s_mov_b32 m0, %1\n\ts_nop 0\n\tglobal_load_lds_dwordx4 %0, %2" ::"v"(voff), "s"(lds_dst), "s"(base) : "memory", "m0");
 }
-template <int DT, int NR>
+template <int DT, int NR, bool ABS = false>
 __device__ __forceinline__ void conv_direct_xl_body(const ConvArgs &p, const int ng, const int mtile_in, char *smem) {
     constexpr int MR = 4;
     const int lane = threadIdx.x & 63, wave = __builtin_amdgcn_readfirstlane(threadIdx.x >> 6);
@@ -381,10 +410,10 @@
     }
     asm volatile("s_waitcnt vmcnt(0)" ::: "memory");
     s16x8 rpre[1][1];
-    conv_direct_epilogue<DT, NR, MR, false>(p, ng, m0, li, g, acc, rpre);
-}
-
-template <int DT, int NR, int MR, bool PRE, bool WL = false>
+    conv_direct_epilogue<DT, NR, MR, false, ABS>(p, ng, m0, li, g, acc, rpre);
+}
+
+template <int DT, int NR, int MR, bool PRE, bool WL = false, bool ABS = false>
 __global__ __launch_bounds__(256) void conv_direct_kernel(const ConvArgs p) {
     extern __shared__ __attribute__((aligned(16))) char smem_direct[];
     const int ngroups = p.cout / (16 * NR);
@@ -392,14 +421,14 @@
     const int mtile = (blockIdx.x / (8 * ngroups)) * 8 + (blockIdx.x & 7);
     if constexpr (WL && is16(DT) && NR == 6 && MR == 4 && !PRE) {
         if (p.xlds && conv_xl_ok(p)) {
-            conv_direct_xl_body<DT, NR>(p, ng, mtile, smem_direct);
+            conv_direct_xl_body<DT, NR, ABS>(p, ng, mtile, smem_direct);
             return;
         }
     }
-    conv_direct_body<DT, NR, MR, PRE, WL>(p, ng, mtile, smem_direct);
-}
-
-template <int DT, int NR, int MR, bool WL = false>
+    conv_direct_body<DT, NR, MR, PRE, WL, ABS>(p, ng, mtile, smem_direct);
+}
+
+template <int DT, int NR, int MR, bool WL = false, bool ABS = false>
 __global__ __launch_bounds__(256) void conv_direct_group_kernel(const ConvArgs *__restrict__ probs,
                                                                 const int2 *__restrict__ map) {
     extern __shared__ __attribute__((aligned(16))) char smem_direct[];
@@ -409,11 +438,11 @@
     const ConvArgs p = probs[prob];
     if constexpr (WL && is16(DT) && NR == 6 && MR == 4) {
         if (p.xlds && conv_xl_ok(p)) {
-            conv_direct_xl_body<DT, NR>(p, ng, mtile, smem_direct);
+            conv_direct_xl_body<DT, NR, ABS>(p, ng, mtile, smem_direct);
             return;
         }
     }
-    conv_direct_body<DT, NR, MR, false, WL>(p, ng, mtile, smem_direct);
+    conv_direct_body<DT, NR, MR, false, WL, ABS>(p, ng, mtile, smem_direct);
 }
 
 template <int DT, int NR>
@@ -423,31 +452,38 @@
     return wl;
 }
 
-template <int DT, int NR>
+template <int DT, int NR, bool ABS = false>
 static hipError_t launch_conv_group_t(const ConvArgs *probs, const int2 *map, int nblocks, int mr, int wlds, hipStream_t s) {
     if (mr == 1)
-        hipLaunchKernelGGL((conv_direct_group_kernel<DT, NR, 1>), dim3(nblocks), dim3(256), 0, s, probs, map);
+        hipLaunchKernelGGL((conv_direct_group_kernel<DT, NR, 1, false, ABS>), dim3(nblocks), dim3(256), 0, s, probs, map);
     else if (mr == 2)
-        hipLaunchKernelGGL((conv_direct_group_kernel<DT, NR, 2>), dim3(nblocks), dim3(256), 0, s, probs, map);
+        hipLaunchKernelGGL((conv_direct_group_kernel<DT, NR, 2, false, ABS>), dim3(nblocks), dim3(256), 0, s, probs, map);
     else if (is16(DT) && wlds)
     {
         const int lds = direct_lds_bytes<DT, NR>(wlds);
         static std::atomic<unsigned long long> lds_set{0};
         if (lds > 65536) {
-            const hipError_t e = set_dynamic_lds((const void *)conv_direct_group_kernel<DT, NR, 4, is16(DT)>, direct_lds_bytes<DT, NR>(2), lds_set);
+            const hipError_t e = set_dynamic_lds((const void *)conv_direct_group_kernel<DT, NR, 4, is16(DT), ABS>, direct_lds_bytes<DT, NR>(2), lds_set);
             if (e != hipSuccess) return e;
         }
-        hipLaunchKernelGGL((conv_direct_group_kernel<DT, NR, 4, is16(DT)>), dim3(nblocks), dim3(256), lds, s, probs, map);
+        hipLaunchKernelGGL((conv_direct_group_kernel<DT, NR, 4, is16(DT), ABS>), dim3(nblocks), dim3(256), lds, s, probs, map);
     }
     else
-        hipLaunchKernelGGL((conv_direct_group_kernel<DT, NR, 4>), dim3(nblocks), dim3(256), 0, s, probs, map);
+        hipLaunchKernelGGL((conv_direct_group_kernel<DT, NR, 4, false, ABS>), dim3(nblocks), dim3(256), 0, s, probs, map);
     return hipGetLastError();
 }
 
-hipError_t launch_conv_group(int dtype, const ConvArgs *probs_dev, const void *map_dev, int nblocks, int nr, int mr, int wlds,
+hipError_t launch_conv_group(int dtype, const ConvArgs *probs_dev, const void *map_dev, int nblocks, int nr, int mr, int wlds, int absorb,
                              hipStream_t s) {
     if (nblocks <= 0) return hipSuccess;
     const int2 *map = (const int2 *)map_dev;
+    if (absorb) {
+        if (dtype == DT_BF16 && nr == 6) return launch_conv_group_t<DT_BF16, 6, true>(probs_dev, map, nblocks, mr, wlds, s);
+        if (dtype == DT_BF16 && nr == 4) return launch_conv_group_t<DT_BF16, 4, true>(probs_dev, map, nblocks, mr, wlds, s);
+        if (dtype == DT_F16 && nr == 6) return launch_conv_group_t<DT_F16, 6, true>(probs_dev, map, nblocks, mr, wlds, s);
+        if (dtype == DT_F16 && nr == 4) return launch_conv_group_t<DT_F16, 4, true>(probs_dev, map, nblocks, mr, wlds, s);
+        return hipErrorInvalidValue;
+    }
     if (dtype == DT_BF16) {
         if (nr == 6) return launch_conv_group_t<DT_BF16, 6>(probs_dev, map, nblocks, mr, wlds, s);
         if (nr == 4) return launch_conv_group_t<DT_BF16, 4>(probs_dev, map, nblocks, mr, wlds, s);
@@ -466,17 +502,17 @@
     return hipErrorInvalidValue;
 }
 
-template <int DT, int NR, int MR, bool PRE>
+template <int DT, int NR, int MR, bool PRE, bool ABS = false>
 static hipError_t launch_conv_tt(const ConvArgs &a, hipStream_t s) {
     const int mtiles = (a.m + 64 * MR - 1) / (64 * MR);
     dim3 grid(((mtiles + 7) / 8) * 8 * (a.cout / (16 * NR)));
-    hipLaunchKernelGGL((conv_direct_kernel<DT, NR, MR, PRE>), grid, dim3(256), 0, s, a);
+    hipLaunchKernelGGL((conv_direct_kernel<DT, NR, MR, PRE, false, ABS>), grid, dim3(256), 0, s, a);
     return hipGetLastError();
 }
 
-template <int DT, int NR>
+template <int DT, int NR, bool ABS = false>
 static hipError_t launch_conv_t(const ConvArgs &a, hipStream_t s) {
-    if constexpr (is16(DT) && NR % 2 == 0) {
+    if constexpr (is16(DT) && NR % 2 == 0 && !ABS) {
         const int pre_mode = a.pre_mode;
         if (a.res && a.ksize == 1 && pre_mode == 1) return launch_conv_tt<DT, NR, 4, true>(a, s);
         if (a.res && a.ksize == 1 && pre_mode == 2) return launch_conv_tt<DT, NR, 2, true>(a, s);
@@ -484,8 +520,8 @@
     }
     const int ngroups = a.cout / (16 * NR);
     const long blocks4 = (long)((a.m + 255) / 256) * ngroups;
-    if (blocks4 < 256) return launch_conv_tt<DT, NR, 1, false>(a, s);
-    if (blocks4 < 512) return launch_conv_tt<DT, NR, 2, false>(a, s);
+    if (blocks4 < 256) return launch_conv_tt<DT, NR, 1, false, ABS>(a, s);
+    if (blocks4 < 512) return launch_conv_tt<DT, NR, 2, false, ABS>(a, s);
     if constexpr (is16(DT))
         if (a.wlds && a.kchunks >= 2 * WL_G) {
             const int mtiles = (a.m + 255) / 256;
@@ -493,17 +529,24 @@
             const int lds = direct_lds_bytes<DT, NR>(a.xlds ? 2 : 1);
             static std::atomic<unsigned long long> lds_set{0};
             if (lds > 65536) {
-                const hipError_t e = set_dynamic_lds((const void *)conv_direct_kernel<DT, NR, 4, false, true>, direct_lds_bytes<DT, NR>(2), lds_set);
+                const hipError_t e = set_dynamic_lds((const void *)conv_direct_kernel<DT, NR, 4, false, true, ABS>, direct_lds_bytes<DT, NR>(2), lds_set);
                 if (e != hipSuccess) return e;
             }
-            hipLaunchKernelGGL((conv_direct_kernel<DT, NR, 4, false, true>), grid, dim3(256), lds, s, a);
+            hipLaunchKernelGGL((conv_direct_kernel<DT, NR, 4, false, true, ABS>), grid, dim3(256), lds, s, a);
             return hipGetLastError();
         }
-    return launch_conv_tt<DT, NR, 4, false>(a, s);
+    return launch_conv_tt<DT, NR, 4, false, ABS>(a, s);
 }
 
 hipError_t launch_conv(int dtype, const ConvArgs &a, int nr, hipStream_t s) {
     if (a.m <= 0) return hipSuccess;
+    if (a.fuse_n) {
+        if (dtype == DT_BF16 && nr == 6) return launch_conv_t<DT_BF16, 6, true>(a, s);
+        if (dtype == DT_BF16 && nr == 4) return launch_conv_t<DT_BF16, 4, true>(a, s);
+        if (dtype == DT_F16 && nr == 6) return launch_conv_t<DT_F16, 6, true>(a, s);
+        if (dtype == DT_F16 && nr == 4) return launch_conv_t<DT_F16, 4, true>(a, s);
+        return hipErrorInvalidValue;
+    }
     if (dtype == DT_BF16) {
         if (nr == 6) return launch_conv_t<DT_BF16, 6>(a, s);
         if (nr == 4) return launch_conv_t<DT_BF16, 4>(a, s);
diff --git a/simple-hrnet_amd/native.py b/simple-hrnet_amd/native.py
--- a/simple-hrnet_amd/native.py
+++ b/simple-hrnet_amd/native.py
@@ -1059,6 +1059,14 @@
     def stem_fused(self) -> bool:
         return bool(self._lib.hrn_stem_fused(self._h))
 
+    def fuse_launches(self, unabsorbed: bool = False) -> List[Tuple[str, List[int]]]:
+        out = []
+        for i in range(self._lib.hrn_fuse_launch_count(self._h, int(unabsorbed))):
+            fi = _lib.FuseLaunchInfo()
+            self._check(self._lib.hrn_get_fuse_launch_info(self._h, int(unabsorbed), i, ctypes.byref(fi)), "hrn_get_fuse_launch_info")
+            out.append((fi.stage.decode(), list(range(fi.first_output, fi.first_output + fi.outputs))))
+        return out
+
     def pad_violations(self) -> int:
         return int(self._lib.hrn_debug_pad_violations(self._h))
 
```

Result: no change. 10760 crops/s (-0.1%).
